# microsoft/tutel

Measured on AMD Instinct MI355X. Metric: MoE-layer fwd tokens/sec, 4096 tok x H=2048 x E=64 top-2, higher is better.
Workload: dtype bf16

## Files before the change

### include/tutel_amd.h

```cpp
#ifndef TUTEL_AMD_H
#define TUTEL_AMD_H

#include <stddef.h>
#include <stdint.h>

#ifdef __cplusplus
extern "C" {
#endif

#define TUTEL_AMD_ABI_VERSION 1

typedef void *tutel_stream_t;

enum { TUTEL_F32 = 0, TUTEL_F16 = 1, TUTEL_BF16 = 2, TUTEL_F64 = 3 };
enum { TUTEL_ACT_NONE = 0, TUTEL_ACT_RELU = 1, TUTEL_ACT_GELU = 2, TUTEL_ACT_SILU = 3 };

int tutel_amd_abi_version(void);
const char *tutel_amd_target_arch(void);
const char *tutel_amd_last_error(void);

size_t tutel_amd_routing_workspace_bytes(int T, int E, int k);

int tutel_amd_gate_topk(const void *in, int dtype, int apply_softmax, int T, int E, int k,
                        int normalize_gate, void *scores_out, int32_t *idx, void *gates, void *ws,
                        size_t ws_bytes, int32_t *clear_map, int clear_n, tutel_stream_t stream);

int tutel_amd_gate_proj_splits(int T, int M, int E, int dtype);
int tutel_amd_gate_proj(const void *x, const void *wg, int dtype, int T, int M, int E, float *partials,
                        size_t partial_bytes, tutel_stream_t stream);
int tutel_amd_gate_topk_partials(const float *partials, int splits, int dtype, int T, int E, int k,
                                 int normalize_gate, void *logits_out, void *scores_out, int32_t *idx, void *gates,
                                 void *ws, size_t ws_bytes, int32_t *clear_map, int clear_n, tutel_stream_t stream);

int tutel_amd_cache_warm(const void *p, size_t chunk_bytes, int n_chunks, size_t stride_bytes, int blocks, void *sink4,
                         tutel_stream_t stream);

int tutel_amd_compute_location(const int32_t *idx, int T, int E, int k, int hist_ready, void *ws,
                               size_t ws_bytes, int32_t *loc, int32_t *dispatch_count,
                               int32_t *stats, void *l_aux, int l_aux_dtype, int capacity,
                               int32_t *slot_map, int slot_map_cleared, tutel_stream_t stream);

int tutel_amd_slot_map(const int32_t *idx, const int32_t *loc, int T, int E, int k, int capacity,
                       int32_t *slot_map, tutel_stream_t stream);

int tutel_amd_cumsum_sub_one(const int32_t *mask, int32_t *out, int T, int E,
                             tutel_stream_t stream);

int tutel_amd_fast_encode(const void *x, int dtype, const int32_t *slot_map, const void *gates,
                          int gate_dtype, int T, int M, int n_slots, int capacity, int num_experts,
                          int chunk_rows, int expert_slice, int ep_world, void *out,
                          tutel_stream_t stream);

int tutel_amd_fast_decode(const void *buf, int dtype, const int32_t *idx, const int32_t *loc,
                          const void *gates, int gate_dtype, int T, int M, int k, int capacity,
                          int num_experts, int chunk_rows, int expert_slice, int ep_world, void *out,
                          tutel_stream_t stream);

int tutel_amd_gate_grad(const void *x, const void *buf, int dtype, const int32_t *idx,
                        const int32_t *loc, int T, int M, int k, int capacity, float *ggate,
                        tutel_stream_t stream);

int tutel_amd_expert_gemm(const void *A, int64_t a_stride_e, int64_t a_stride_w, int a_rows_per_w,
                          int lda, const void *W, int w_kmajor, int64_t w_stride_e, int ldw,
                          const void *bias, int64_t bias_stride_e, void *D, int64_t d_stride_e,
                          int64_t d_stride_w, int d_rows_per_w, int ldd, int E_loc, int R, int N,
                          int K, int dtype, int act, const int32_t *row_counts, int row_align,
                          tutel_stream_t stream);

int tutel_amd_expert_gemm_gather(const void *X, int ldx, const int32_t *slot_map, int T,
                                 const void *zero_row, const void *W, int w_kmajor,
                                 int64_t w_stride_e, int ldw, const void *bias,
                                 int64_t bias_stride_e, void *D, int64_t d_stride_e, int ldd,
                                 int E_loc, int R, int N, int K, int dtype, int act,
                                 const int32_t *row_counts, int row_align, tutel_stream_t stream);

int tutel_amd_expert_ffn(const void *A, int64_t x_stride_e, int ldx, const int32_t *slot_map, int T, const void *zero_row,
                         const void *W1, int64_t w1_stride_e, int ldw1, const void *b1, int64_t b1_stride_e, void *hid,
                         int64_t hid_stride_e, int ldh, const void *W2, int64_t w2_stride_e, int ldw2, const void *b2,
                         int64_t b2_stride_e, void *D, int64_t d_stride_e, int ldd, int E_loc, int R, int M, int H, int M_out,
                         int dtype, int act, tutel_stream_t stream);

int tutel_amd_expert_gemm_glu(const void *A, int64_t a_stride_e, int64_t a_stride_w,
                              int a_rows_per_w, int lda, const void *W, int w_kmajor,
                              int64_t w_stride_e, int ldw, const void *bias, int64_t bias_stride_e,
                              const void *G, void *D, int64_t d_stride_e, int64_t d_stride_w,
                              int d_rows_per_w, int ldd, int E_loc, int R, int N, int K, int dtype,
                              int act, const int32_t *row_counts, int row_align,
                              tutel_stream_t stream);

int tutel_amd_expert_gemm_gate_up(const void *A, int64_t a_stride_e, int64_t a_stride_w, int a_rows_per_w, int lda,
                                  const void *W_gate, const void *W_up, int64_t w_stride_e, int ldw, void *D, int64_t d_stride_e,
                                  int64_t d_stride_w, int d_rows_per_w, int ldd, int E_loc, int R, int N, int K, int dtype, int act,
                                  const int32_t *row_counts, int row_align, tutel_stream_t stream);

typedef struct tutel_amd_ep_comm tutel_amd_ep_comm_t;
#define TUTEL_AMD_EP_ID_BYTES 128

int tutel_amd_ep_load_rccl(const char *path_hint );
int tutel_amd_ep_unique_id(void *out, size_t bytes );
int tutel_amd_ep_comm_create(const void *id, size_t bytes, int world, int rank, tutel_amd_ep_comm_t **out);
int tutel_amd_ep_comm_destroy(tutel_amd_ep_comm_t *comm);
typedef int (*tutel_amd_exchange_fn)(void *user, const void *send, void *recv, size_t bytes_per_peer, int world);
int tutel_amd_ep_comm_create_hosted(int world, int rank, tutel_amd_exchange_fn fn, void *user, tutel_amd_ep_comm_t **out);
int tutel_amd_ep_comm_info(const tutel_amd_ep_comm_t *comm, int *world, int *rank);

typedef struct tutel_amd_ep_segment tutel_amd_ep_segment_t;
#define TUTEL_AMD_IPC_HANDLE_BYTES 64
int tutel_amd_ep_segment_alloc(size_t bytes, int flag_memory, tutel_amd_ep_segment_t **out, void *handle_out, size_t handle_bytes);
int tutel_amd_ep_segment_open(tutel_amd_ep_segment_t *seg, int world, int rank, const void *handles, size_t handle_bytes);
void *tutel_amd_ep_segment_ptr(const tutel_amd_ep_segment_t *seg, int peer);
int tutel_amd_ep_segment_read(const tutel_amd_ep_segment_t *seg, size_t off, void *dst, size_t bytes, tutel_stream_t stream);
int tutel_amd_ep_segment_free(tutel_amd_ep_segment_t *seg);
size_t tutel_amd_ep_flag_bytes(void);
int tutel_amd_ep_comm_create_ipc(int world, int rank, tutel_amd_ep_comm_t **out);
int tutel_amd_ep_comm_attach_ipc(tutel_amd_ep_comm_t *comm, tutel_amd_ep_segment_t *flags, int timeout_ms);
int tutel_amd_ep_comm_has_ipc(const tutel_amd_ep_comm_t *comm);
int tutel_amd_ep_ipc_set_timeout(tutel_amd_ep_comm_t *comm, int timeout_ms);
int tutel_amd_ep_ipc_status(tutel_amd_ep_comm_t *comm);
int tutel_amd_ep_ipc_exchange(tutel_amd_ep_comm_t *comm, tutel_amd_ep_segment_t *seg, const void *send, size_t bytes_per_peer,
                              size_t recv_off, tutel_stream_t stream);
int tutel_amd_ep_ipc_selfcheck(tutel_amd_ep_comm_t *comm, tutel_amd_ep_segment_t *seg, size_t bytes_per_peer, int passes, int flavour,
                               int side_stream, unsigned long long *mismatch, tutel_stream_t stream);

int tutel_amd_ep_all_to_all(tutel_amd_ep_comm_t *comm, const void *send, void *recv, size_t bytes_per_peer,
                            tutel_stream_t stream);

typedef int (*tutel_amd_exchange_v_fn)(void *user, const void *send, void *recv, const uint64_t *send_bytes,
                                       const uint64_t *send_offsets, const uint64_t *recv_bytes, int world);
int tutel_amd_ep_comm_set_hosted_v(tutel_amd_ep_comm_t *comm, tutel_amd_exchange_v_fn fn);
int tutel_amd_ep_all_to_all_v(tutel_amd_ep_comm_t *comm, const void *send, void *recv, const uint64_t *send_bytes,
                              const uint64_t *recv_bytes, tutel_stream_t stream);
int tutel_amd_ep_all_gather_v(tutel_amd_ep_comm_t *comm, const void *send, void *recv, const uint64_t *recv_bytes,
                              tutel_stream_t stream);

typedef struct {
  int sliced;
  int experts_per_stage;
  int chunk;
  int rows;
  int gemm_rows;
} tutel_amd_ep_plan_t;
int tutel_amd_ep_plan(int num_experts, int world, int capacity, int degree, int allow_sliced, tutel_amd_ep_plan_t *out);

typedef struct {
  int T, M, H, M_out;
  int num_experts, world, k;
  int capacity;
  int degree;
  int allow_sliced;
  int dtype, gate_dtype, act;
  int is_postscore;
  int w2_kmajor;
  int fuse_encode;
  const void *x;
  const int32_t *slot_map;
  const int32_t *idx, *loc;
  const void *gates;
  const void *w1, *b1, *w2, *b2;
  void *enc, *recv, *hid, *send, *back;
  const void *zero_row;
  const int32_t *row_counts;
  int row_align;
  void *y;
  const struct tutel_amd_ep_segment *peer_seg;
} tutel_amd_ep_args_t;
int tutel_amd_ep_forward(tutel_amd_ep_comm_t *comm, const tutel_amd_ep_args_t *args, tutel_stream_t stream);

typedef struct {
  tutel_amd_ep_args_t ep;
  const void *logits;
  int logits_dtype;
  int normalize_gate;
  void *ws;
  size_t ws_bytes;
  int32_t *dispatch_count;
  int32_t *stats;
  void *l_aux;
  int capacity_limit, alignment, max_capacity;
  int *capacity_out;
  const void *gate_w;
  float *gate_partials;
  size_t gate_partial_bytes;
  void *logits_out;
  void *fl_ws;
  size_t fl_ws_bytes;
} tutel_amd_moe_args_t;
#define TUTEL_AMD_EAGAIN 1000
#define TUTEL_AMD_ENOTSUP 1001
int tutel_amd_moe_forward(tutel_amd_ep_comm_t *comm, const tutel_amd_moe_args_t *args, tutel_stream_t stream);

typedef struct {
  void *ws;
  size_t ws_bytes;
  int32_t *offsets;
  int32_t *capacity;
} tutel_amd_packed_args_t;
typedef struct {
  int rows_bound;
  int tiles_bound;
  int tile_rows;
  int row_limit;
  size_t ws_bytes;
} tutel_amd_packed_plan_t;
int tutel_amd_packed_plan(int T, int E, int k, int M, int H, int M_out, int dtype, int capacity_limit, int alignment,
                          tutel_amd_packed_plan_t *out);
size_t tutel_amd_moe_packed_workspace_bytes(int T, int E, int k, int M, int H, int M_out, int dtype, int capacity_limit,
                                            int alignment);
int tutel_amd_moe_forward_packed(tutel_amd_ep_comm_t *comm, const tutel_amd_moe_args_t *args,
                                 const tutel_amd_packed_args_t *packed, tutel_stream_t stream);
int tutel_amd_moe_forward_packed_glu(tutel_amd_ep_comm_t *comm, const tutel_amd_moe_args_t *args,
                                     const tutel_amd_packed_args_t *packed, const void *w_up, tutel_stream_t stream);

int tutel_amd_packed_layout(const int32_t *dispatch_count, const int32_t *idx, const int32_t *loc, int T, int E, int k,
                            int capacity_limit, int alignment, int rows_bound, int tiles_bound, int32_t *offsets, int32_t *tiles,
                            int32_t *ntiles, int32_t *capacity, int32_t *slot_map, tutel_stream_t stream);
int tutel_amd_expert_gemm_packed(const void *A, int lda, const int32_t *a_rows, int T, const void *zero_row, const void *W,
                                 int w_kmajor, int64_t w_stride_e, int ldw, const void *bias, int64_t bias_stride_e, const void *mul,
                                 void *D, int ldd, int E, int rows_bound, int N, int K, int dtype, int act, const int32_t *offsets,
                                 const int32_t *tiles, const int32_t *ntiles, const int32_t *capacity, int tiles_bound,
                                 tutel_stream_t stream);
int tutel_amd_expert_wgrad_packed(const void *A, int lda, const void *B, int ldb, const int32_t *rows_map, int gather, int T,
                                  const void *zero_row, void *D, int E, int rows_bound, int Na, int Nb, int dtype,
                                  const int32_t *offsets, tutel_stream_t stream);
int tutel_amd_expert_bgrad_packed(const void *B, int ldb, void *D, int E, int N, int dtype, const int32_t *offsets,
                                  tutel_stream_t stream);
int tutel_amd_gate_grad_packed(const void *x, const void *buf, int dtype, const int32_t *idx, const int32_t *loc, int T, int M,
                               int k, int row_limit, const int32_t *offsets, float *ggate, tutel_stream_t stream);
int tutel_amd_fast_decode_packed(const void *buf, int dtype, const int32_t *idx, const int32_t *loc, const void *gates, int gate_dtype,
                                 int T, int M, int k, int row_limit, const int32_t *offsets, void *out, tutel_stream_t stream);

int tutel_amd_range_push(const char *name);
int tutel_amd_range_pop(void);

enum {
  TUTEL_STAGE_GATE_TOPK = 0, TUTEL_STAGE_LOCATION = 1, TUTEL_STAGE_ENCODE = 2, TUTEL_STAGE_FC1 = 3, TUTEL_STAGE_FC2 = 4,
  TUTEL_STAGE_DECODE = 5, TUTEL_STAGE_A2A_DISPATCH = 6, TUTEL_STAGE_A2A_COMBINE = 7, TUTEL_STAGE_OTHER = 8, TUTEL_STAGE_GATE_PROJ = 9,
  TUTEL_STAGE_COUNT = 10
};
int tutel_amd_stage_timing(int enable);
int tutel_amd_stage_report(double *total_us, int *counts, int n_stages );
int tutel_amd_mark(tutel_stream_t stream);
int tutel_amd_marks_reserve(int n);
int tutel_amd_marks_report(double *delta_us, int n);

#define TUTEL_OPT_GEMM_IMPL 0
#define TUTEL_OPT_GEMM_TILE 1
#define TUTEL_OPT_DECODE 2
#define TUTEL_OPT_EP_STAGE_GRID 3
#define TUTEL_OPT_GEMM_PERSIST 4
#define TUTEL_OPT_EP_STREAMS 5
#define TUTEL_OPT_EP_CANARY 6
#define TUTEL_OPT_GEMM_SPLITK 7
#define TUTEL_OPT_GEMM_GATHER 8
#define TUTEL_OPT_FUSED_LOCATION 9
#define TUTEL_OPT_GEMM_STORE 10
#define TUTEL_OPT_TIE_RULE 11
#define TUTEL_OPT_FFN_FUSED 12
#define TUTEL_OPT_COUNT 13
int tutel_amd_set_option(int key, int value);

int tutel_amd_probe_tr16(uint16_t *out, tutel_stream_t stream);

#ifdef __cplusplus
}
#endif
#endif
```

### tutel_amd/_lib.py

```python
import ctypes
import os
import subprocess

_HERE = os.path.dirname(os.path.abspath(__file__))
LIB_PATH = os.path.join(_HERE, "lib", "libtutel_amd.so")
CSRC_DIR = os.path.join(_HERE, "csrc")

F32, F16, BF16, F64 = 0, 1, 2, 3
ACT_NONE, ACT_RELU, ACT_GELU, ACT_SILU = 0, 1, 2, 3
OPT_GEMM_IMPL, OPT_GEMM_TILE, OPT_DECODE, OPT_EP_STAGE_GRID, OPT_GEMM_PERSIST, OPT_EP_STREAMS, OPT_EP_CANARY, OPT_GEMM_SPLITK, OPT_GEMM_GATHER, OPT_FUSED_LOCATION, OPT_GEMM_STORE, OPT_TIE_RULE, OPT_FFN_FUSED = 0, 1, 2, 3, 4, 5, 6, 7, 8, 9, 10, 11, 12

_vp, _i, _i64, _sz = ctypes.c_void_p, ctypes.c_int, ctypes.c_int64, ctypes.c_size_t

SIGNATURES = {
    "tutel_amd_abi_version": (_i, []),
    "tutel_amd_target_arch": (ctypes.c_char_p, []),
    "tutel_amd_last_error": (ctypes.c_char_p, []),
    "tutel_amd_routing_workspace_bytes": (_sz, [_i, _i, _i]),
    "tutel_amd_gate_topk": (_i, [_vp, _i, _i, _i, _i, _i, _i, _vp, _vp, _vp, _vp, _sz, _vp, _i, _vp]),
    "tutel_amd_gate_proj_splits": (_i, [_i, _i, _i, _i]),
    "tutel_amd_gate_proj": (_i, [_vp, _vp, _i, _i, _i, _i, _vp, _sz, _vp]),
    "tutel_amd_gate_topk_partials": (_i, [_vp, _i, _i, _i, _i, _i, _i, _vp, _vp, _vp, _vp, _vp, _sz, _vp, _i, _vp]),
    "tutel_amd_cache_warm": (_i, [_vp, _sz, _i, _sz, _i, _vp, _vp]),
    "tutel_amd_compute_location": (_i, [_vp, _i, _i, _i, _i, _vp, _sz, _vp, _vp, _vp, _vp, _i, _i, _vp, _i, _vp]),
    "tutel_amd_slot_map": (_i, [_vp, _vp, _i, _i, _i, _i, _vp, _vp]),
    "tutel_amd_cumsum_sub_one": (_i, [_vp, _vp, _i, _i, _vp]),
    "tutel_amd_fast_encode": (_i, [_vp, _i, _vp, _vp, _i, _i, _i, _i, _i, _i, _i, _i, _i, _vp, _vp]),
    "tutel_amd_fast_decode": (_i, [_vp, _i, _vp, _vp, _vp, _i, _i, _i, _i, _i, _i, _i, _i, _i, _vp, _vp]),
    "tutel_amd_gate_grad": (_i, [_vp, _vp, _i, _vp, _vp, _i, _i, _i, _i, _vp, _vp]),
    "tutel_amd_expert_gemm": (_i, [_vp, _i64, _i64, _i, _i, _vp, _i, _i64, _i, _vp, _i64, _vp, _i64,
                                   _i64, _i, _i, _i, _i, _i, _i, _i, _i, _vp, _i, _vp]),
    "tutel_amd_expert_gemm_gather": (_i, [_vp, _i, _vp, _i, _vp, _vp, _i, _i64, _i, _vp, _i64, _vp, _i64, _i,
                                          _i, _i, _i, _i, _i, _i, _vp, _i, _vp]),
    "tutel_amd_expert_ffn": (_i, [_vp, _i64, _i, _vp, _i, _vp, _vp, _i64, _i, _vp, _i64, _vp, _i64, _i, _vp, _i64, _i, _vp, _i64, _vp, _i64, _i,
                                  _i, _i, _i, _i, _i, _i, _i, _vp]),
    "tutel_amd_expert_gemm_glu": (_i, [_vp, _i64, _i64, _i, _i, _vp, _i, _i64, _i, _vp, _i64, _vp, _vp, _i64,
                                       _i64, _i, _i, _i, _i, _i, _i, _i, _i, _vp, _i, _vp]),
    "tutel_amd_expert_gemm_gate_up": (_i, [_vp, _i64, _i64, _i, _i, _vp, _vp, _i64, _i, _vp, _i64, _i64, _i, _i,
                                           _i, _i, _i, _i, _i, _i, _vp, _i, _vp]),
    "tutel_amd_set_option": (_i, [_i, _i]),
    "tutel_amd_probe_tr16": (_i, [_vp, _vp]),
}



class EpPlan(ctypes.Structure):
    _fields_ = [(n, _i) for n in ("sliced", "experts_per_stage", "chunk", "rows", "gemm_rows")]


class EpArgs(ctypes.Structure):
    _fields_ = ([(n, _i) for n in ("T", "M", "H", "M_out", "num_experts", "world", "k", "capacity", "degree", "allow_sliced",
                                   "dtype", "gate_dtype", "act", "is_postscore", "w2_kmajor", "fuse_encode")] +
                [(n, _vp) for n in ("x", "slot_map", "idx", "loc", "gates", "w1", "b1", "w2", "b2",
                                    "enc", "recv", "hid", "send", "back", "zero_row", "row_counts")] +
                [("row_align", _i), ("y", _vp), ("peer_seg", _vp)])


class MoeArgs(ctypes.Structure):
    _fields_ = [("ep", EpArgs), ("logits", _vp), ("logits_dtype", _i), ("normalize_gate", _i), ("ws", _vp), ("ws_bytes", _sz),
                ("dispatch_count", _vp), ("stats", _vp), ("l_aux", _vp),
                ("capacity_limit", _i), ("alignment", _i), ("max_capacity", _i), ("capacity_out", ctypes.POINTER(_i)),
                ("gate_w", _vp), ("gate_partials", _vp), ("gate_partial_bytes", _sz), ("logits_out", _vp),
                ("fl_ws", _vp), ("fl_ws_bytes", _sz)]


class PackedArgs(ctypes.Structure):
    _fields_ = [("ws", _vp), ("ws_bytes", _sz), ("offsets", _vp), ("capacity", _vp)]


class PackedPlan(ctypes.Structure):
    _fields_ = [("rows_bound", _i), ("tiles_bound", _i), ("tile_rows", _i), ("row_limit", _i), ("ws_bytes", _sz)]


SIGNATURES.update({
    "tutel_amd_moe_forward": (_i, [_vp, ctypes.POINTER(MoeArgs), _vp]),
    "tutel_amd_packed_plan": (_i, [_i] * 9 + [ctypes.POINTER(PackedPlan)]),
    "tutel_amd_moe_packed_workspace_bytes": (_sz, [_i] * 9),
    "tutel_amd_moe_forward_packed": (_i, [_vp, ctypes.POINTER(MoeArgs), ctypes.POINTER(PackedArgs), _vp]),
    "tutel_amd_moe_forward_packed_glu": (_i, [_vp, ctypes.POINTER(MoeArgs), ctypes.POINTER(PackedArgs), _vp, _vp]),
    "tutel_amd_packed_layout": (_i, [_vp, _vp, _vp] + [_i] * 7 + [_vp] * 6),
    "tutel_amd_expert_gemm_packed": (_i, [_vp, _i, _vp, _i, _vp, _vp, _i, _i64, _i, _vp, _i64, _vp, _vp] + [_i] * 7 + [_vp] * 4 + [_i, _vp]),
    "tutel_amd_expert_wgrad_packed": (_i, [_vp, _i, _vp, _i, _vp, _i, _i, _vp, _vp] + [_i] * 5 + [_vp, _vp]),
    "tutel_amd_expert_bgrad_packed": (_i, [_vp, _i, _vp, _i, _i, _i, _vp, _vp]),
    "tutel_amd_gate_grad_packed": (_i, [_vp, _vp, _i, _vp, _vp] + [_i] * 4 + [_vp, _vp, _vp]),
    "tutel_amd_fast_decode_packed": (_i, [_vp, _i, _vp, _vp, _vp] + [_i] * 5 + [_vp, _vp, _vp]),
    "tutel_amd_ep_load_rccl": (_i, [ctypes.c_char_p]),
    "tutel_amd_ep_unique_id": (_i, [_vp, _sz]),
    "tutel_amd_ep_comm_create": (_i, [_vp, _sz, _i, _i, ctypes.POINTER(_vp)]),
    "tutel_amd_ep_comm_destroy": (_i, [_vp]),
    "tutel_amd_ep_comm_create_hosted": (_i, [_i, _i, _vp, _vp, ctypes.POINTER(_vp)]),
    "tutel_amd_ep_comm_info": (_i, [_vp, ctypes.POINTER(_i), ctypes.POINTER(_i)]),
    "tutel_amd_ep_all_to_all": (_i, [_vp, _vp, _vp, _sz, _vp]),
    "tutel_amd_ep_comm_set_hosted_v": (_i, [_vp, _vp]),
    "tutel_amd_ep_all_to_all_v": (_i, [_vp, _vp, _vp, ctypes.POINTER(ctypes.c_uint64), ctypes.POINTER(ctypes.c_uint64), _vp]),
    "tutel_amd_ep_all_gather_v": (_i, [_vp, _vp, _vp, ctypes.POINTER(ctypes.c_uint64), _vp]),
    "tutel_amd_ep_plan": (_i, [_i, _i, _i, _i, _i, ctypes.POINTER(EpPlan)]),
    "tutel_amd_ep_forward": (_i, [_vp, ctypes.POINTER(EpArgs), _vp]),
    "tutel_amd_ep_segment_alloc": (_i, [_sz, _i, ctypes.POINTER(_vp), _vp, _sz]),
    "tutel_amd_ep_segment_open": (_i, [_vp, _i, _i, _vp, _sz]),
    "tutel_amd_ep_segment_ptr": (_vp, [_vp, _i]),
    "tutel_amd_ep_segment_read": (_i, [_vp, _sz, _vp, _sz, _vp]),
    "tutel_amd_ep_segment_free": (_i, [_vp]),
    "tutel_amd_ep_flag_bytes": (_sz, []),
    "tutel_amd_ep_comm_create_ipc": (_i, [_i, _i, ctypes.POINTER(_vp)]),
    "tutel_amd_ep_comm_attach_ipc": (_i, [_vp, _vp, _i]),
    "tutel_amd_ep_comm_has_ipc": (_i, [_vp]),
    "tutel_amd_ep_ipc_set_timeout": (_i, [_vp, _i]),
    "tutel_amd_ep_ipc_status": (_i, [_vp]),
    "tutel_amd_ep_ipc_exchange": (_i, [_vp, _vp, _vp, _sz, _sz, _vp]),
    "tutel_amd_ep_ipc_selfcheck": (_i, [_vp, _vp, _sz, _i, _i, _i, _vp, _vp]),
    "tutel_amd_mark": (_i, [_vp]),
    "tutel_amd_marks_reserve": (_i, [_i]),
    "tutel_amd_marks_report": (_i, [ctypes.POINTER(ctypes.c_double), _i]),
    "tutel_amd_stage_timing": (_i, [_i]),
    "tutel_amd_stage_report": (_i, [ctypes.POINTER(ctypes.c_double), ctypes.POINTER(_i), _i]),
    "tutel_amd_range_push": (_i, [ctypes.c_char_p]),
    "tutel_amd_range_pop": (_i, []),
})
EXCHANGE_FN = ctypes.CFUNCTYPE(_i, _vp, _vp, _vp, _sz, _i)
_u64p = ctypes.POINTER(ctypes.c_uint64)
EXCHANGE_V_FN = ctypes.CFUNCTYPE(_i, _vp, _vp, _vp, _u64p, _u64p, _u64p, _i)
EP_ID_BYTES = 128
IPC_HANDLE_BYTES = 64
EAGAIN, ENOTSUP = 1000, 1001
STAGES = ("gate_topk", "location", "fast_encode", "expert_fc1", "expert_fc2", "fast_decode", "all_to_all_dispatch", "all_to_all_combine", "other",
          "gate_projection")

_lib = None


class TutelAmdError(RuntimeError):
    pass


def build(force=False):
    if force or not os.path.exists(LIB_PATH):
        subprocess.check_call(["make", "-C", CSRC_DIR, "-j8"] + (["-B"] if force else []))
    return LIB_PATH


def lib():
    global _lib
    if _lib is None:
        import torch
        if not os.path.exists(LIB_PATH):
            raise TutelAmdError(
                f"tutel_amd: HIP library {LIB_PATH} is missing. Build it with "
                f"`python -c 'import __graft_entry__ as g; g.build()'` or `make -C tutel_amd/csrc` "
                f"(hipcc --offload-arch=gfx950). There is no CPU fallback for the MoE hot path.")
        try:
            handle = ctypes.CDLL(LIB_PATH)
        except OSError as ex:
            raise TutelAmdError(f"tutel_amd: cannot load {LIB_PATH}: {ex}") from ex
        for name, (res, args) in SIGNATURES.items():
            try:
                fn = getattr(handle, name)
            except AttributeError as ex:
                raise TutelAmdError(f"tutel_amd: {LIB_PATH} does not export `{name}` (stale build?)") from ex
            fn.restype, fn.argtypes = res, args
        if handle.tutel_amd_abi_version() != 1:
            raise TutelAmdError("tutel_amd: ABI version mismatch between python and libtutel_amd.so")
        _lib = handle
    return _lib


def check(status, what):
    if status != 0:
        msg = lib().tutel_amd_last_error().decode("utf-8", "replace")
        raise TutelAmdError(f"{what} failed (status {status}): {msg}")
```

### tutel_amd/csrc/api.hip

```cpp
#include <stdarg.h>
#include <stdlib.h>

#include "common.h"

static thread_local char g_err[512] = "";

void tutel_set_error(const char *fmt, ...) {
  va_list ap;
  va_start(ap, fmt);
  vsnprintf(g_err, sizeof(g_err), fmt, ap);
  va_end(ap);
}

extern "C" int tutel_amd_abi_version(void) { return TUTEL_AMD_ABI_VERSION; }
extern "C" const char *tutel_amd_target_arch(void) { return "gfx950"; }
extern "C" const char *tutel_amd_last_error(void) { return g_err; }

static int g_opt[TUTEL_OPT_COUNT] = {-2, -2, -2, -2, -2, -2, -2, -2, -2, -2, -2, -2, -2};
static const char *const g_opt_env[TUTEL_OPT_COUNT] = {"TUTEL_AMD_GEMM_IMPL", "TUTEL_AMD_GEMM_BIG", "TUTEL_AMD_DECODE", "TUTEL_AMD_EP_STAGE_GRID",
                                                       "TUTEL_AMD_GEMM_PERSIST", "TUTEL_AMD_EP_STREAMS", "TUTEL_AMD_EP_CANARY", "TUTEL_AMD_GEMM_SPLITK",
                                                       "TUTEL_AMD_GEMM_GATHER", "TUTEL_AMD_FUSED_LOCATION", "TUTEL_AMD_GEMM_STORE", "TUTEL_AMD_TIE_RULE", "TUTEL_AMD_FFN_FUSED"};

int tutel_get_option(int key) {
  if (key < 0 || key >= TUTEL_OPT_COUNT) return -1;
  if (g_opt[key] == -2) {
    const char *s = getenv(g_opt_env[key]);
    g_opt[key] = s ? atoi(s) : -1;
  }
  return g_opt[key];
}

extern "C" int tutel_amd_set_option(int key, int value) {
  TUTEL_REQUIRE(key >= 0 && key < TUTEL_OPT_COUNT, "tutel_amd_set_option: unknown key %d", key);
  TUTEL_REQUIRE(value >= -1 && value <= 7, "tutel_amd_set_option: value %d out of range", value);
  g_opt[key] = value;
  return 0;
}

#include <dlfcn.h>
static thread_local int g_stage_hint = -1;
static int (*g_roctx_push)(const char *) = nullptr;
static int (*g_roctx_pop)() = nullptr;
static void roctx_init() {
  static bool done = false;
  if (done) return;
  done = true;
  void *h = dlopen("libroctx64.so", RTLD_NOW | RTLD_NOLOAD);
  if (h == nullptr) h = dlopen("libroctx64.so.4", RTLD_NOW | RTLD_NOLOAD);
  if (h == nullptr && getenv("TUTEL_AMD_ROCTX") != nullptr) h = dlopen("libroctx64.so", RTLD_NOW | RTLD_GLOBAL);
  if (h == nullptr) return;
  g_roctx_push = (int (*)(const char *))dlsym(h, "roctxRangePushA");
  g_roctx_pop = (int (*)())dlsym(h, "roctxRangePop");
  if (g_roctx_push == nullptr || g_roctx_pop == nullptr) g_roctx_push = nullptr;
}
extern "C" int tutel_amd_range_push(const char *name) {
  roctx_init();
  return g_roctx_push ? g_roctx_push(name) : 0;
}
extern "C" int tutel_amd_range_pop(void) { return g_roctx_push ? g_roctx_pop() : 0; }
static const char *const g_stage_names[TUTEL_STAGE_COUNT] = {
    "tutel_amd.gate_topk", "tutel_amd.compute_location", "tutel_amd.fast_encode", "tutel_amd.expert_fc1", "tutel_amd.expert_fc2",
    "tutel_amd.fast_decode", "tutel_amd.all_to_all_dispatch", "tutel_amd.all_to_all_combine", "tutel_amd.other", "tutel_amd.gate_projection"};
void tutel_stage_range_push(int stage) {
  roctx_init();
  if (g_stage_hint >= 0) stage = g_stage_hint;
  if (g_roctx_push) g_roctx_push(g_stage_names[stage >= 0 && stage < TUTEL_STAGE_COUNT ? stage : TUTEL_STAGE_OTHER]);
}
void tutel_stage_range_pop() {
  if (g_roctx_push) g_roctx_pop();
}

#include <mutex>
#include <vector>
static std::mutex g_meas_mu;
struct StageRec { hipEvent_t a, b; int stage; };
static std::vector<StageRec> g_recs;
static std::vector<std::pair<hipEvent_t, hipEvent_t>> g_free;
static int g_timing = 0;

void tutel_stage_hint(int stage) { g_stage_hint = stage; }
static thread_local int g_gemm_corun = 0;
void tutel_gemm_corun_hint(int on) { g_gemm_corun = on; }
int tutel_gemm_corun() { return g_gemm_corun; }

int tutel_stage_begin(int stage, hipStream_t st) {
  if (!g_timing) return -1;
  if (g_stage_hint >= 0) stage = g_stage_hint;
  if (g_timing == 2 && stage != TUTEL_STAGE_FC1 && stage != TUTEL_STAGE_FC2) return -1;
  hipStreamCaptureStatus cs = hipStreamCaptureStatusNone;
  if (hipStreamIsCapturing(st, &cs) != hipSuccess || cs != hipStreamCaptureStatusNone) return -1;
  std::lock_guard<std::mutex> lock(g_meas_mu);
  StageRec r;
  r.stage = stage;
  if (!g_free.empty()) {
    r.a = g_free.back().first;
    r.b = g_free.back().second;
    g_free.pop_back();
  } else if (hipEventCreateWithFlags(&r.a, hipEventReleaseToDevice) != hipSuccess ||
             hipEventCreateWithFlags(&r.b, hipEventReleaseToDevice) != hipSuccess) {
    return -1;
  }
  (void)hipEventRecord(r.a, st);
  g_recs.push_back(r);
  return (int)g_recs.size() - 1;
}
void tutel_stage_end(int token, hipStream_t st) {
  if (token < 0) return;
  std::lock_guard<std::mutex> lock(g_meas_mu);
  if (token < (int)g_recs.size()) (void)hipEventRecord(g_recs[token].b, st);
}

static std::vector<hipEvent_t> g_marks;
static std::vector<hipEvent_t> g_marks_free;
extern "C" int tutel_amd_mark(tutel_stream_t stream) {
  std::lock_guard<std::mutex> lock(g_meas_mu);
  hipEvent_t ev;
  if (!g_marks_free.empty()) {
    ev = g_marks_free.back();
    g_marks_free.pop_back();
  } else {
    TUTEL_REQUIRE(hipEventCreateWithFlags(&ev, hipEventReleaseToDevice) == hipSuccess, "tutel_amd_mark: cannot create an event");
  }
  TUTEL_REQUIRE(hipEventRecord(ev, (hipStream_t)stream) == hipSuccess, "tutel_amd_mark: hipEventRecord failed");
  g_marks.push_back(ev);
  return 0;
}
extern "C" int tutel_amd_marks_reserve(int n) {
  std::lock_guard<std::mutex> lock(g_meas_mu);
  while ((int)g_marks_free.size() < n) {
    hipEvent_t ev;
    TUTEL_REQUIRE(hipEventCreateWithFlags(&ev, hipEventReleaseToDevice) == hipSuccess, "tutel_amd_marks_reserve: cannot create an event");
    g_marks_free.push_back(ev);
  }
  return 0;
}
extern "C" int tutel_amd_marks_report(double *delta_us, int n) {
  std::lock_guard<std::mutex> lock(g_meas_mu);
  const int have = (int)g_marks.size();
  int m = 0;
  for (int i = 0; i + 1 < have; ++i) {
    float ms = 0.f;
    if (hipEventSynchronize(g_marks[i + 1]) == hipSuccess && hipEventElapsedTime(&ms, g_marks[i], g_marks[i + 1]) == hipSuccess && m < n && delta_us)
      delta_us[m++] = 1e3 * ms;
  }
  for (auto ev : g_marks) g_marks_free.push_back(ev);
  g_marks.clear();
  return m;
}

extern "C" int tutel_amd_stage_timing(int enable) {
  g_timing = enable < 0 ? 0 : enable > 2 ? 1 : enable;
  return 0;
}

extern "C" int tutel_amd_stage_report(double *total_us, int *counts, int n_stages) {
  TUTEL_REQUIRE(total_us != nullptr && counts != nullptr && n_stages >= TUTEL_STAGE_COUNT, "tutel_amd_stage_report: need arrays of %d entries", TUTEL_STAGE_COUNT);
  for (int i = 0; i < n_stages; ++i) { total_us[i] = 0.0; counts[i] = 0; }
  std::lock_guard<std::mutex> lock(g_meas_mu);
  for (auto &r : g_recs) {
    float ms = 0.f;
    if (hipEventSynchronize(r.b) == hipSuccess && hipEventElapsedTime(&ms, r.a, r.b) == hipSuccess && r.stage >= 0 && r.stage < n_stages) {
      total_us[r.stage] += 1e3 * ms;
      counts[r.stage] += 1;
    }
    g_free.push_back({r.a, r.b});
  }
  g_recs.clear();
  return 0;
}
```

### tutel_amd/csrc/common.h

```cpp
#pragma once
#include <hip/hip_runtime.h>
#include <stdint.h>
#include <stdio.h>
#include <string.h>

#include "../../include/tutel_amd.h"

#define WAVE 64

void tutel_set_error(const char *fmt, ...);
int tutel_get_option(int key);

int tutel_stage_begin(int stage, hipStream_t st);
void tutel_stage_end(int token, hipStream_t st);
void tutel_stage_hint(int stage);
void tutel_gemm_corun_hint(int on);
int tutel_gemm_corun();
void tutel_stage_range_push(int stage);
void tutel_stage_range_pop();
struct StageScope {
  int token;
  hipStream_t st;
  StageScope(int stage, hipStream_t s) : token(tutel_stage_begin(stage, s)), st(s) { tutel_stage_range_push(stage); }
  ~StageScope() {
    tutel_stage_end(token, st);
    tutel_stage_range_pop();
  }
};

#define EP_NCAN 16
struct PeerCanary {
  const uint32_t *epoch;
  long long off;
  int world;
  int stale;
};
struct EncodePeer {
  const uint64_t *tab;
  long long off;
  int rank, rows;
  int slot0;
  PeerCanary can;
};
int tutel_encode_launch(const void *x, int dtype, const int32_t *slot_map, const void *gates, int gate_dtype, int T, int M,
                        int n_slots, int capacity, int num_experts, int chunk_rows, int expert_slice, int ep_world, void *out,
                        const EncodePeer &peer, hipStream_t st);
int tutel_expert_gemm_peer(const void *A, int64_t a_stride_e, int64_t a_stride_w, int a_rows_per_w, int lda, const void *W,
                           int w_kmajor, int64_t w_stride_e, int ldw, const void *bias, int64_t bias_stride_e,
                           const uint64_t *d_peer, int64_t d_peer_off, int64_t d_stride_e, int d_rows_per_w, int ldd, int E_loc,
                           int R, int N, int K, int dtype, int act, const PeerCanary &can, hipStream_t st);

int tutel_expert_gemm_gather_fl(const void *X, int ldx, int32_t *slot_map, int T, const void *zero_row, const void *W, int64_t w_stride_e,
                                int ldw, const void *bias, int64_t bias_stride_e, void *D, int64_t d_stride_e, int ldd, int E_loc, int R,
                                int N, int K, int dtype, int act, const uint8_t *idx8, int n, int32_t *loc, hipStream_t st);
int tutel_expert_ffn(const void *X, int64_t x_stride_e, int ldx, const int32_t *slot_map, int T, const void *zero_row, const void *W1,
                     int64_t w1_stride_e, int ldw1, const void *b1, int64_t b1_stride_e, void *hid, int64_t hid_stride_e, int ldh,
                     const void *W2, int64_t w2_stride_e, int ldw2, const void *b2, int64_t b2_stride_e, void *D, int64_t d_stride_e, int ldd,
                     int E_loc, int R, int M, int H, int M_out, int dtype, int act, const uint8_t *idx8, int n, int32_t *loc, int query,
                     hipStream_t st);
struct RouteFinish;
void tutel_route_finish_args(int T, int E, int k, void *ws, RouteFinish *out);
int tutel_decode_finish_launch(const void *buf, int dtype, const int32_t *idx, const int32_t *loc, const void *gates, int gate_dtype, int T, int M,
                               int k, int capacity, int num_experts, void *out, const RouteFinish &fin, hipStream_t st);
#define PK_TILE_ROWS 256
int tutel_expert_gemm_packed(const void *A, int lda, const int32_t *a_rows, int T, const void *zero_row, const void *W, int64_t w_stride_e,
                             int ldw, const void *bias, int64_t bias_stride_e, void *D, int ldd, int E, int rows_bound, int N, int K, int dtype,
                             int act, const int32_t *off, const int32_t *tiles, const int32_t *ntiles, const int32_t *cap, int tiles_bound,
                             hipStream_t st);
int tutel_expert_gemm_packed_ex(const void *A, int lda, const int32_t *a_rows, int T, const void *zero_row, const void *W, int w_kmajor,
                                int64_t w_stride_e, int ldw, const void *bias, int64_t bias_stride_e, const void *mul, void *D, int ldd, int E,
                                int rows_bound, int N, int K, int dtype, int act, const int32_t *off, const int32_t *tiles, const int32_t *ntiles,
                                const int32_t *cap, int tiles_bound, hipStream_t st);
int tutel_expert_gemm_gate_up_packed(const void *A, int lda, const int32_t *a_rows, int T, const void *zero_row, const void *W_gate,
                                     const void *W_up, int64_t w_stride_e, int ldw, void *D, int ldd, int E, int rows_bound, int N, int K,
                                     int dtype, int act, const int32_t *off, const int32_t *tiles, const int32_t *ntiles, const int32_t *cap,
                                     int tiles_bound, hipStream_t st);
int tutel_decode_packed_launch(const void *buf, int dtype, const int32_t *idx, const int32_t *loc, const void *gates, int gate_dtype, int T,
                               int M, int k, int row_limit, const int32_t *off, void *out, hipStream_t st);
int tutel_gate_topk_launch(const void *in, const float *partials, int splits, int dtype, int T, int E, int k, int normalize_gate,
                           void *logits_out, int32_t *idx, void *gates, void *ws, int32_t *clear_map, int clear_n, uint8_t *idx8,
                           hipStream_t st);

#define TUTEL_REQUIRE(cond, ...)           \
  do {                                     \
    if (!(cond)) {                         \
      tutel_set_error(__VA_ARGS__);        \
      return -1;                           \
    }                                      \
  } while (0)

#define TUTEL_CHECK_LAUNCH(what)                                                    \
  do {                                                                              \
    hipError_t _e = hipGetLastError();                                              \
    if (_e != hipSuccess) {                                                         \
      tutel_set_error("%s: launch failed: %s", what, hipGetErrorString(_e));        \
      return (int)_e;                                                               \
    }                                                                               \
  } while (0)

struct bf16_t { uint16_t v; };
struct f16_t { _Float16 v; };

__device__ __forceinline__ uint16_t f32_to_bf16_bits(float f) {
  uint32_t u = __float_as_uint(f);
  if ((u & 0x7fffffffu) > 0x7f800000u) return 0x7fc0;
  u += 0x7fffu + ((u >> 16) & 1u);
  return (uint16_t)(u >> 16);
}
__device__ __forceinline__ float bf16_bits_to_f32(uint16_t b) {
  return __uint_as_float(((uint32_t)b) << 16);
}

template <typename T> struct Elem;
template <> struct Elem<double> {
  using ct = double;
  static constexpr int dtype = 3;
  __device__ static __forceinline__ double to_f32(double x) { return x; }
  __device__ static __forceinline__ double from_f32(double x) { return x; }
  __device__ static __forceinline__ double eps() { return 2.220446049250313e-16; }
};
template <> struct Elem<float> {
  using ct = float;
  static constexpr int dtype = TUTEL_F32;
  __device__ static __forceinline__ float to_f32(float x) { return x; }
  __device__ static __forceinline__ float from_f32(float x) { return x; }
  __device__ static __forceinline__ float eps() { return 1.1920928955078125e-07f; }
};
template <> struct Elem<bf16_t> {
  using ct = float;
  static constexpr int dtype = TUTEL_BF16;
  __device__ static __forceinline__ float to_f32(bf16_t x) { return bf16_bits_to_f32(x.v); }
  __device__ static __forceinline__ bf16_t from_f32(float x) { return bf16_t{f32_to_bf16_bits(x)}; }
  __device__ static __forceinline__ float eps() { return 0.0078125f; }
};
template <> struct Elem<f16_t> {
  using ct = float;
  static constexpr int dtype = TUTEL_F16;
  __device__ static __forceinline__ float to_f32(f16_t x) { return (float)x.v; }
  __device__ static __forceinline__ f16_t from_f32(float x) { return f16_t{(_Float16)x}; }
  __device__ static __forceinline__ float eps() { return 0.0009765625f; }
};

template <typename T> __device__ __forceinline__ typename Elem<T>::ct round_to(typename Elem<T>::ct x) {
  return Elem<T>::to_f32(Elem<T>::from_f32(x));
}
__device__ __forceinline__ float ct_exp(float x) { return expf(x); }
__device__ __forceinline__ double ct_exp(double x) { return exp(x); }
__device__ __forceinline__ float ct_max(float a, float b) { return fmaxf(a, b); }
__device__ __forceinline__ double ct_max(double a, double b) { return fmax(a, b); }

static inline int dtype_size(int dtype) { return dtype == TUTEL_F32 ? 4 : 2; }
static inline bool dtype_ok(int dtype) {
  return dtype == TUTEL_F32 || dtype == TUTEL_F16 || dtype == TUTEL_BF16;
}

struct __attribute__((aligned(16))) vec16 { uint32_t w[4]; };

template <typename T> struct Vec;
template <> struct Vec<float> {
  static constexpr int N = 4;
  __device__ static __forceinline__ void unpack(const vec16 &v, float *f) {
#pragma unroll
    for (int i = 0; i < 4; ++i) f[i] = __uint_as_float(v.w[i]);
  }
  __device__ static __forceinline__ void pack(const float *f, vec16 &v) {
#pragma unroll
    for (int i = 0; i < 4; ++i) v.w[i] = __float_as_uint(f[i]);
  }
};
template <> struct Vec<bf16_t> {
  static constexpr int N = 8;
  __device__ static __forceinline__ void unpack(const vec16 &v, float *f) {
#pragma unroll
    for (int i = 0; i < 4; ++i) {
      f[2 * i] = __uint_as_float(v.w[i] << 16);
      f[2 * i + 1] = __uint_as_float(v.w[i] & 0xffff0000u);
    }
  }
  __device__ static __forceinline__ void pack(const float *f, vec16 &v) {
#pragma unroll
    for (int i = 0; i < 4; ++i)
      v.w[i] = (uint32_t)f32_to_bf16_bits(f[2 * i]) | ((uint32_t)f32_to_bf16_bits(f[2 * i + 1]) << 16);
  }
};
template <> struct Vec<f16_t> {
  static constexpr int N = 8;
  __device__ static __forceinline__ void unpack(const vec16 &v, float *f) {
#pragma unroll
    for (int i = 0; i < 4; ++i) {
      union { uint32_t u; _Float16 h[2]; } c;
      c.u = v.w[i];
      f[2 * i] = (float)c.h[0];
      f[2 * i + 1] = (float)c.h[1];
    }
  }
  __device__ static __forceinline__ void pack(const float *f, vec16 &v) {
#pragma unroll
    for (int i = 0; i < 4; ++i) {
      union { uint32_t u; _Float16 h[2]; } c;
      c.h[0] = (_Float16)f[2 * i];
      c.h[1] = (_Float16)f[2 * i + 1];
      v.w[i] = c.u;
    }
  }
};

__device__ __forceinline__ float mul_rn(float a, float b) { return __fmul_rn(a, b); }
__device__ __forceinline__ float add_rn(float a, float b) { return __fadd_rn(a, b); }

__device__ __forceinline__ int lane_id() { return (int)(threadIdx.x & 63); }
__device__ __forceinline__ float wave_max(float v) {
#pragma unroll
  for (int o = 32; o > 0; o >>= 1) v = fmaxf(v, __shfl_xor(v, o, 64));
  return v;
}
__device__ __forceinline__ float wave_sum(float v) {
#pragma unroll
  for (int o = 32; o > 0; o >>= 1) v += __shfl_xor(v, o, 64);
  return v;
}

__device__ __forceinline__ void peer_canary_store(const uint64_t *tab, const PeerCanary &c) {
  if (c.epoch == nullptr) return;
  const int nb = (int)gridDim.x, nlast = nb < EP_NCAN ? nb : EP_NCAN, back = nb - 1 - (int)blockIdx.x;
  if (back >= nlast) return;
  __syncthreads();
  const int t = (int)threadIdx.x;
  if (t >= c.world * EP_NCAN) return;
  const int w = t / EP_NCAN, j = t % EP_NCAN;
  if (j % nlast != back) return;
  const uint32_t e = *c.epoch + (c.stale ? 0u : 1u);
  reinterpret_cast<uint32_t *>(tab[w] + c.off)[j] = e;
}
```

### tutel_amd/csrc/ep.hip

```cpp
#include <dlfcn.h>
#include <stdlib.h>

#include <vector>

#include <rccl/rccl.h>

#include "common.h"
#include "routing_dev.h"

struct RcclApi {
  void *handle;
  ncclResult_t (*GetUniqueId)(ncclUniqueId *);
  ncclResult_t (*CommInitRank)(ncclComm_t *, int, ncclUniqueId, int);
  ncclResult_t (*CommDestroy)(ncclComm_t);
  ncclResult_t (*AllToAll)(const void *, void *, size_t, ncclDataType_t, ncclComm_t, hipStream_t);
  const char *(*GetErrorString)(ncclResult_t);
  ncclResult_t (*GroupStart)();
  ncclResult_t (*GroupEnd)();
  ncclResult_t (*Send)(const void *, size_t, ncclDataType_t, int, ncclComm_t, hipStream_t);
  ncclResult_t (*Recv)(void *, size_t, ncclDataType_t, int, ncclComm_t, hipStream_t);
};
static RcclApi g_rccl = {};

extern "C" int tutel_amd_ep_load_rccl(const char *path) {
// ... 623 lines not shown
      case 1: hipLaunchKernelGGL(ep_check_write_kernel<1>, dim3(grid), dim3(256), 0, st, seg->tab_dev, 0LL, vpp, c->world, c->rank, tag, can); break;
      case 2: hipLaunchKernelGGL(ep_check_write_kernel<2>, dim3(grid), dim3(256), 0, st, seg->tab_dev, 0LL, vpp, c->world, c->rank, tag, can); break;
      case 3: hipLaunchKernelGGL(ep_check_write_kernel<3>, dim3(grid), dim3(256), 0, st, seg->tab_dev, 0LL, vpp, c->world, c->rank, tag, can); break;
      default: hipLaunchKernelGGL(ep_check_write_kernel<0>, dim3(grid), dim3(256), 0, st, seg->tab_dev, 0LL, vpp, c->world, c->rank, tag, can);
    }
    TUTEL_CHECK_LAUNCH("tutel_amd_ep_ipc_selfcheck (write)");
    if ((rc = ipc_signal(c, 0, slot, 1, st)) != 0) break;
    if (rd != st) {
      HIP_CHECK(hipEventRecord(c->recv_ev[0], st), "hipEventRecord");
      HIP_CHECK(hipStreamWaitEvent(rd, c->recv_ev[0], 0), "hipStreamWaitEvent");
    }
    if ((rc = ipc_wait(c, 0, slot, 1, rd, seg)) != 0) break;
    hipLaunchKernelGGL(ep_check_read_kernel, dim3(grid), dim3(256), 0, rd, (const uint4 *)seg->local, vpp, c->world, c->rank, tag, mismatch);
    TUTEL_CHECK_LAUNCH("tutel_amd_ep_ipc_selfcheck (read)");
    if ((rc = ipc_signal(c, 1, slot, 1, rd)) != 0) break;
    if (rd != st) {
      HIP_CHECK(hipEventRecord(c->done_ev[0], rd), "hipEventRecord");
      HIP_CHECK(hipStreamWaitEvent(st, c->done_ev[0], 0), "hipStreamWaitEvent");
    }
  }
  if (rc == 0) rc = ipc_wait(c, 1, slot, 1, st);
  return rc;
}

extern "C" int tutel_amd_ep_plan(int E, int W, int capacity, int degree, int allow_sliced, tutel_amd_ep_plan_t *out) {
  TUTEL_REQUIRE(out != nullptr && E >= 1 && W >= 1 && E % W == 0 && degree >= 1 && degree <= EP_MAX_SPLIT && capacity >= 0,
                "tutel_amd_ep_plan: bad sizes E=%d W=%d C=%d degree=%d", E, W, capacity, degree);
  const int E_loc = E / W;
  out->sliced = (allow_sliced && E_loc >= degree && E_loc % degree == 0) ? 1 : 0;
  if (out->sliced) {
    out->experts_per_stage = E_loc / degree;
    out->chunk = capacity;
  } else {
    TUTEL_REQUIRE(capacity % degree == 0, "tutel_amd_ep_plan: capacity %d is not a multiple of a2a_ffn_overlap_degree %d", capacity, degree);
    out->experts_per_stage = E_loc;
    out->chunk = capacity / degree;
  }
  out->rows = out->experts_per_stage * out->chunk;
  out->gemm_rows = W * out->chunk;
  return 0;
}

extern "C" int tutel_amd_ep_forward(tutel_amd_ep_comm_t *c, const tutel_amd_ep_args_t *a, tutel_stream_t stream) {
  TUTEL_REQUIRE(a != nullptr, "tutel_amd_ep_forward: null arguments");
  const int W = a->world, E = a->num_experts, C = a->capacity, T = a->T, M = a->M, H = a->H, Mo = a->M_out, k = a->k;
  TUTEL_REQUIRE(W >= 1 && E >= 1 && E % W == 0 && T >= 0 && M >= 1 && H >= 1 && Mo >= 1 && k >= 1 && C >= 0,
                "tutel_amd_ep_forward: bad sizes");
  TUTEL_REQUIRE(c == nullptr ? W == 1 : c->world == W, "tutel_amd_ep_forward: communicator world size does not match (%d)", W);
  TUTEL_REQUIRE(a->dtype == TUTEL_BF16 || a->dtype == TUTEL_F16, "tutel_amd_ep_forward: bf16 / fp16 experts only (got dtype %d)", a->dtype);
  TUTEL_REQUIRE((T == 0 || (a->x && a->idx && a->loc && a->y)) && (a->slot_map || C == 0) && a->w1 && a->w2, "tutel_amd_ep_forward: null pointer");
  if (T == 0 && c == nullptr) return 0;
  const int E_loc = E / W, es = 2;
  hipStream_t cur = (hipStream_t)stream;
  const void *enc_gates = a->is_postscore ? nullptr : a->gates;
  const void *dec_gates = a->is_postscore ? a->gates : nullptr;
  TUTEL_REQUIRE(a->gates != nullptr || T == 0, "tutel_amd_ep_forward: null gates");
  TUTEL_REQUIRE(a->row_counts == nullptr || (W == 1 && c == nullptr && a->degree <= 1), "tutel_amd_ep_forward: row counts (megablocks) need a single rank");
  const int32_t *rcnt = a->row_counts;
  const int ralign = a->row_counts != nullptr && a->row_align >= 1 ? a->row_align : 1;

  if (C == 0) {
    if (T > 0) HIP_CHECK(hipMemsetAsync(a->y, 0, (size_t)T * Mo * es, cur), "hipMemsetAsync");
    return 0;
  }

  if (c == nullptr && a->degree <= 1 && a->is_postscore && a->fuse_encode) {
    TUTEL_REQUIRE(a->hid && a->send && a->zero_row, "tutel_amd_ep_forward: null workspace");
    int rc = TUTEL_AMD_ENOTSUP;
    if (rcnt == nullptr && a->w2_kmajor) {
      Range r("tutel_amd.expert_ffn");
      rc = tutel_expert_ffn(a->x, 0, M, a->slot_map, T, a->zero_row, a->w1, (int64_t)H * M, M, a->b1, H, a->hid, (int64_t)C * H, H, a->w2,
                            (int64_t)H * Mo, H, a->b2, Mo, a->send, (int64_t)C * Mo, Mo, E_loc, C, M, H, Mo, a->dtype, a->act, nullptr, 0, nullptr, 0, cur);
      if (rc != 0 && rc != TUTEL_AMD_ENOTSUP) return rc;
    }
    if (rc == TUTEL_AMD_ENOTSUP) {
      Range r("tutel_amd.expert_fc1");
      rc = tutel_amd_expert_gemm_gather(a->x, M, a->slot_map, T, a->zero_row, a->w1, 1, (int64_t)H * M, M, a->b1, H, a->hid,
                                        (int64_t)C * H, H, E_loc, C, H, M, a->dtype, a->act, rcnt, ralign, cur);
      if (rc) return rc;
      Range r2("tutel_amd.expert_fc2");
      rc = tutel_amd_expert_gemm(a->hid, (int64_t)C * H, 0, C, H, a->w2, a->w2_kmajor, (int64_t)H * Mo, a->w2_kmajor ? H : Mo, a->b2,
                                 Mo, a->send, (int64_t)C * Mo, 0, C, Mo, E_loc, C, Mo, H, a->dtype, TUTEL_ACT_NONE, rcnt, ralign, cur);
      if (rc) return rc;
    }
    Range r("tutel_amd.fast_decode");
    return tutel_amd_fast_decode(a->send, a->dtype, a->idx, a->loc, dec_gates, a->gate_dtype, T, Mo, k, C, E, 0, 0, 1, a->y, cur);
  }

  const bool ipc = a->peer_seg != nullptr;
  TUTEL_REQUIRE(a->recv && a->hid && a->back && (ipc || (a->enc && a->send)), "tutel_amd_ep_forward: null workspace");
  TUTEL_REQUIRE(rcnt == nullptr, "tutel_amd_ep_forward: row counts need the fused-encode single-rank route (is_postscore, fuse_encode)");
  const int degree = a->degree < 1 ? 1 : a->degree;
  tutel_amd_ep_plan_t pl;
  if (tutel_amd_ep_plan(E, W, C, degree, a->allow_sliced, &pl) != 0) return -1;
  const int s = pl.experts_per_stage, cc = pl.chunk, rows = pl.rows, R = pl.gemm_rows;
  const int chunk_rows = pl.sliced ? 0 : cc, expert_slice = pl.sliced ? s : 0;
  int rc;

  const size_t msg_in = (size_t)W * rows * M * es, msg_out = (size_t)W * rows * Mo * es;
  const size_t hid_stage = (size_t)s * R * H * es;
  const tutel_amd_ep_segment *seg = a->peer_seg;
  long long recv_off = 0, back_off = 0;
  if (ipc) {
    if (ipc_check(c, "tutel_amd_ep_forward") != 0) return -1;
    TUTEL_REQUIRE(seg->tab_dev != nullptr && seg->world == W && seg->rank == c->rank, "tutel_amd_ep_forward: the peer segment is not open for this communicator");
    recv_off = (const char *)a->recv - (const char *)seg->local;
    back_off = (const char *)a->back - (const char *)seg->local;
    TUTEL_REQUIRE(recv_off >= 0 && back_off >= 0 && (size_t)recv_off + degree * msg_in <= seg->bytes && (size_t)back_off + degree * msg_out <= seg->bytes &&
                      recv_off % 16 == 0 && back_off % 16 == 0,
                  "tutel_amd_ep_forward: recv / back must lie inside the peer segment");
  }
  auto stage_gemms = [&](int i, hipStream_t st) -> int {
    const char *recv_i = (const char *)a->recv + (size_t)i * msg_in;
    char *hid_i = (char *)a->hid + (size_t)i * hid_stage;
    const int e0 = pl.sliced ? i * s : 0;
    const char *w1 = (const char *)a->w1 + (size_t)e0 * H * M * es, *w2 = (const char *)a->w2 + (size_t)e0 * H * Mo * es;
    const char *b1 = a->b1 ? (const char *)a->b1 + (size_t)e0 * H * es : nullptr, *b2 = a->b2 ? (const char *)a->b2 + (size_t)e0 * Mo * es : nullptr;
    int r1;
    {
      Range r("tutel_amd.expert_fc1");
      tutel_stage_hint(TUTEL_STAGE_FC1);
      r1 = tutel_amd_expert_gemm(recv_i, (int64_t)cc * M, (int64_t)rows * M, cc, M, w1, 1, (int64_t)H * M, M, b1, H, hid_i,
                                 (int64_t)R * H, 0, R, H, s, R, H, M, a->dtype, a->act, nullptr, 1, st);
      tutel_stage_hint(-1);
      if (r1) return r1;
    }
    Range r("tutel_amd.expert_fc2");
    if (ipc)
      return tutel_expert_gemm_peer(hid_i, (int64_t)R * H, 0, R, H, w2, a->w2_kmajor, (int64_t)H * Mo, a->w2_kmajor ? H : Mo, b2, Mo, seg->tab_dev,
                                    back_off + (long long)(((size_t)i * W + c->rank) * rows * Mo * es), (int64_t)cc * Mo, cc, Mo, s, R, Mo, H, a->dtype,
                                    TUTEL_ACT_NONE, producer_canary(c, seg, 1, i), st);
    char *send_i = (char *)a->send + (size_t)i * msg_out;
    return tutel_amd_expert_gemm(hid_i, (int64_t)R * H, 0, R, H, w2, a->w2_kmajor, (int64_t)H * Mo, a->w2_kmajor ? H : Mo, b2, Mo, send_i,
                                 (int64_t)cc * Mo, (int64_t)rows * Mo, cc, Mo, s, R, Mo, H, a->dtype, TUTEL_ACT_NONE, nullptr, 1, st);
  };
  auto encode_stage = [&](int i, int nst) -> int {
    Range r("tutel_amd.fast_encode");
    EncodePeer pe = {ipc ? seg->tab_dev : nullptr, recv_off, ipc ? c->rank : 0, rows, i * W * rows, producer_canary(ipc ? c : nullptr, seg, 0, i)};
    return tutel_encode_launch(a->x, a->dtype, a->slot_map, enc_gates, a->gate_dtype, T, M, (i + nst) * W * rows, C, E, chunk_rows, expert_slice, W,
                               ipc ? nullptr : a->enc, pe, cur);
  };

  struct ForkGuard {
    hipStream_t cur;
    hipStream_t forked[2] = {nullptr, nullptr};
    hipEvent_t ev[2] = {nullptr, nullptr};
    void fork(int slot, hipStream_t ks, hipEvent_t join_ev) { forked[slot] = ks; ev[slot] = join_ev; }
    void joined(int slot) { forked[slot] = nullptr; }
    ~ForkGuard() {
      for (int j = 0; j < 2; ++j)
        if (forked[j] != nullptr && hipEventRecord(ev[j], forked[j]) == hipSuccess) (void)hipStreamWaitEvent(cur, ev[j], 0);
      tutel_gemm_corun_hint(0);
    }
  } guard{cur};

  if (ipc) {
    hipStream_t kss[2] = {cur, cur};
    if (degree > 1) side_streams_for(c, cur, kss);
    if (degree == 1) {
      rc = encode_stage(0, 1);
      if (rc) return rc;
      {
        StageScope sc(TUTEL_STAGE_A2A_DISPATCH, cur);
        if ((rc = ipc_signal(c, 0, 0, 1, cur)) != 0 || (rc = ipc_wait(c, 0, 0, 1, cur, seg)) != 0) return rc;
      }
      rc = stage_gemms(0, cur);
      if (rc) return rc;
      StageScope sc(TUTEL_STAGE_A2A_COMBINE, cur);
      if ((rc = ipc_signal(c, 1, 0, 1, cur)) != 0) return rc;
    } else {
      for (int i = 0; i < degree; ++i) {
        rc = encode_stage(i, 1);
        if (rc) return rc;
        {
          StageScope sc(TUTEL_STAGE_A2A_DISPATCH, cur);
          if ((rc = ipc_signal(c, 0, i, 1, cur)) != 0) return rc;
        }
        HIP_CHECK(hipEventRecord(c->recv_ev[i], cur), "hipEventRecord");
      }
      for (int i = 0; i < degree; ++i) {
        hipStream_t ks = kss[i & 1];
        HIP_CHECK(hipStreamWaitEvent(ks, c->recv_ev[i], 0), "hipStreamWaitEvent");
        guard.fork(i & 1, ks, c->done_ev[i]);
        {
          StageScope sc(TUTEL_STAGE_A2A_DISPATCH, ks);
          if ((rc = ipc_wait(c, 0, i, 1, ks, seg)) != 0) return rc;
        }
        tutel_gemm_corun_hint(kss[0] != kss[1] && tutel_get_option(TUTEL_OPT_EP_STAGE_GRID) != 0);
        rc = stage_gemms(i, ks);
        tutel_gemm_corun_hint(0);
        if (rc) return rc;
        StageScope sc(TUTEL_STAGE_A2A_COMBINE, ks);
        if ((rc = ipc_signal(c, 1, i, 1, ks)) != 0) return rc;
      }
      for (int j = 0; j < 2; ++j)
        if (guard.forked[j] != nullptr) {
          HIP_CHECK(hipEventRecord(guard.ev[j], guard.forked[j]), "hipEventRecord");
          HIP_CHECK(hipStreamWaitEvent(cur, guard.ev[j], 0), "hipStreamWaitEvent");
          guard.joined(j);
        }
    }
    {
      StageScope sc(TUTEL_STAGE_A2A_COMBINE, cur);
      if ((rc = ipc_wait(c, 1, 0, degree, cur, seg)) != 0) return rc;
    }
    Range r("tutel_amd.fast_decode");
    rc = tutel_amd_fast_decode(a->back, a->dtype, a->idx, a->loc, dec_gates, a->gate_dtype, T, Mo, k, C, E, chunk_rows, expert_slice, W, a->y, cur);
    if (rc != 0 || T == 0) return rc;
    StageScope sc(TUTEL_STAGE_DECODE, cur);
    hipLaunchKernelGGL(ep_poison_kernel, dim3(1), dim3(1024), 0, cur, (const uint32_t *)c->epochs, (uint32_t *)a->y, (size_t)T * Mo * es / 4);
    TUTEL_CHECK_LAUNCH("tutel_amd_ep_forward (poison)");
    return 0;
  }

  rc = encode_stage(0, degree);
  if (rc) return rc;
  if (degree == 1 || c == nullptr) {
    for (int i = 0; i < degree; ++i) {
      {
        Range r("tutel_amd.all_to_all");
        rc = exchange(c, (const char *)a->enc + (size_t)i * msg_in, (char *)a->recv + (size_t)i * msg_in, (size_t)rows * M * es, W, cur, TUTEL_STAGE_A2A_DISPATCH);
        if (rc) return rc;
      }
      rc = stage_gemms(i, cur);
      if (rc) return rc;
      Range r("tutel_amd.all_to_all");
      rc = exchange(c, (const char *)a->send + (size_t)i * msg_out, (char *)a->back + (size_t)i * msg_out, (size_t)rows * Mo * es, W, cur, TUTEL_STAGE_A2A_COMBINE);
      if (rc) return rc;
    }
  } else {
    hipStream_t kss[2];
    side_streams_for(c, cur, kss);
    {
      Range r("tutel_amd.all_to_all(dispatch)");
      for (int i = 0; i < degree; ++i) {
        rc = exchange(c, (const char *)a->enc + (size_t)i * msg_in, (char *)a->recv + (size_t)i * msg_in, (size_t)rows * M * es, W, cur, TUTEL_STAGE_A2A_DISPATCH);
        if (rc) return rc;
        HIP_CHECK(hipEventRecord(c->recv_ev[i], cur), "hipEventRecord");
      }
    }
    for (int i = 0; i < degree; ++i) {
      hipStream_t ks = kss[i & 1];
      HIP_CHECK(hipStreamWaitEvent(ks, c->recv_ev[i], 0), "hipStreamWaitEvent");
      guard.fork(0, ks, c->done_ev[i]);
      tutel_gemm_corun_hint(c->comm != nullptr && tutel_get_option(TUTEL_OPT_EP_STAGE_GRID) != 0);
      rc = stage_gemms(i, ks);
      tutel_gemm_corun_hint(0);
      if (rc) return rc;
      HIP_CHECK(hipEventRecord(c->done_ev[i], ks), "hipEventRecord");
      HIP_CHECK(hipStreamWaitEvent(cur, c->done_ev[i], 0), "hipStreamWaitEvent");
      guard.joined(0);
      Range r("tutel_amd.all_to_all(combine)");
      rc = exchange(c, (const char *)a->send + (size_t)i * msg_out, (char *)a->back + (size_t)i * msg_out, (size_t)rows * Mo * es, W, cur, TUTEL_STAGE_A2A_COMBINE);
      if (rc) return rc;
    }
  }

  Range r("tutel_amd.fast_decode");
  return tutel_amd_fast_decode(a->back, a->dtype, a->idx, a->loc, dec_gates, a->gate_dtype, T, Mo, k, C, E, chunk_rows, expert_slice, W, a->y, cur);
}

extern "C" int tutel_amd_moe_forward(tutel_amd_ep_comm_t *c, const tutel_amd_moe_args_t *m, tutel_stream_t stream) {
  TUTEL_REQUIRE(m != nullptr, "tutel_amd_moe_forward: null arguments");
  const tutel_amd_ep_args_t &a = m->ep;
  const int T = a.T, E = a.num_experts, k = a.k;
  const bool project = m->logits == nullptr && m->gate_w != nullptr;
  TUTEL_REQUIRE((m->logits != nullptr || project || T == 0) && m->ws != nullptr && m->dispatch_count != nullptr, "tutel_amd_moe_forward: null pointer");
  int splits = 0;
  if (project && T > 0) {
    TUTEL_REQUIRE(a.dtype == m->logits_dtype, "tutel_amd_moe_forward: the in-call gate projection needs the gate in the token dtype (%d vs %d)", m->logits_dtype, a.dtype);
    splits = tutel_amd_gate_proj_splits(T, a.M, E, a.dtype);
    TUTEL_REQUIRE(splits > 0, "tutel_amd_moe_forward: the in-call gate projection does not cover T=%d, M=%d, E=%d, dtype=%d (pass logits)", T, a.M, E, a.dtype);
    TUTEL_REQUIRE(a.x != nullptr && m->gate_partials != nullptr && m->gate_partial_bytes >= (size_t)splits * T * E * sizeof(float),
                  "tutel_amd_moe_forward: gate_partials must hold %d x %d x %d floats", splits, T, E);
  }
  TUTEL_REQUIRE(a.slot_map && (T == 0 || (a.idx && a.loc && a.gates)), "tutel_amd_moe_forward: null routing buffers");
  if (T == 0 && c == nullptr) return 0;
  const bool dropless = a.capacity <= 0;
  TUTEL_REQUIRE(!dropless || (c == nullptr && a.world == 1 && m->stats != nullptr && m->capacity_out != nullptr && m->max_capacity >= 1),
                "tutel_amd_moe_forward: dropless routing needs a single rank, stats, capacity_out and max_capacity");
  int32_t *smap = const_cast<int32_t *>(a.slot_map);
  int rc;
  const int Ho = a.H, Mo = a.M_out;
  bool fl = !dropless && c == nullptr && a.world == 1 && a.degree <= 1 && a.is_postscore && a.fuse_encode && T > 0 && k <= 8 && E <= 128 &&
            (long long)k * T <= 15360 && m->fl_ws != nullptr && m->fl_ws_bytes >= (((size_t)k * T + 15) & ~(size_t)15) &&
            (a.dtype == TUTEL_BF16 || a.dtype == TUTEL_F16) && a.row_counts == nullptr && a.hid && a.send && a.zero_row && a.loc && a.w1 &&
            ((uintptr_t)m->fl_ws & 15) == 0;
  if (fl) {
    TUTEL_REQUIRE(k >= 1 && k <= E, "tutel_amd_moe_forward: need 1 <= k <= E (got k=%d, E=%d)", k, E);
    TUTEL_REQUIRE(m->ws_bytes >= tutel_amd_routing_workspace_bytes(T, E, k), "tutel_amd_moe_forward: routing workspace too small (%zu bytes, need %zu)",
                  m->ws_bytes, tutel_amd_routing_workspace_bytes(T, E, k));
  }
  if (fl) {
    char keep[512];
    strncpy(keep, tutel_amd_last_error(), sizeof(keep) - 1);
    keep[sizeof(keep) - 1] = 0;
    fl = tutel_expert_gemm_gather_fl(a.x, a.M, smap, T, a.zero_row, a.w1, (int64_t)Ho * a.M, a.M, a.b1, Ho, a.hid, (int64_t)a.capacity * Ho, Ho, E,
                                     a.capacity, Ho, a.M, a.dtype, a.act, (const uint8_t *)m->fl_ws, k * T, nullptr, (hipStream_t)stream) == 0;
    if (!fl) tutel_set_error("%s", keep);
  }
  if (fl) {
    hipStream_t st = (hipStream_t)stream;
    uint8_t *idx8 = (uint8_t *)m->fl_ws;
    if (project) {
      rc = tutel_amd_gate_proj(a.x, m->gate_w, a.dtype, T, a.M, E, m->gate_partials, m->gate_partial_bytes, stream);
      if (rc) return rc;
    }
    rc = tutel_gate_topk_launch(project ? nullptr : m->logits, project ? m->gate_partials : nullptr, splits, m->logits_dtype, T, E, k,
                                m->normalize_gate, project ? m->logits_out : nullptr, const_cast<int32_t *>(a.idx), const_cast<void *>(a.gates),
                                m->ws, nullptr, 0, idx8, st);
    if (rc) return rc;
    if (m->capacity_out != nullptr) *m->capacity_out = a.capacity;
    rc = TUTEL_AMD_ENOTSUP;
    if (a.w2_kmajor) {
      Range r("tutel_amd.expert_ffn");
      rc = tutel_expert_ffn(a.x, 0, a.M, smap, T, a.zero_row, a.w1, (int64_t)Ho * a.M, a.M, a.b1, Ho, a.hid, (int64_t)a.capacity * Ho, Ho, a.w2,
                            (int64_t)Ho * Mo, Ho, a.b2, Mo, a.send, (int64_t)a.capacity * Mo, Mo, E, a.capacity, a.M, Ho, Mo, a.dtype, a.act, idx8, k * T,
                            const_cast<int32_t *>(a.loc), 0, st);
      if (rc != 0 && rc != TUTEL_AMD_ENOTSUP) return rc;
    }
    if (rc == TUTEL_AMD_ENOTSUP) {
      Range r("tutel_amd.expert_fc1");
      rc = tutel_expert_gemm_gather_fl(a.x, a.M, smap, T, a.zero_row, a.w1, (int64_t)Ho * a.M, a.M, a.b1, Ho, a.hid, (int64_t)a.capacity * Ho, Ho,
                                       E, a.capacity, Ho, a.M, a.dtype, a.act, idx8, k * T, const_cast<int32_t *>(a.loc), st);
      if (rc) return rc;
      Range r2("tutel_amd.expert_fc2");
      rc = tutel_amd_expert_gemm(a.hid, (int64_t)a.capacity * Ho, 0, a.capacity, Ho, a.w2, a.w2_kmajor, (int64_t)Ho * Mo, a.w2_kmajor ? Ho : Mo,
                                 a.b2, Mo, a.send, (int64_t)a.capacity * Mo, 0, a.capacity, Mo, E, a.capacity, Mo, Ho, a.dtype, TUTEL_ACT_NONE,
                                 nullptr, 1, stream);
      if (rc) return rc;
    }
    Range r("tutel_amd.fast_decode");
    RouteFinish fin;
    tutel_route_finish_args(T, E, k, m->ws, &fin);
    fin.on = 1;
    fin.dispatch_count = m->dispatch_count;
    fin.stats = m->stats;
    fin.l_aux = m->l_aux;
    fin.l_aux_dtype = m->logits_dtype;
    return tutel_decode_finish_launch(a.send, a.dtype, a.idx, a.loc, a.gates, m->logits_dtype, T, Mo, k, a.capacity, E, a.y, fin, st);
  }
  if (project && T > 0) {
    rc = tutel_amd_gate_proj(a.x, m->gate_w, a.dtype, T, a.M, E, m->gate_partials, m->gate_partial_bytes, stream);
    if (rc) return rc;
    rc = tutel_amd_gate_topk_partials(m->gate_partials, splits, a.dtype, T, E, k, m->normalize_gate, m->logits_out, nullptr,
                                      const_cast<int32_t *>(a.idx), const_cast<void *>(a.gates), m->ws, m->ws_bytes,
                                      dropless ? nullptr : smap, dropless ? 0 : E * a.capacity, stream);
  } else {
    rc = tutel_amd_gate_topk(m->logits, m->logits_dtype, 1, T, E, k, m->normalize_gate, nullptr, const_cast<int32_t *>(a.idx),
                             const_cast<void *>(a.gates), m->ws, m->ws_bytes, dropless ? nullptr : smap, dropless ? 0 : E * a.capacity, stream);
  }
  if (rc) return rc;
  rc = tutel_amd_compute_location(a.idx, T, E, k, 1, m->ws, m->ws_bytes, const_cast<int32_t *>(a.loc), m->dispatch_count, m->stats,
                                  m->l_aux, m->logits_dtype, dropless ? 0 : a.capacity, dropless ? nullptr : smap, dropless ? 0 : 1, stream);
  if (rc) return rc;
  tutel_amd_ep_args_t e = a;
  e.gate_dtype = m->logits_dtype;
  if (dropless) {
    hipStream_t st = (hipStream_t)stream;
    HIP_CHECK(hipMemcpyAsync(m->capacity_out, m->stats, sizeof(int), hipMemcpyDeviceToHost, st), "hipMemcpyAsync");
    HIP_CHECK(hipStreamSynchronize(st), "hipStreamSynchronize");
    int cap = *m->capacity_out;
    if (m->capacity_limit > 0 && cap > m->capacity_limit) cap = m->capacity_limit;
    const int al = m->alignment >= 1 ? m->alignment : 1;
    cap = (cap + al - 1) / al * al;
    *m->capacity_out = cap;
    if (cap > m->max_capacity) return TUTEL_AMD_EAGAIN;
    if (cap == 0) return hipMemsetAsync(a.y, 0, (size_t)T * a.M_out * 2, st) == hipSuccess ? 0 : -1;
    rc = tutel_amd_slot_map(a.idx, a.loc, T, E, k, cap, smap, stream);
    if (rc) return rc;
    e.capacity = cap;
  } else if (m->capacity_out != nullptr) {
    *m->capacity_out = a.capacity;
  }
  return tutel_amd_ep_forward(c, &e, stream);
}
```

### tutel_amd/csrc/gate_proj.hip

```cpp
#include "common.h"

typedef __attribute__((ext_vector_type(16))) float gp_f32x16;
typedef __attribute__((ext_vector_type(8))) __bf16 gp_bf16x8;
typedef __attribute__((ext_vector_type(8))) _Float16 gp_f16x8;
typedef __attribute__((ext_vector_type(4))) uint32_t gp_u32x4;
typedef __attribute__((ext_vector_type(4))) float gp_f32x4;

template <typename T> struct GpMma;
template <> struct GpMma<bf16_t> {
  __device__ static __forceinline__ gp_f32x16 run(gp_u32x4 a, gp_u32x4 b, gp_f32x16 c) {
    return __builtin_amdgcn_mfma_f32_32x32x16_bf16(__builtin_bit_cast(gp_bf16x8, a), __builtin_bit_cast(gp_bf16x8, b), c, 0, 0, 0);
  }
};
template <> struct GpMma<f16_t> {
  __device__ static __forceinline__ gp_f32x16 run(gp_u32x4 a, gp_u32x4 b, gp_f32x16 c) {
    return __builtin_amdgcn_mfma_f32_32x32x16_f16(__builtin_bit_cast(gp_f16x8, a), __builtin_bit_cast(gp_f16x8, b), c, 0, 0, 0);
  }
};

#define GP_TM 64
#define GP_THREADS 256
#define GP_PANEL 4096

__device__ __forceinline__ void gp_dma16(const uint16_t *g, uint16_t *l) {
  __builtin_amdgcn_global_load_lds((const __attribute__((address_space(1))) void *)g, (__attribute__((address_space(3))) void *)l, 16, 0, 0);
}

template <typename T, int ER, int NP>
__global__ __launch_bounds__(GP_THREADS) void gate_proj_kernel(const uint16_t *__restrict__ x, const uint16_t *__restrict__ wg,
                                                              int Tn, int M, int E, int S, float *__restrict__ part) {
  extern __shared__ __attribute__((aligned(16))) unsigned char smem[];
  uint16_t *sX = reinterpret_cast<uint16_t *>(smem);
  uint16_t *sW = sX + NP * GP_PANEL;
  constexpr int WPW = ER / 32;
  constexpr int NPW = ER / 64;

  const int tid = threadIdx.x, lane = tid & 63;
  const int wid = __builtin_amdgcn_readfirstlane(tid >> 6);
  const int b = blockIdx.x, s = b % S, tile = b / S;
  const int t0 = tile * GP_TM;
  const int kp0 = s * NP;
  const int npan = min(NP, M / 64 - kp0);

  const int rl = lane >> 3;
  {
    const uint16_t *xs[2], *ws[WPW];
#pragma unroll
    for (int i = 0; i < 2; ++i) {
      const int r = 8 * (wid * 2 + i) + rl;
      const int c = (lane & 7) ^ ((r >> 1) & 7);
      xs[i] = x + (size_t)min(t0 + r, Tn - 1) * M + (size_t)kp0 * 64 + c * 8;
    }
#pragma unroll
    for (int i = 0; i < WPW; ++i) {
      const int r = 8 * (wid * WPW + i) + rl;
      const int c = (lane & 7) ^ ((r >> 1) & 7);
      ws[i] = wg + (size_t)min(r, E - 1) * M + (size_t)kp0 * 64 + c * 8;
    }
#pragma unroll
    for (int p = 0; p < NP; ++p) {
      if (p < npan) {
#pragma unroll
        for (int i = 0; i < 2; ++i) gp_dma16(xs[i] + p * 64, sX + p * GP_PANEL + (wid * 2 + i) * 512);
#pragma unroll
        for (int i = 0; i < WPW; ++i) gp_dma16(ws[i] + p * 64, sW + p * (ER * 64) + (wid * WPW + i) * 512);
      }
    }
  }

  const int tt = wid & 1, eg = wid >> 1;
  const int l31 = lane & 31, kg = lane >> 5;
  const int sw = (l31 >> 1) & 7;
  int frag_k[4];
#pragma unroll
  for (int kk = 0; kk < 4; ++kk) frag_k[kk] = (((kk * 2 + kg) ^ sw) << 3);
  const int x_row = (tt * 32 + l31) * 64;
  const int w_row = (eg * NPW * 32 + l31) * 64;

  gp_f32x16 acc[NPW];
#pragma unroll
  for (int i = 0; i < NPW; ++i)
#pragma unroll
    for (int r = 0; r < 16; ++r) acc[i][r] = 0.f;

  constexpr int OPS = 2 + WPW;
#define GP_FRAGS(P, FA, FW)                                                                          \
  do {                                                                                               \
    const uint16_t *cx_ = sX + (P) * GP_PANEL + x_row, *cw_ = sW + (P) * (ER * 64) + w_row;          \
    _Pragma("unroll") for (int kk = 0; kk < 4; ++kk) {                                               \
      FA[kk] = *reinterpret_cast<const gp_u32x4 *>(cx_ + frag_k[kk]);                                \
      _Pragma("unroll") for (int i = 0; i < NPW; ++i)                                                \
        FW[kk][i] = *reinterpret_cast<const gp_u32x4 *>(cw_ + i * 32 * 64 + frag_k[kk]);             \
    }                                                                                                \
  } while (0)
#define GP_MMA(FA, FW)                                                                               \
  do {                                                                                               \
    _Pragma("unroll") for (int kk = 0; kk < 4; ++kk)                                                 \
      _Pragma("unroll") for (int i = 0; i < NPW; ++i) acc[i] = GpMma<T>::run(FW[kk][i], FA[kk], acc[i]); \
  } while (0)
  if (npan == NP) {
#pragma unroll
    for (int p = 0; p < NP; ++p) {
      asm volatile("s_waitcnt vmcnt(%0)" ::"n"((NP - 1 - p) * OPS) : "memory");
      __builtin_amdgcn_s_barrier();
      gp_u32x4 fa[4], fw[4][NPW];
      GP_FRAGS(p, fa, fw);
      __builtin_amdgcn_sched_barrier(0);
      GP_MMA(fa, fw);
      __builtin_amdgcn_sched_barrier(0);
    }
  } else {
    __syncthreads();
    for (int p = 0; p < npan; ++p) {
      gp_u32x4 fa[4], fw[4][NPW];
      GP_FRAGS(p, fa, fw);
      __builtin_amdgcn_sched_barrier(0);
      GP_MMA(fa, fw);
      __builtin_amdgcn_sched_barrier(0);
    }
  }
#undef GP_FRAGS
#undef GP_MMA

  const int t = t0 + tt * 32 + l31;
  if (t < Tn) {
    float *row = part + ((size_t)s * Tn + t) * E;
#pragma unroll
    for (int i = 0; i < NPW; ++i)
#pragma unroll
      for (int rg = 0; rg < 4; ++rg) {
        const int n = (eg * NPW + i) * 32 + rg * 8 + kg * 4;
        if (n < E) {
          gp_f32x4 v = {acc[i][rg * 4 + 0], acc[i][rg * 4 + 1], acc[i][rg * 4 + 2], acc[i][rg * 4 + 3]};
          *reinterpret_cast<gp_f32x4 *>(row + n) = v;
        }
      }
  }
}

struct GpPlan {
  int er, np, splits;
};
static bool gp_plan(int T, int M, int E, int dtype, GpPlan *out) {
  if (!(dtype == TUTEL_BF16 || dtype == TUTEL_F16) || T < 1 || E < 1 || E > 128 || (E & 3) || M < 64 || (M & 63)) return false;
  const int P = M / 64, ntt = (T + GP_TM - 1) / GP_TM;
  const int er = E <= 64 ? 64 : 128;
  int np = er == 64 ? 8 : 4;
  while (np > 2 && (long long)ntt * ((P + np - 1) / np) < 256) np >>= 1;
  const int S = (P + np - 1) / np;
  if (S > 64) return false;
  out->er = er;
  out->np = np;
  out->splits = S;
  return true;
}

extern "C" int tutel_amd_gate_proj_splits(int T, int M, int E, int dtype) {
  GpPlan pl;
  return gp_plan(T, M, E, dtype, &pl) ? pl.splits : 0;
}

template <typename T, int ER, int NP>
static int gp_launch(const void *x, const void *wg, int Tn, int M, int E, int S, float *part, hipStream_t st) {
  const size_t lds = (size_t)NP * (GP_PANEL + ER * 64) * 2;
  if (lds > 65536) (void)hipFuncSetAttribute((const void *)gate_proj_kernel<T, ER, NP>, hipFuncAttributeMaxDynamicSharedMemorySize, (int)lds);
  const int ntt = (Tn + GP_TM - 1) / GP_TM;
  hipLaunchKernelGGL((gate_proj_kernel<T, ER, NP>), dim3(ntt * S), dim3(GP_THREADS), lds, st, (const uint16_t *)x, (const uint16_t *)wg, Tn, M,
                     E, S, part);
  TUTEL_CHECK_LAUNCH("tutel_amd_gate_proj");
  return 0;
}

template <typename T>
static int gp_dispatch(const GpPlan &pl, const void *x, const void *wg, int Tn, int M, int E, float *part, hipStream_t st) {
  if (pl.er == 64) {
    if (pl.np == 8) return gp_launch<T, 64, 8>(x, wg, Tn, M, E, pl.splits, part, st);
    if (pl.np == 4) return gp_launch<T, 64, 4>(x, wg, Tn, M, E, pl.splits, part, st);
    return gp_launch<T, 64, 2>(x, wg, Tn, M, E, pl.splits, part, st);
  }
  if (pl.np == 4) return gp_launch<T, 128, 4>(x, wg, Tn, M, E, pl.splits, part, st);
  return gp_launch<T, 128, 2>(x, wg, Tn, M, E, pl.splits, part, st);
}

extern "C" int tutel_amd_gate_proj(const void *x, const void *wg, int dtype, int T, int M, int E, float *partials,
                                   size_t partial_bytes, tutel_stream_t stream) {
  GpPlan pl;
  if (T == 0) return 0;
  if (!gp_plan(T, M, E, dtype, &pl)) {
    tutel_set_error("tutel_amd_gate_proj: shape not covered (T=%d, M=%d, E=%d, dtype=%d): needs a 16-bit dtype, E <= 128, E %% 4 == 0, "
                    "M %% 64 == 0 -- use a library GEMM + tutel_amd_gate_topk", T, M, E, dtype);
    return TUTEL_AMD_ENOTSUP;
  }
  TUTEL_REQUIRE(x && wg && partials, "tutel_amd_gate_proj: null pointer");
  TUTEL_REQUIRE(((uintptr_t)x & 15) == 0 && ((uintptr_t)wg & 15) == 0 && ((uintptr_t)partials & 15) == 0,
                "tutel_amd_gate_proj: x, wg and partials must be 16-byte aligned");
  TUTEL_REQUIRE(partial_bytes >= (size_t)pl.splits * T * E * sizeof(float), "tutel_amd_gate_proj: partials buffer too small (%zu < %zu)",
                partial_bytes, (size_t)pl.splits * T * E * sizeof(float));
  hipStream_t st = (hipStream_t)stream;
  StageScope stage(TUTEL_STAGE_GATE_PROJ, st);
  if (dtype == TUTEL_BF16) return gp_dispatch<bf16_t>(pl, x, wg, T, M, E, partials, st);
  return gp_dispatch<f16_t>(pl, x, wg, T, M, E, partials, st);
}

#define CW_THREADS 512
#define CW_UNR 8
__global__ __launch_bounds__(CW_THREADS) void cache_warm_kernel(const unsigned char *__restrict__ base, size_t chunk_vec, int n_chunks,
                                                                size_t stride_bytes, uint32_t *__restrict__ sink) {
  const int c = blockIdx.x % n_chunks, bi = blockIdx.x / n_chunks, nbi = (gridDim.x - c + n_chunks - 1) / n_chunks;
  const gp_u32x4 *p = reinterpret_cast<const gp_u32x4 *>(base + (size_t)c * stride_bytes);
  const size_t stride = (size_t)nbi * CW_THREADS;
  size_t i = (size_t)bi * CW_THREADS + threadIdx.x;
  uint32_t acc = 0;
  for (; i + (CW_UNR - 1) * stride < chunk_vec; i += CW_UNR * stride) {
    gp_u32x4 v[CW_UNR];
#pragma unroll
    for (int u = 0; u < CW_UNR; ++u) v[u] = p[i + u * stride];
#pragma unroll
    for (int u = 0; u < CW_UNR; ++u) acc ^= v[u][u & 3];
  }
  for (; i < chunk_vec; i += stride) acc ^= p[i][0];
  if (acc == 0x9e3779b9u && sink != nullptr) *sink = acc;
}

extern "C" int tutel_amd_cache_warm(const void *p, size_t chunk_bytes, int n_chunks, size_t stride_bytes, int blocks, void *sink4,
                                    tutel_stream_t stream) {
  if (chunk_bytes < 16 || n_chunks < 1) return 0;
  TUTEL_REQUIRE(p != nullptr && ((uintptr_t)p & 15) == 0 && (stride_bytes & 15) == 0, "tutel_amd_cache_warm: pointer and stride must be 16-byte aligned");
  if (blocks < n_chunks) blocks = n_chunks > 256 ? n_chunks : 256;
  hipLaunchKernelGGL(cache_warm_kernel, dim3(blocks), dim3(CW_THREADS), 0, (hipStream_t)stream, (const unsigned char *)p, chunk_bytes / 16, n_chunks,
                     stride_bytes, (uint32_t *)sink4);
  TUTEL_CHECK_LAUNCH("tutel_amd_cache_warm");
  return 0;
}
```

### tutel_amd/csrc/routing.hip

```cpp
#include "common.h"
#include "routing_dev.h"
#include "topk_ties.h"

#define GT_THREADS 1024
#define GT_WAVES 16
#define RT_MAX_TILES 128
#define RT_MAX_K 16
#define RT_MAX_E 4096
#define GT_COL_SLAB 1024

static inline int rt_tile(int T) {
  int per = (T + 64 * RT_MAX_TILES - 1) / (64 * RT_MAX_TILES);
  if (per < 1) per = 1;
  return 64 * per;
}
static inline int rt_ntiles(int T) { return (T + rt_tile(T) - 1) / rt_tile(T); }

extern "C" size_t tutel_amd_routing_workspace_bytes(int T, int E, int k) {
  if (T <= 0 || E <= 0 || k <= 0) return 0;
  size_t nt = (size_t)rt_ntiles(T);
  return nt * ((size_t)k * E * sizeof(int32_t) + (size_t)E * sizeof(float));
}

template <typename T, int EPL, int GT_BATCH>
__global__ __launch_bounds__(GT_THREADS) void gate_topk_kernel(
    const T *__restrict__ in, int apply_softmax, int Tn, int E, int k, int normalize, int tile,
    T *__restrict__ scores_out, int32_t *__restrict__ idx, T *__restrict__ gates,
    int32_t *__restrict__ ws_hist, float *__restrict__ ws_colsum, int32_t *__restrict__ clear_map,
    int clear_n, int tie_mode) {
  using CT = typename Elem<T>::ct;
  extern __shared__ __attribute__((aligned(16))) unsigned char smem[];
  int32_t *s_hist = reinterpret_cast<int32_t *>(smem);
  float *s_col = reinterpret_cast<float *>(smem) + (size_t)k * E;
  const int tie_slots = tie_mode > 0 ? tie_mode : GT_WAVES, tie_slot = (int)(threadIdx.x >> 6) % tie_slots;
  CT *s_tv = reinterpret_cast<CT *>(smem + (((size_t)k * E * 4 + 7) & ~(size_t)7)) + (size_t)tie_slot * E;
  uint16_t *s_tp = reinterpret_cast<uint16_t *>(reinterpret_cast<CT *>(smem + (((size_t)k * E * 4 + 7) & ~(size_t)7)) + (size_t)tie_slots * E) +
                   (size_t)tie_slot * E;
  __shared__ int s_lock[GT_WAVES];

  const int tid = threadIdx.x, lane = tid & 63, wid = tid >> 6;
  const int b = blockIdx.x;
  const int t0 = b * tile, t1 = min(Tn, t0 + tile);

  if (clear_map != nullptr) {
    const int per = (clear_n + (int)gridDim.x - 1) / (int)gridDim.x;
    const int c0 = b * per, c1 = min(clear_n, c0 + per);
    for (int i = c0 + tid; i < c1; i += GT_THREADS) clear_map[i] = -1;
  }

  for (int i = tid; i < k * E; i += GT_THREADS) s_hist[i] = 0;
  if (tid < GT_WAVES) s_lock[tid] = 0;
  __syncthreads();

  float colacc[EPL];
#pragma unroll
  for (int j = 0; j < EPL; ++j) colacc[j] = 0.f;

  for (int tb = t0 + wid; tb < t1; tb += GT_WAVES * GT_BATCH) {
    CT v[GT_BATCH][EPL];
    bool live[GT_BATCH];
    int tt[GT_BATCH];
#pragma unroll
    for (int u = 0; u < GT_BATCH; ++u) {
      tt[u] = tb + u * GT_WAVES;
      live[u] = tt[u] < t1;
      const T *row = in + (size_t)min(tt[u], Tn - 1) * E;
#pragma unroll
      for (int j = 0; j < EPL; ++j) {
        int e = lane + 64 * j;
        v[u][j] = (e < E) ? Elem<T>::to_f32(row[e]) : -INFINITY;
      }
    }
    if (apply_softmax) {
      CT m[GT_BATCH], s[GT_BATCH];
#pragma unroll
      for (int u = 0; u < GT_BATCH; ++u) {
        m[u] = -INFINITY;
#pragma unroll
        for (int j = 0; j < EPL; ++j) m[u] = ct_max(m[u], v[u][j]);
      }
#pragma unroll
      for (int o = 32; o > 0; o >>= 1)
#pragma unroll
        for (int u = 0; u < GT_BATCH; ++u) m[u] = ct_max(m[u], __shfl_xor(m[u], o, 64));
#pragma unroll
      for (int u = 0; u < GT_BATCH; ++u) {
        s[u] = 0.f;
#pragma unroll
        for (int j = 0; j < EPL; ++j) {
          int e = lane + 64 * j;
          v[u][j] = (e < E) ? ct_exp(v[u][j] - m[u]) : 0.f;
          s[u] += v[u][j];
        }
      }
#pragma unroll
      for (int o = 32; o > 0; o >>= 1)
#pragma unroll
        for (int u = 0; u < GT_BATCH; ++u) s[u] += __shfl_xor(s[u], o, 64);
#pragma unroll
      for (int u = 0; u < GT_BATCH; ++u)
#pragma unroll
        for (int j = 0; j < EPL; ++j) {
          int e = lane + 64 * j;
          if (e < E) {
            T r = Elem<T>::from_f32(v[u][j] / s[u]);
            v[u][j] = Elem<T>::to_f32(r);
            if (scores_out && live[u]) scores_out[(size_t)tt[u] * E + e] = r;
          } else {
            v[u][j] = -INFINITY;
          }
        }
    }
    unsigned long long nanm[GT_BATCH];
#pragma unroll
    for (int u = 0; u < GT_BATCH; ++u) {
      nanm[u] = 0;
#pragma unroll
      for (int j = 0; j < EPL; ++j) {
        int e = lane + 64 * j;
        if (e < E && live[u]) colacc[j] += (float)v[u][j];
        if (v[u][j] != v[u][j]) { v[u][j] = -INFINITY; nanm[u] |= 1ull << j; }
      }
    }

    unsigned long long taken[GT_BATCH];
    CT myg[GT_BATCH], prev[GT_BATCH];
    int myidx[GT_BATCH];
    bool tied[GT_BATCH];
#pragma unroll
    for (int u = 0; u < GT_BATCH; ++u) { taken[u] = 0; myg[u] = 0; myidx[u] = -1; prev[u] = 0; tied[u] = false; }
    const int rounds = tie_mode ? k + 1 : k;
    for (int c = 0; c < rounds; ++c) {
      CT bv[GT_BATCH];
      int be[GT_BATCH];
#pragma unroll
      for (int u = 0; u < GT_BATCH; ++u) {
        bv[u] = -INFINITY;
        be[u] = 0x7fffffff;
#pragma unroll
        for (int j = 0; j < EPL; ++j) {
          int e = lane + 64 * j;
          bool ok = (e < E) && !((taken[u] >> j) & 1ull);
          if (ok && (v[u][j] > bv[u] || (v[u][j] == bv[u] && e < be[u]))) { bv[u] = v[u][j]; be[u] = e; }
        }
      }
#pragma unroll
      for (int o = 32; o > 0; o >>= 1)
#pragma unroll
        for (int u = 0; u < GT_BATCH; ++u) {
          CT ov = __shfl_xor(bv[u], o, 64);
          int oe = __shfl_xor(be[u], o, 64);
          if (ov > bv[u] || (ov == bv[u] && oe < be[u])) { bv[u] = ov; be[u] = oe; }
        }
#pragma unroll
      for (int u = 0; u < GT_BATCH; ++u) {
        if (c > 0 && bv[u] == prev[u] && be[u] != 0x7fffffff) tied[u] = true;
        prev[u] = bv[u];
        if (c < k) {
          if ((be[u] & 63) == lane) taken[u] |= 1ull << (be[u] >> 6);
          if (lane == c) { myg[u] = bv[u]; myidx[u] = be[u]; }
        }
      }
    }
    if (tie_mode) {
#pragma unroll
      for (int u = 0; u < GT_BATCH; ++u) {
        if (__ballot(nanm[u] != 0ull) != 0ull) tied[u] = true;
        if (tied[u] && live[u]) {
          const bool shared_slot = tie_slots < GT_WAVES;
          if (shared_slot) {
            if (lane == 0)
              while (atomicCAS(&s_lock[tie_slot], 0, 1) != 0) __builtin_amdgcn_s_sleep(2);
            __builtin_amdgcn_fence(__ATOMIC_ACQUIRE, "workgroup");
            __builtin_amdgcn_wave_barrier();
          }
#pragma unroll
          for (int j = 0; j < EPL; ++j) {
            int e = lane + 64 * j;
            if (e < E) {
              s_tv[e] = ((nanm[u] >> j) & 1ull) ? (CT)NAN : v[u][j];
              s_tp[e] = (uint16_t)e;
            }
          }
          __builtin_amdgcn_fence(__ATOMIC_RELEASE, "wavefront");
          __builtin_amdgcn_wave_barrier();
          if constexpr (EPL <= 4) {
            using Rep = typename TkRepOf<T>::type;
            WaveQueue<EPL, Rep> wq;
            wq.sel = reinterpret_cast<uint8_t *>(s_tp);
            wq.seln = E;
#pragma unroll
            for (int j = 0; j < EPL; ++j) wq.r[j] = Rep::make(((nanm[u] >> j) & 1ull) ? (CT)NAN : v[u][j], lane + 64 * j);
            AtenTopk<WaveQueue<EPL, Rep>> tsw(wq);
            tsw.run(E, k);
            if (lane < k) {
              myidx[u] = Rep::id_of(wq.r[0].unpack());
              myg[u] = s_tv[myidx[u]];
            }
          } else {
            if (lane == 0) {
              LdsQueue<CT, uint16_t> lq{s_tv, s_tp};
              AtenTopk<LdsQueue<CT, uint16_t>> ts(lq);
              ts.run(E, k);
            }
            __builtin_amdgcn_fence(__ATOMIC_ACQ_REL, "wavefront");
            __builtin_amdgcn_wave_barrier();
            if (lane < k) {
              myidx[u] = s_tp[lane];
              myg[u] = s_tv[myidx[u]];
            }
          }
          __builtin_amdgcn_fence(__ATOMIC_ACQ_REL, "wavefront");
          __builtin_amdgcn_wave_barrier();
          if (shared_slot) {
            __builtin_amdgcn_fence(__ATOMIC_RELEASE, "workgroup");
            __builtin_amdgcn_wave_barrier();
            if (lane == 0) __hip_atomic_store(&s_lock[tie_slot], 0, __ATOMIC_RELEASE, __HIP_MEMORY_SCOPE_WORKGROUP);
          }
        }
      }
    }
#pragma unroll
    for (int u = 0; u < GT_BATCH; ++u) {
      CT denom = __shfl(myg[u], 0, 64);
      for (int c = 1; c < k; ++c) denom = round_to<T>(denom + __shfl(myg[u], c, 64));
      if (lane < k && live[u]) {
        CT g = myg[u];
        if (normalize && k > 1) {
          CT d = ct_max(denom, (CT)Elem<T>::eps());
          if (denom != denom) d = denom;
          g = g / d;
        }
        gates[(size_t)lane * Tn + tt[u]] = Elem<T>::from_f32(g);
        idx[(size_t)lane * Tn + tt[u]] = myidx[u];
        atomicAdd(&s_hist[lane * E + myidx[u]], 1);
      }
    }
  }

  __syncthreads();
  for (int i = tid; i < k * E; i += GT_THREADS) ws_hist[(size_t)b * k * E + i] = s_hist[i];
  const int slab = E < GT_COL_SLAB ? E : GT_COL_SLAB;
  for (int e0 = 0; e0 < E; e0 += slab) {
#pragma unroll
    for (int j = 0; j < EPL; ++j) {
      int e = lane + 64 * j;
      if (e >= e0 && e < e0 + slab && e < E) s_col[wid * slab + (e - e0)] = colacc[j];
    }
    __syncthreads();
    for (int e = e0 + tid; e < e0 + slab && e < E; e += GT_THREADS) {
      float s = 0.f;
#pragma unroll
      for (int w = 0; w < GT_WAVES; ++w) s += s_col[w * slab + (e - e0)];
      ws_colsum[(size_t)b * E + e] = s;
    }
    __syncthreads();
  }
}

__global__ __launch_bounds__(RT_THREADS) void tile_hist_kernel(const int32_t *__restrict__ idx,
                                                              int Tn, int E, int k, int tile,
                                                              int32_t *__restrict__ ws_hist) {
  extern __shared__ __attribute__((aligned(16))) unsigned char smem[];
  int32_t *s_hist = reinterpret_cast<int32_t *>(smem);
  const int tid = threadIdx.x, b = blockIdx.x;
  const int t0 = b * tile, t1 = min(Tn, t0 + tile);
  for (int i = tid; i < k * E; i += RT_THREADS) s_hist[i] = 0;
  __syncthreads();
  for (int j = 0; j < k; ++j)
    for (int t = t0 + tid; t < t1; t += RT_THREADS) {
      int e = idx[(size_t)j * Tn + t];
      if (e >= 0 && e < E) atomicAdd(&s_hist[j * E + e], 1);
    }
  __syncthreads();
  for (int i = tid; i < k * E; i += RT_THREADS) ws_hist[(size_t)b * k * E + i] = s_hist[i];
}

template <int NW, bool COH = false>
__device__ __forceinline__ void loc_rank(int tid, int t0, int t1, int Tn, int E, int k, const int32_t *__restrict__ idx,
                                         const int32_t *lidx, int lidx_stride, int e_first, bool have_first, int32_t *s_cur,
                                         int32_t *__restrict__ loc, int capacity, int32_t *__restrict__ slot_map) {
  const int lane = tid & 63, wid = tid >> 6;
  int ebits = 0;
  while ((1 << ebits) < E) ++ebits;
  for (int j = wid; j < k; j += NW) {
    int32_t *cur = s_cur + j * E;
    for (int c0 = t0; c0 < t1; c0 += 64) {
      int t = c0 + lane;
      int e;
      if (have_first && j == wid && c0 == t0) e = e_first;
      else if (t >= t1) e = -1;
      else e = lidx != nullptr ? lidx[j * lidx_stride + (t - t0)] : idx[(size_t)j * Tn + t];
      bool valid = (e >= 0) && (e < E);
      unsigned long long same = __ballot(valid);
      for (int bit = 0; bit < ebits; ++bit) {
        const unsigned long long bb = __ballot(valid && ((e >> bit) & 1));
        same &= ((e >> bit) & 1) ? bb : ~bb;
      }
      const int rank = __popcll(same & ((1ull << lane) - 1ull));
      const int cnt = __popcll(same);
      const bool leader = valid && (__ffsll((long long)same) - 1 == lane);
      int base = valid ? cur[e] : 0;
      int l = base + rank;
      if (leader) cur[e] = base + cnt;
      if (t < t1) {
        loc[(size_t)j * Tn + t] = valid ? l : 0;
        if (slot_map != nullptr && valid && l < capacity) st_i32<COH>(slot_map + (size_t)e * capacity + l, j * Tn + t);
      }
    }
  }
}

__global__ __launch_bounds__(RT_THREADS) void location_kernel(
    const int32_t *__restrict__ idx, int Tn, int E, int k, int tile, int ntiles,
    const int32_t *__restrict__ ws_hist, const float *__restrict__ ws_colsum,
    int32_t *__restrict__ loc, int32_t *__restrict__ dispatch_count, int32_t *__restrict__ stats,
    void *__restrict__ l_aux, int l_aux_dtype, int capacity, int32_t *__restrict__ slot_map) {
  extern __shared__ __attribute__((aligned(16))) unsigned char smem[];
  int32_t *s_cur = reinterpret_cast<int32_t *>(smem);
  int32_t *s_tot = s_cur + (size_t)k * E;
  float *s_parts = reinterpret_cast<float *>(smem) + (size_t)2 * k * E;
  __shared__ float s_red[RT_WAVES];
  __shared__ int s_redi[RT_WAVES];

  const int tid = threadIdx.x, lane = tid & 63, wid = tid >> 6;
  const int b = blockIdx.x;
  const int t0 = b * tile, t1 = min(Tn, t0 + tile);

  int e_first = -1;
  if (wid < k && t0 + lane < t1) e_first = idx[(size_t)wid * Tn + t0 + lane];
  const int cs_parts = (E >= RT_THREADS) ? 1 : (RT_THREADS / E);
  const int cs_per = (ntiles + cs_parts - 1) / cs_parts;
  const bool cs_early = b == 0 && l_aux != nullptr && cs_parts * E <= RT_THREADS;
  float cs_first[16];
  if (cs_early && tid < cs_parts * E) {
    const int e = tid % E, a = (tid / E) * cs_per, z = min(ntiles, a + cs_per);
#pragma unroll
    for (int u = 0; u < 16; ++u) cs_first[u] = (a + u < z) ? ws_colsum[(size_t)(a + u) * E + e] : 0.f;
  }
  loc_prefix<RT_WAVES>(tid, b, E, k, ntiles, ws_hist, s_cur, s_tot, dispatch_count);
  loc_rank<RT_WAVES>(tid, t0, t1, Tn, E, k, idx, nullptr, 0, e_first, true, s_cur, loc, capacity, slot_map);
  if (b == 0) loc_finish<RT_WAVES>(tid, Tn, E, k, ntiles, ws_colsum, s_tot, s_parts, s_red, s_redi, cs_first, cs_early, stats, l_aux, l_aux_dtype);
}

#define GQ_LPT 16
#define GQ_THREADS 1024

template <typename V, int N> struct alignas((sizeof(V) * N) > 16 ? 16 : (sizeof(V) * N)) GqPack { V v[N]; };
template <typename V, int N> __device__ __forceinline__ void gq_load(const V *p, V (&o)[N]) {
  const GqPack<V, N> pk = *reinterpret_cast<const GqPack<V, N> *>(p);
#pragma unroll
  for (int i = 0; i < N; ++i) o[i] = pk.v[i];
}

template <typename T, int EPQ>
__global__ __launch_bounds__(GQ_THREADS) void gate_topk_quad_kernel(
    const T *__restrict__ in, int apply_softmax, int Tn, int E, int k, int normalize, int tile,
    T *__restrict__ scores_out, int32_t *__restrict__ idx, T *__restrict__ gates,
    int32_t *__restrict__ ws_hist, float *__restrict__ ws_colsum, int32_t *__restrict__ clear_map,
    int clear_n, const float *__restrict__ part, int nsplit, T *__restrict__ logits_out, uint8_t *__restrict__ idx8, int tie_mode) {
  using CT = typename Elem<T>::ct;
  extern __shared__ __attribute__((aligned(16))) unsigned char smem[];
  const int ES = GQ_LPT * EPQ + 1;
  int32_t *s_hist = reinterpret_cast<int32_t *>(smem);
  float *s_sc = reinterpret_cast<float *>(smem) + (size_t)k * E;
  CT *s_tv = reinterpret_cast<CT *>(smem + ((((size_t)k * E + (size_t)64 * ES) * 4 + 7) & ~(size_t)7));
  uint8_t *s_sel = reinterpret_cast<uint8_t *>(s_tv + (size_t)64 * E) + (size_t)(threadIdx.x >> 6) * 256;
  __shared__ int s_nlist[2];
  __shared__ int s_list[64];

  const int tid = threadIdx.x, q = tid & (GQ_LPT - 1), tl = tid / GQ_LPT;
  const int b = blockIdx.x;
  const int t0 = b * tile, t1 = min(Tn, t0 + tile);

  if (clear_map != nullptr) {
    const int per = (clear_n + (int)gridDim.x - 1) / (int)gridDim.x;
    const int c0 = b * per, c1 = min(clear_n, c0 + per);
    for (int i = c0 + tid; i < c1; i += GQ_THREADS) clear_map[i] = -1;
  }
  for (int i = tid; i < k * E; i += GQ_THREADS) s_hist[i] = 0;
  if (tid < 2) s_nlist[tid] = 0;
  float colsum = 0.f;
  __syncthreads();

  int pass = -1;
  for (int ts = t0; ts < t1; ts += 64) {
    ++pass;
    const int t = ts + tl;
    const bool live = t < t1;
    CT v[EPQ];
    if (part != nullptr) {
      const float *row = part + (size_t)min(t, Tn - 1) * E + q * EPQ;
      const size_t sstride = (size_t)Tn * E;
      const bool exact = E == GQ_LPT * EPQ;
      int ej[EPQ];
#pragma unroll
      for (int j = 0; j < EPQ; ++j) ej[j] = min(q * EPQ + j, E - 1) - q * EPQ;
      float a[EPQ];
#pragma unroll
      for (int j = 0; j < EPQ; ++j) a[j] = 0.f;
#define GQ_PART_SUM(LOAD)                                                                          \
      for (int s0 = 0; s0 < nsplit; s0 += 4) {                                                     \
        float b[4][EPQ];                                                                           \
        _Pragma("unroll") for (int i = 0; i < 4; ++i) {                                            \
          const float *rs = row + (size_t)min(s0 + i, nsplit - 1) * sstride;                       \
          LOAD;                                                                                    \
        }                                                                                          \
        _Pragma("unroll") for (int i = 0; i < 4; ++i)                                              \
          if (s0 + i < nsplit) {                                                                   \
            _Pragma("unroll") for (int j = 0; j < EPQ; ++j) a[j] = (s0 + i == 0) ? b[i][j] : a[j] + b[i][j]; \
          }                                                                                        \
      }
      if (exact) {
        GQ_PART_SUM((gq_load<float, EPQ>(rs, b[i])));
      } else {
        GQ_PART_SUM(_Pragma("unroll") for (int j = 0; j < EPQ; ++j) b[i][j] = rs[ej[j]]);
      }
#undef GQ_PART_SUM
#pragma unroll
      for (int j = 0; j < EPQ; ++j) {
        int e = q * EPQ + j;
        const T r = Elem<T>::from_f32((CT)a[j]);
        if (logits_out && live && e < E) logits_out[(size_t)t * E + e] = r;
        v[j] = (e < E) ? Elem<T>::to_f32(r) : -INFINITY;
      }
    } else {
      const T *row = in + (size_t)min(t, Tn - 1) * E + q * EPQ;
      T raw[EPQ];
      if (E == GQ_LPT * EPQ && (reinterpret_cast<uintptr_t>(in) & 15) == 0) {
        gq_load<T, EPQ>(row, raw);
      } else {
#pragma unroll
        for (int j = 0; j < EPQ; ++j) raw[j] = row[min(q * EPQ + j, E - 1) - q * EPQ];
      }
#pragma unroll
      for (int j = 0; j < EPQ; ++j) {
        int e = q * EPQ + j;
        v[j] = (e < E) ? Elem<T>::to_f32(raw[j]) : -INFINITY;
      }
    }
    if (apply_softmax) {
      CT m = -INFINITY;
#pragma unroll
      for (int j = 0; j < EPQ; ++j) m = ct_max(m, v[j]);
#pragma unroll
      for (int o = 1; o < GQ_LPT; o <<= 1) m = ct_max(m, __shfl_xor(m, o, 64));
      CT s = 0;
#pragma unroll
      for (int j = 0; j < EPQ; ++j) {
        int e = q * EPQ + j;
        v[j] = (e < E) ? ct_exp(v[j] - m) : CT(0);
        s += v[j];
      }
#pragma unroll
      for (int o = 1; o < GQ_LPT; o <<= 1) s += __shfl_xor(s, o, 64);
#pragma unroll
      for (int j = 0; j < EPQ; ++j) {
        int e = q * EPQ + j;
        if (e < E) {
          T r = Elem<T>::from_f32(v[j] / s);
          v[j] = Elem<T>::to_f32(r);
          if (scores_out && live) scores_out[(size_t)t * E + e] = r;
        } else {
          v[j] = -INFINITY;
        }
      }
    }
    uint32_t nanm = 0;
#pragma unroll
    for (int j = 0; j < EPQ; ++j) {
      int e = q * EPQ + j;
      if (e < E) s_sc[tl * ES + e] = live ? (float)v[j] : 0.f;
      if (v[j] != v[j]) { v[j] = -INFINITY; nanm |= 1u << j; }
    }

    uint32_t taken = 0;
    CT myg = 0, prev = 0;
    int myidx = 0;
    bool tied = false;
    const int rounds = tie_mode ? k + 1 : k;
    for (int c = 0; c < rounds; ++c) {
      CT bv = -INFINITY;
      int be = 0x7fffffff;
#pragma unroll
      for (int j = 0; j < EPQ; ++j) {
        int e = q * EPQ + j;
        bool ok = (e < E) && !((taken >> j) & 1u);
        if (ok && (v[j] > bv || (v[j] == bv && e < be))) { bv = v[j]; be = e; }
      }
#pragma unroll
      for (int o = 1; o < GQ_LPT; o <<= 1) {
        CT ov = __shfl_xor(bv, o, 64);
        int oe = __shfl_xor(be, o, 64);
        if (ov > bv || (ov == bv && oe < be)) { bv = ov; be = oe; }
      }
      if (c > 0 && bv == prev && be != 0x7fffffff) tied = true;
      prev = bv;
      if (c < k) {
        if (be / EPQ == q) taken |= 1u << (be - q * EPQ);
        if (c == q) { myg = bv; myidx = be; }
        if (q == 0 && live) {
          idx[(size_t)c * Tn + t] = be;
          if (idx8 != nullptr) idx8[(size_t)c * Tn + t] = (uint8_t)be;
        }
      }
    }
    if (tie_mode) {
      const int rowsh = (int)(threadIdx.x & 48);
      if ((__ballot(nanm != 0) >> rowsh) & 0xffffull) tied = true;
      if (tied && live) {
#pragma unroll
        for (int j = 0; j < EPQ; ++j) {
          int e = q * EPQ + j;
          if (e < E) s_tv[tl * E + e] = ((nanm >> j) & 1u) ? (CT)NAN : v[j];
        }
        if (q == 0) s_list[atomicAdd(&s_nlist[pass & 1], 1)] = tl;
      }
    }
    {
      const int row0 = (int)(threadIdx.x & 48);
      CT denom = __shfl(myg, row0, 64);
      for (int c = 1; c < k; ++c) denom = round_to<T>(denom + __shfl(myg, row0 + c, 64));
      if (q < k && live && !(tie_mode && tied)) {
        CT g = myg;
        if (normalize && k > 1) {
          CT d = ct_max(denom, (CT)Elem<T>::eps());
          if (denom != denom) d = denom;
          g = g / d;
        }
        gates[(size_t)q * Tn + t] = Elem<T>::from_f32(g);
        atomicAdd(&s_hist[q * E + myidx], 1);
      }
    }
    __syncthreads();
    if (tid < E) {
      float s = colsum;
      for (int r = 0; r < 64; ++r) s += s_sc[r * ES + tid];
      colsum = s;
    }
    if (tie_mode) {
      const int wv = (int)(threadIdx.x >> 6), nbusy = (E + 63) >> 6, wl = (int)(threadIdx.x & 63);
      constexpr int SL = (GQ_LPT * EPQ + 63) / 64;
      const int nrep = s_nlist[pass & 1];
      for (int ent = wv - nbusy; ent >= 0 && ent < nrep; ent += GQ_THREADS / 64 - nbusy) {
        const int trow = s_list[ent], tt = ts + trow;
        using Rep = typename TkRepOf<T>::type;
        WaveQueue<SL, Rep> wq;
        wq.sel = s_sel;
        wq.seln = E;
#pragma unroll
        for (int sl = 0; sl < SL; ++sl) {
          const int e = wl + 64 * sl;
          wq.r[sl] = Rep::make(e < E ? s_tv[trow * E + e] : (CT)0, e);
        }
        AtenTopk<WaveQueue<SL, Rep>> tk(wq);
        tk.run(E, k);
        TkElem<CT> res;
        res.id = Rep::id_of(wq.r[0].unpack());
        res.v = s_tv[trow * E + (wl < k ? res.id : 0)];
        CT denom = tk_readlane(res.v, 0);
        for (int c = 1; c < k; ++c) denom = round_to<T>(denom + tk_readlane(res.v, c));
        if (wl < k) {
          CT g = res.v;
          if (normalize && k > 1) {
            CT d = ct_max(denom, (CT)Elem<T>::eps());
            if (denom != denom) d = denom;
            g = g / d;
          }
          gates[(size_t)wl * Tn + tt] = Elem<T>::from_f32(g);
          idx[(size_t)wl * Tn + tt] = res.id;
          if (idx8 != nullptr) idx8[(size_t)wl * Tn + tt] = (uint8_t)res.id;
          atomicAdd(&s_hist[wl * E + res.id], 1);
        }
      }
      if (tid == 0) s_nlist[(pass + 1) & 1] = 0;
    }
    __syncthreads();
  }
  for (int i = tid; i < k * E; i += GQ_THREADS) ws_hist[(size_t)b * k * E + i] = s_hist[i];
  if (tid < E) ws_colsum[(size_t)b * E + tid] = colsum;
}

__global__ __launch_bounds__(256) void slot_map_kernel(const int32_t *__restrict__ idx,
                                                       const int32_t *__restrict__ loc, int n,
                                                       int E, int capacity,
                                                       int32_t *__restrict__ slot_map) {
  int q = blockIdx.x * 256 + threadIdx.x;
  if (q >= n) return;
  int e = idx[q], l = loc[q];
  if (e >= 0 && e < E && l >= 0 && l < capacity) slot_map[(size_t)e * capacity + l] = q;
}

#define CS_WAVES 16
__global__ __launch_bounds__(CS_WAVES * 64) void cumsum_kernel(const int32_t *__restrict__ in,
                                                              int32_t *__restrict__ out, int Tn,
                                                              int E) {
  __shared__ int32_t s_part[CS_WAVES][64];
  const int lane = threadIdx.x & 63, wid = threadIdx.x >> 6;
  const int col = blockIdx.x * 64 + lane;
  const int rows_per = (Tn + CS_WAVES - 1) / CS_WAVES;
  const int r0 = wid * rows_per, r1 = min(Tn, r0 + rows_per);
  int acc = 0;
  if (col < E)
    for (int r = r0; r < r1; ++r) acc += in[(size_t)r * E + col];
  s_part[wid][lane] = acc;
  __syncthreads();
  int run = -1;
  for (int w = 0; w < wid; ++w) run += s_part[w][lane];
  if (col < E)
    for (int r = r0; r < r1; ++r) {
      run += in[(size_t)r * E + col];
      out[(size_t)r * E + col] = run;
    }
}

template <typename T>
static int launch_gate_topk(const void *in, int apply_softmax, int Tn, int E, int k, int normalize,
                            void *scores_out, int32_t *idx, void *gates, void *ws,
                            int32_t *clear_map, int clear_n, hipStream_t st, const float *part = nullptr, int nsplit = 0,
                            void *logits_out = nullptr, uint8_t *idx8 = nullptr) {
  const int tile = rt_tile(Tn), nt = rt_ntiles(Tn);
  int32_t *ws_hist = (int32_t *)ws;
  float *ws_col = (float *)(ws_hist + (size_t)nt * k * E);
  using CTh = typename Elem<T>::ct;
  int tie_mode = tutel_get_option(TUTEL_OPT_TIE_RULE) != 0;
  size_t lds = (size_t)k * E * 4 + 8;
  {
    const size_t col = (size_t)GT_WAVES * (E < GT_COL_SLAB ? E : GT_COL_SLAB) * 4, slot = (size_t)E * (sizeof(CTh) + 2);
    const size_t room = (size_t)160 * 1024 - lds - 256;
    int slots = (int)(room / slot);
    if (slots > GT_WAVES) slots = GT_WAVES;
    if (slots < 1) tie_mode = 0;
    const size_t tie = tie_mode ? (size_t)slots * slot : 0;
    lds += tie > col ? tie : col;
    if (tie_mode && E > 128) tie_mode = slots;
  }
  if (E <= 128) {
    const int epq = (E + GQ_LPT - 1) / GQ_LPT;
    const int epq_t = epq <= 1 ? 1 : (epq <= 2 ? 2 : (epq <= 4 ? 4 : 8));
    const size_t lds_q = ((size_t)k * E + (size_t)64 * (GQ_LPT * epq_t + 1)) * 4 + 8 + (tie_mode ? (size_t)64 * E * sizeof(CTh) + 16 * 256 : 0);
#define GQ_LAUNCH(EPQ)                                                                         \
    do {                                                                                       \
      if (lds_q > 65536) {                                                                     \
        (void)hipFuncSetAttribute((const void *)gate_topk_quad_kernel<T, EPQ>, hipFuncAttributeMaxDynamicSharedMemorySize, (int)lds_q); \
        (void)hipGetLastError();                                                               \
      }                                                                                        \
      hipLaunchKernelGGL((gate_topk_quad_kernel<T, EPQ>), dim3(nt), dim3(GQ_THREADS), lds_q, st,            \
                         (const T *)in, apply_softmax, Tn, E, k, normalize, tile, (T *)scores_out,          \
                         idx, (T *)gates, ws_hist, ws_col, clear_map, clear_n, part, nsplit, (T *)logits_out, idx8, tie_mode); \
    } while (0)
    if (epq_t == 1) GQ_LAUNCH(1);
    else if (epq_t == 2) GQ_LAUNCH(2);
    else if (epq_t == 4) GQ_LAUNCH(4);
    else GQ_LAUNCH(8);
#undef GQ_LAUNCH
    TUTEL_CHECK_LAUNCH("tutel_amd_gate_topk");
    return 0;
  }
  TUTEL_REQUIRE(part == nullptr && idx8 == nullptr, "tutel_amd_gate_topk_partials: E = %d is past the 128 experts the partial-sum form covers", E);
  const int epl = (E + 63) / 64;
#define GT_LAUNCH(EPL)                                                                          \
  do {                                                                                          \
    if (lds > 65536) {                                                                          \
      (void)hipFuncSetAttribute((const void *)gate_topk_kernel<T, EPL, (EPL <= 4 ? 4 : (EPL <= 8 ? 2 : 1))>,                         \
                                hipFuncAttributeMaxDynamicSharedMemorySize, (int)lds);          \
      (void)hipGetLastError();                                                                  \
    }                                                                                           \
    hipLaunchKernelGGL((gate_topk_kernel<T, EPL, (EPL <= 4 ? 4 : (EPL <= 8 ? 2 : 1))>), dim3(nt), dim3(GT_THREADS), lds, st,         \
                       (const T *)in, apply_softmax, Tn, E, k, normalize, tile,                 \
                       (T *)scores_out, idx, (T *)gates, ws_hist, ws_col, clear_map, clear_n, tie_mode);  \
  } while (0)
  if (epl <= 1) GT_LAUNCH(1);
  else if (epl <= 2) GT_LAUNCH(2);
  else if (epl <= 4) GT_LAUNCH(4);
  else if (epl <= 8) GT_LAUNCH(8);
  else if (epl <= 16) GT_LAUNCH(16);
  else if (epl <= 32) GT_LAUNCH(32);
  else GT_LAUNCH(64);
#undef GT_LAUNCH
  TUTEL_CHECK_LAUNCH("tutel_amd_gate_topk");
  return 0;
}

extern "C" int tutel_amd_gate_topk(const void *in, int dtype, int apply_softmax, int T, int E,
                                   int k, int normalize_gate, void *scores_out, int32_t *idx,
                                   void *gates, void *ws, size_t ws_bytes, int32_t *clear_map,
                                   int clear_n, tutel_stream_t stream) {
  TUTEL_REQUIRE(dtype_ok(dtype) || dtype == TUTEL_F64, "tutel_amd_gate_topk: unsupported dtype %d", dtype);
  TUTEL_REQUIRE(T >= 0 && E >= 1 && E <= RT_MAX_E, "tutel_amd_gate_topk: need 1 <= E <= %d (got %d)", RT_MAX_E, E);
  TUTEL_REQUIRE(k >= 1 && k <= RT_MAX_K && k <= E, "tutel_amd_gate_topk: need 1 <= k <= min(E,%d) (got k=%d, E=%d)", RT_MAX_K, k, E);
  TUTEL_REQUIRE((size_t)k * E <= 8192, "tutel_amd_gate_topk: k*E = %d exceeds 8192", k * E);
  if (T == 0) return 0;
  TUTEL_REQUIRE(in && idx && gates && ws, "tutel_amd_gate_topk: null pointer");
  TUTEL_REQUIRE(ws_bytes >= tutel_amd_routing_workspace_bytes(T, E, k), "tutel_amd_gate_topk: workspace too small");
  TUTEL_REQUIRE(clear_n >= 0 && (clear_map != nullptr || clear_n == 0), "tutel_amd_gate_topk: bad clear_map");
  if (clear_n == 0) clear_map = nullptr;
  hipStream_t st = (hipStream_t)stream;
  StageScope stage(TUTEL_STAGE_GATE_TOPK, st);
  if (dtype == TUTEL_F64) return launch_gate_topk<double>(in, apply_softmax, T, E, k, normalize_gate, scores_out, idx, gates, ws, clear_map, clear_n, st);
  if (dtype == TUTEL_F32) return launch_gate_topk<float>(in, apply_softmax, T, E, k, normalize_gate, scores_out, idx, gates, ws, clear_map, clear_n, st);
  if (dtype == TUTEL_BF16) return launch_gate_topk<bf16_t>(in, apply_softmax, T, E, k, normalize_gate, scores_out, idx, gates, ws, clear_map, clear_n, st);
  return launch_gate_topk<f16_t>(in, apply_softmax, T, E, k, normalize_gate, scores_out, idx, gates, ws, clear_map, clear_n, st);
}

void tutel_route_finish_args(int T, int E, int k, void *ws, RouteFinish *out) {
  const int nt = rt_ntiles(T);
  out->Tn = T; out->E = E; out->k = k; out->ntiles = nt;
  out->ws_hist = (const int32_t *)ws;
  out->ws_colsum = (const float *)((const int32_t *)ws + (size_t)nt * k * E);
}

int tutel_gate_topk_launch(const void *in, const float *partials, int splits, int dtype, int T, int E, int k, int normalize_gate,
                           void *logits_out, int32_t *idx, void *gates, void *ws, int32_t *clear_map, int clear_n, uint8_t *idx8,
                           hipStream_t st) {
  TUTEL_REQUIRE(E <= 128 || (partials == nullptr && idx8 == nullptr), "tutel_gate_topk_launch: E = %d is past the 16-lanes-per-token kernel", E);
  if (clear_n == 0) clear_map = nullptr;
  StageScope stage(TUTEL_STAGE_GATE_TOPK, st);
  const int sm = 1;
  if (dtype == TUTEL_F32) return launch_gate_topk<float>(in, sm, T, E, k, normalize_gate, nullptr, idx, gates, ws, clear_map, clear_n, st, partials, splits, logits_out, idx8);
  if (dtype == TUTEL_BF16) return launch_gate_topk<bf16_t>(in, sm, T, E, k, normalize_gate, nullptr, idx, gates, ws, clear_map, clear_n, st, partials, splits, logits_out, idx8);
  return launch_gate_topk<f16_t>(in, sm, T, E, k, normalize_gate, nullptr, idx, gates, ws, clear_map, clear_n, st, partials, splits, logits_out, idx8);
}

extern "C" int tutel_amd_gate_topk_partials(const float *partials, int splits, int dtype, int T, int E, int k,
                                            int normalize_gate, void *logits_out, void *scores_out, int32_t *idx,
                                            void *gates, void *ws, size_t ws_bytes, int32_t *clear_map, int clear_n,
                                            tutel_stream_t stream) {
  TUTEL_REQUIRE(dtype == TUTEL_F16 || dtype == TUTEL_BF16, "tutel_amd_gate_topk_partials: the logits dtype must be fp16 / bf16 (got %d)", dtype);
  TUTEL_REQUIRE(T >= 0 && E >= 1 && E <= 128, "tutel_amd_gate_topk_partials: need 1 <= E <= 128 (got %d)", E);
  TUTEL_REQUIRE(k >= 1 && k <= RT_MAX_K && k <= E, "tutel_amd_gate_topk_partials: need 1 <= k <= min(E,%d) (got k=%d, E=%d)", RT_MAX_K, k, E);
  TUTEL_REQUIRE(splits >= 1 && splits <= 64, "tutel_amd_gate_topk_partials: bad split count %d", splits);
  if (T == 0) return 0;
  TUTEL_REQUIRE(partials && idx && gates && ws, "tutel_amd_gate_topk_partials: null pointer");
  TUTEL_REQUIRE(ws_bytes >= tutel_amd_routing_workspace_bytes(T, E, k), "tutel_amd_gate_topk_partials: workspace too small");
  TUTEL_REQUIRE(clear_n >= 0 && (clear_map != nullptr || clear_n == 0), "tutel_amd_gate_topk_partials: bad clear_map");
  if (clear_n == 0) clear_map = nullptr;
  hipStream_t st = (hipStream_t)stream;
  StageScope stage(TUTEL_STAGE_GATE_TOPK, st);
  if (dtype == TUTEL_BF16)
    return launch_gate_topk<bf16_t>(nullptr, 1, T, E, k, normalize_gate, scores_out, idx, gates, ws, clear_map, clear_n, st, partials, splits, logits_out);
  return launch_gate_topk<f16_t>(nullptr, 1, T, E, k, normalize_gate, scores_out, idx, gates, ws, clear_map, clear_n, st, partials, splits, logits_out);
}

extern "C" int tutel_amd_compute_location(const int32_t *idx, int T, int E, int k, int hist_ready,
                                          void *ws, size_t ws_bytes, int32_t *loc,
                                          int32_t *dispatch_count, int32_t *stats, void *l_aux,
                                          int l_aux_dtype, int capacity, int32_t *slot_map,
                                          int slot_map_cleared, tutel_stream_t stream) {
  TUTEL_REQUIRE(T >= 0 && E >= 1 && E <= RT_MAX_E, "tutel_amd_compute_location: need 1 <= E <= %d (got %d)", RT_MAX_E, E);
  TUTEL_REQUIRE(k >= 1 && k <= RT_MAX_K, "tutel_amd_compute_location: need 1 <= k <= %d (got %d)", RT_MAX_K, k);
  TUTEL_REQUIRE((size_t)k * E <= 8192, "tutel_amd_compute_location: k*E = %d exceeds 8192", k * E);
  TUTEL_REQUIRE(dispatch_count != nullptr, "tutel_amd_compute_location: dispatch_count is null");
  TUTEL_REQUIRE(l_aux == nullptr || dtype_ok(l_aux_dtype), "tutel_amd_compute_location: bad l_aux dtype %d", l_aux_dtype);
  TUTEL_REQUIRE((long long)k * T < 0x7fffffffLL, "tutel_amd_compute_location: k*T overflows int32");
  TUTEL_REQUIRE(hist_ready || l_aux == nullptr, "tutel_amd_compute_location: l_aux needs the column sums written by tutel_amd_gate_topk (hist_ready=1)");
  hipStream_t st = (hipStream_t)stream;
  if (T == 0) {
    (void)hipMemsetAsync(dispatch_count, 0, (size_t)E * 4, st);
    if (stats) (void)hipMemsetAsync(stats, 0, 4, st);
    if (l_aux) (void)hipMemsetAsync(l_aux, 0, dtype_size(l_aux_dtype), st);
    if (slot_map && capacity > 0) (void)hipMemsetAsync(slot_map, 0xFF, (size_t)E * capacity * 4, st);
    return 0;
  }
  TUTEL_REQUIRE(idx && loc && ws, "tutel_amd_compute_location: null pointer");
  TUTEL_REQUIRE(ws_bytes >= tutel_amd_routing_workspace_bytes(T, E, k), "tutel_amd_compute_location: workspace too small");
  const int tile = rt_tile(T), nt = rt_ntiles(T);
  int32_t *ws_hist = (int32_t *)ws;
  float *ws_col = (float *)(ws_hist + (size_t)nt * k * E);
  StageScope stage(TUTEL_STAGE_LOCATION, st);
  if (!hist_ready) {
    hipLaunchKernelGGL(tile_hist_kernel, dim3(nt), dim3(RT_THREADS), (size_t)k * E * 4, st, idx, T, E, k, tile, ws_hist);
    TUTEL_CHECK_LAUNCH("tutel_amd_compute_location(hist)");
  }
  if (slot_map != nullptr && capacity > 0) {
    if (!slot_map_cleared) {
      hipError_t e = hipMemsetAsync(slot_map, 0xFF, (size_t)E * capacity * 4, st);
      TUTEL_REQUIRE(e == hipSuccess, "tutel_amd_compute_location: memset failed: %s", hipGetErrorString(e));
    }
  } else {
    slot_map = nullptr;
    capacity = 0;
  }
  const size_t lds_loc = ((size_t)2 * k * E + (size_t)(E > RT_THREADS ? E : RT_THREADS)) * 4;
  if (lds_loc > 65536) {
    (void)hipFuncSetAttribute((const void *)location_kernel, hipFuncAttributeMaxDynamicSharedMemorySize, (int)lds_loc);
    (void)hipGetLastError();
  }
  hipLaunchKernelGGL(location_kernel, dim3(nt), dim3(RT_THREADS), lds_loc, st, idx, T, E, k,
                     tile, nt, ws_hist, ws_col, loc, dispatch_count, stats, l_aux, l_aux_dtype, capacity, slot_map);
  TUTEL_CHECK_LAUNCH("tutel_amd_compute_location");
  return 0;
}

extern "C" int tutel_amd_slot_map(const int32_t *idx, const int32_t *loc, int T, int E, int k,
                                  int capacity, int32_t *slot_map, tutel_stream_t stream) {
  TUTEL_REQUIRE(E >= 1 && k >= 1 && capacity >= 0 && T >= 0, "tutel_amd_slot_map: bad sizes");
  TUTEL_REQUIRE((long long)k * T < 0x7fffffffLL, "tutel_amd_slot_map: k*T overflows int32");
  hipStream_t st = (hipStream_t)stream;
  if (capacity == 0) return 0;
  TUTEL_REQUIRE(slot_map != nullptr, "tutel_amd_slot_map: null slot_map");
  StageScope stage(TUTEL_STAGE_OTHER, st);
  hipError_t e = hipMemsetAsync(slot_map, 0xFF, (size_t)E * capacity * 4, st);
  TUTEL_REQUIRE(e == hipSuccess, "tutel_amd_slot_map: memset failed: %s", hipGetErrorString(e));
  int n = k * T;
  if (n == 0) return 0;
  TUTEL_REQUIRE(idx && loc, "tutel_amd_slot_map: null pointer");
  hipLaunchKernelGGL(slot_map_kernel, dim3((n + 255) / 256), dim3(256), 0, st, idx, loc, n, E, capacity, slot_map);
  TUTEL_CHECK_LAUNCH("tutel_amd_slot_map");
  return 0;
}

extern "C" int tutel_amd_cumsum_sub_one(const int32_t *mask, int32_t *out, int T, int E,
                                        tutel_stream_t stream) {
  TUTEL_REQUIRE(T >= 0 && E >= 0, "tutel_amd_cumsum_sub_one: bad sizes");
  if (T == 0 || E == 0) return 0;
  TUTEL_REQUIRE(mask && out, "tutel_amd_cumsum_sub_one: null pointer");
  hipLaunchKernelGGL(cumsum_kernel, dim3((E + 63) / 64), dim3(CS_WAVES * 64), 0, (hipStream_t)stream, mask, out, T, E);
  TUTEL_CHECK_LAUNCH("tutel_amd_cumsum_sub_one");
  return 0;
}
```

### tutel_amd/ops.py

```python
import torch

from . import _lib

_DT = {torch.float32: _lib.F32, torch.float16: _lib.F16, torch.bfloat16: _lib.BF16}
ACT_CODES = {"none": _lib.ACT_NONE, "relu": _lib.ACT_RELU, "gelu": _lib.ACT_GELU, "silu": _lib.ACT_SILU}


def _code(t):
    try:
        return _DT[t.dtype]
    except KeyError:
        raise _lib.TutelAmdError(f"tutel_amd: dtype {t.dtype} is not supported by the HIP kernels") from None


def _dev(*tensors):
    for t in tensors:
        if t is not None and not t.is_cuda:
            raise _lib.TutelAmdError(
                "tutel_amd: the MoE hot path runs on the HIP device only (got a CPU tensor); "
                "there is no CPU fallback.")


def _ptr(t):
    return None if t is None else t.data_ptr()


def _a16(t):
    if t is None or t.data_ptr() % 16 == 0:
        return t
    return t.clone(memory_format=torch.contiguous_format)


_raw_stream = getattr(torch._C, "_cuda_getCurrentRawStream", None)


def _stream():
    if _raw_stream is not None:
        return _raw_stream(torch.cuda.current_device())
    return torch.cuda.current_stream().cuda_stream


def supported_dtype(dtype):
    return dtype in _DT


def routing_dtype(dtype):
    return dtype in _DT or dtype == torch.float64


def routing_workspace(T, E, k, device):
    n = _lib.lib().tutel_amd_routing_workspace_bytes(T, E, k)
    return torch.empty([max(int(n), 4)], dtype=torch.uint8, device=device)


def gate_topk(inp, k, apply_softmax=False, normalize_gate=True, want_scores=False, ws=None, clear=None):
    _dev(inp)
    assert inp.dim() == 2
    inp = inp.contiguous()
    T, E = inp.shape
    k = min(int(k), E)
    idx = torch.empty([k, T], dtype=torch.int32, device=inp.device)
    gates = torch.empty([k, T], dtype=inp.dtype, device=inp.device)
    scores = torch.empty_like(inp) if (want_scores and apply_softmax) else None
    if ws is None:
        ws = routing_workspace(T, E, k, inp.device)
    L = _lib.lib()
    code = _lib.F64 if inp.dtype == torch.float64 else _code(inp)
    _lib.check(L.tutel_amd_gate_topk(_ptr(inp), code, int(bool(apply_softmax)), T, E, k,
                                     int(bool(normalize_gate)), _ptr(scores), _ptr(idx), _ptr(gates),
                                     _ptr(ws), ws.numel(), _ptr(clear), clear.numel() if clear is not None else 0,
                                     _stream()), "tutel_amd_gate_topk")
    return idx, gates, ws, (scores if apply_softmax else inp)


def gate_proj_splits(T, M, E, dtype):
    if dtype not in (torch.bfloat16, torch.float16):
        return 0
    return int(_lib.lib().tutel_amd_gate_proj_splits(int(T), int(M), int(E), _lib.BF16 if dtype == torch.bfloat16 else _lib.F16))


def gate_proj(x, wg, partials=None):
    _dev(x)
    assert x.dim() == 2 and wg.dim() == 2 and x.shape[1] == wg.shape[1] and x.dtype == wg.dtype
    T, M = x.shape
    E = wg.shape[0]
    S = gate_proj_splits(T, M, E, x.dtype)
    if S == 0 or T == 0:
        return None
    x, wg = x.contiguous(), wg.contiguous()
    if partials is None:
        partials = torch.empty([S, T, E], dtype=torch.float32, device=x.device)
    assert partials.numel() >= S * T * E and partials.dtype == torch.float32
    _lib.check(_lib.lib().tutel_amd_gate_proj(_ptr(x), _ptr(wg), _code(x), T, M, E, _ptr(partials), partials.numel() * 4, _stream()),
               "tutel_amd_gate_proj")
    return partials


def gate_topk_partials(partials, dtype, k, normalize_gate=True, want_logits=False, want_scores=False, ws=None, clear=None):
    _dev(partials)
    assert partials.dim() == 3 and partials.dtype == torch.float32 and partials.is_contiguous()
    S, T, E = partials.shape
    k = min(int(k), E)
    dev = partials.device
    idx = torch.empty([k, T], dtype=torch.int32, device=dev)
    gates = torch.empty([k, T], dtype=dtype, device=dev)
    logits = torch.empty([T, E], dtype=dtype, device=dev) if want_logits else None
    scores = torch.empty([T, E], dtype=dtype, device=dev) if want_scores else None
    if ws is None:
        ws = routing_workspace(T, E, k, dev)
    code = _lib.BF16 if dtype == torch.bfloat16 else _lib.F16
    _lib.check(_lib.lib().tutel_amd_gate_topk_partials(_ptr(partials), S, code, T, E, k, int(bool(normalize_gate)), _ptr(logits),
                                                       _ptr(scores), _ptr(idx), _ptr(gates), _ptr(ws), ws.numel(), _ptr(clear),
                                                       clear.numel() if clear is not None else 0, _stream()),
               "tutel_amd_gate_topk_partials")
    return idx, gates, ws, logits, scores


def gate_logits(x, wg):
    part = gate_proj(x, wg)
    if part is None:
        return None
    return gate_topk_partials(part, x.dtype, 1, want_logits=True)[3]


def cache_warm(t, chunk_bytes=None, n_chunks=1, stride_bytes=0, blocks=0, offset=0):
    _dev(t)
    total = t.numel() * t.element_size()
    chunk_bytes = total - offset if chunk_bytes is None else int(chunk_bytes)
    assert offset + (n_chunks - 1) * stride_bytes + chunk_bytes <= total
    _lib.check(_lib.lib().tutel_amd_cache_warm(t.data_ptr() + offset, chunk_bytes, int(n_chunks), int(stride_bytes), int(blocks), None, _stream()),
               "tutel_amd_cache_warm")


def compute_location(idx, E, ws=None, capacity=0, want_l_aux=False, l_aux_dtype=torch.float32, cleared_slot_map=None):
    _dev(idx)
    assert idx.dtype == torch.int32 and idx.dim() == 2 and idx.is_contiguous()
    k, T = idx.shape
    dev = idx.device
    hist_ready = ws is not None
    if ws is None:
        ws = routing_workspace(T, E, k, dev)
    loc = torch.empty_like(idx)
    cnt = torch.empty([E], dtype=torch.int32, device=dev)
    stats = torch.empty([1], dtype=torch.int32, device=dev)
    l_aux = torch.empty([1], dtype=l_aux_dtype, device=dev) if (want_l_aux and hist_ready) else None
    smap = None
    if capacity > 0:
        if cleared_slot_map is not None:
            assert cleared_slot_map.numel() == E * capacity and cleared_slot_map.dtype == torch.int32
            smap = cleared_slot_map
        else:
            smap = torch.empty([E * capacity], dtype=torch.int32, device=dev)
    L = _lib.lib()
    _lib.check(L.tutel_amd_compute_location(_ptr(idx), T, E, k, int(hist_ready), _ptr(ws), ws.numel(),
                                            _ptr(loc), _ptr(cnt), _ptr(stats), _ptr(l_aux),
                                            _code(l_aux) if l_aux is not None else 0,
                                            int(capacity), _ptr(smap), int(cleared_slot_map is not None), _stream()),
               "tutel_amd_compute_location")
    return loc, cnt, stats, l_aux, smap


def slot_map(idx, loc, E, capacity):
    _dev(idx, loc)
    assert idx.dtype == torch.int32 and loc.dtype == torch.int32
    assert idx.is_contiguous() and loc.is_contiguous() and idx.shape == loc.shape
    k, T = idx.shape
    smap = torch.empty([E * capacity], dtype=torch.int32, device=idx.device)
    _lib.check(_lib.lib().tutel_amd_slot_map(_ptr(idx), _ptr(loc), T, E, k, int(capacity), _ptr(smap),
                                             _stream()), "tutel_amd_slot_map")
    return smap


def cumsum_sub_one(mask):
    _dev(mask)
    m = mask.to(torch.int32).contiguous()
    out = torch.empty_like(m)
    _lib.check(_lib.lib().tutel_amd_cumsum_sub_one(_ptr(m), _ptr(out), m.shape[0], m.shape[1], _stream()),
               "tutel_amd_cumsum_sub_one")
    return out


def fast_encode(x, smap, gates, n_slots, capacity=0, num_experts=0, chunk_rows=0, expert_slice=0, ep_world=1):
    _dev(x, smap, gates)
    assert x.dim() == 2 and x.is_contiguous() and smap.dtype == torch.int32 and smap.numel() == n_slots
    x = _a16(x)
    T, M = x.shape
    out = torch.empty([n_slots, M], dtype=x.dtype, device=x.device)
    if gates is not None:
        assert gates.is_contiguous()
    _lib.check(_lib.lib().tutel_amd_fast_encode(_ptr(x), _code(x), _ptr(smap), _ptr(gates),
                                                _code(gates) if gates is not None else 0, T, M,
                                                int(n_slots), int(capacity), int(num_experts), int(chunk_rows),
                                                int(expert_slice), int(ep_world), _ptr(out), _stream()),
               "tutel_amd_fast_encode")
    return out


def fast_decode(buf, idx, loc, gates, capacity, num_experts=0, chunk_rows=0, expert_slice=0, ep_world=1):
    _dev(buf, idx, loc, gates)
    assert buf.dim() == 2 and buf.is_contiguous()
    buf = _a16(buf)
    assert idx.dtype == torch.int32 and loc.dtype == torch.int32 and idx.is_contiguous() and loc.is_contiguous()
    k, T = idx.shape
    M = buf.shape[1]
    out = torch.empty([T, M], dtype=buf.dtype, device=buf.device)
    if gates is not None:
        assert gates.is_contiguous() and gates.shape == idx.shape
    _lib.check(_lib.lib().tutel_amd_fast_decode(_ptr(buf), _code(buf), _ptr(idx), _ptr(loc), _ptr(gates),
                                                _code(gates) if gates is not None else 0, T, M, k,
                                                int(capacity), int(num_experts), int(chunk_rows), int(expert_slice), int(ep_world),
                                                _ptr(out), _stream()),
               "tutel_amd_fast_decode")
    return out


def gate_grad(x, buf, idx, loc, capacity):
    _dev(x, buf, idx, loc)
    assert x.is_contiguous() and buf.is_contiguous() and x.dtype == buf.dtype
    x, buf = _a16(x), _a16(buf)
    k, T = idx.shape
    M = x.shape[1]
    out = torch.empty([k, T], dtype=torch.float32, device=x.device)
    _lib.check(_lib.lib().tutel_amd_gate_grad(_ptr(x), _ptr(buf), _code(x), _ptr(idx), _ptr(loc), T, M, k,
                                              int(capacity), _ptr(out), _stream()), "tutel_amd_gate_grad")
    return out


def gemm_supported(dtype, N, K):
    return dtype in (torch.bfloat16, torch.float16) and K % 64 == 0 and N % 8 == 0


def expert_gemm(a, w, bias, w_kmajor, act="none", E_loc=None, R=None, a_layout=None, out=None,
                d_layout=None, row_counts=None, row_align=1, mul=None):
    _dev(a, w, bias, out, row_counts, mul)
    assert w.dim() == 3 and w.is_contiguous()
    if w_kmajor:
        El, N, K = w.shape
    else:
        El, K, N = w.shape
    E_loc = El if E_loc is None else E_loc
    if a_layout is None:
        assert a.dim() == 3 and a.is_contiguous() and a.shape[0] == E_loc and a.shape[2] == K
        a = _a16(a)
        R = a.shape[1]
        a_layout = (R * K, 0, R, K)
    assert R is not None
    if out is None:
        out = torch.empty([E_loc, R, N], dtype=a.dtype, device=a.device)
        d_layout = (R * N, 0, R, N)
    assert d_layout is not None
    if bias is not None:
        assert bias.is_contiguous() and bias.shape[-1] == N and bias.dtype == a.dtype
    assert w.dtype == a.dtype
    if mul is not None:
        assert mul.dtype == a.dtype and mul.is_contiguous()
        _lib.check(_lib.lib().tutel_amd_expert_gemm_glu(
            _ptr(a), a_layout[0], a_layout[1], a_layout[2], a_layout[3],
            _ptr(w), int(bool(w_kmajor)), w.stride(0), w.stride(1),
            _ptr(bias), (bias.stride(0) if bias is not None else 0), _ptr(mul),
            _ptr(out), d_layout[0], d_layout[1], d_layout[2], d_layout[3],
            E_loc, R, N, K, _code(a), ACT_CODES[act],
            _ptr(row_counts), int(row_align), _stream()), "tutel_amd_expert_gemm_glu")
        return out
    _lib.check(_lib.lib().tutel_amd_expert_gemm(
        _ptr(a), a_layout[0], a_layout[1], a_layout[2], a_layout[3],
        _ptr(w), int(bool(w_kmajor)), w.stride(0), w.stride(1),
        _ptr(bias), (bias.stride(0) if bias is not None else 0),
        _ptr(out), d_layout[0], d_layout[1], d_layout[2], d_layout[3],
        E_loc, R, N, K, _code(a), ACT_CODES[act],
        _ptr(row_counts), int(row_align), _stream()), "tutel_amd_expert_gemm")
    return out


def expert_gemm_gate_up(a, w_gate, w_up, act="silu", row_counts=None, row_align=1):
    _dev(a, w_gate, w_up, row_counts)
    assert a.dim() == 3 and a.is_contiguous() and w_gate.dim() == 3 and w_gate.is_contiguous()
    assert w_up.shape == w_gate.shape and w_up.is_contiguous() and w_gate.dtype == a.dtype and w_up.dtype == a.dtype
    E, N, K = w_gate.shape
    assert a.shape[0] == E and a.shape[2] == K
    a = _a16(a)
    R = a.shape[1]
    out = torch.empty([E, R, N], dtype=a.dtype, device=a.device)
    _lib.check(_lib.lib().tutel_amd_expert_gemm_gate_up(
        _ptr(a), R * K, 0, R, K, _ptr(w_gate), _ptr(w_up), w_gate.stride(0), w_gate.stride(1),
        _ptr(out), R * N, 0, R, N, E, R, N, K, _code(a), ACT_CODES[act],
        _ptr(row_counts), int(row_align), _stream()), "tutel_amd_expert_gemm_gate_up")
    return out


_zero_rows = {}


def expert_gemm_gather(x, smap, w, bias, w_kmajor, act, R, row_counts=None, row_align=1):
    _dev(x, smap, w, bias, row_counts)
    assert x.dim() == 2 and x.is_contiguous() and w.dim() == 3 and w.is_contiguous() and w.dtype == x.dtype
    E_loc, N, K = (w.shape if w_kmajor else (w.shape[0], w.shape[2], w.shape[1]))
    assert x.shape[1] == K and smap.dtype == torch.int32 and smap.numel() == E_loc * R
    x = _a16(x)
    key = (x.device, x.dtype)
    z = _zero_rows.get(key)
    if z is None or z.numel() < K:
        z = _zero_rows[key] = torch.zeros([max(K, 8192)], dtype=x.dtype, device=x.device)
    out = torch.empty([E_loc, R, N], dtype=x.dtype, device=x.device)
    _lib.check(_lib.lib().tutel_amd_expert_gemm_gather(
        _ptr(x), x.stride(0), _ptr(smap), x.shape[0], _ptr(z), _ptr(w), int(bool(w_kmajor)), w.stride(0), w.stride(1),
        _ptr(bias), (bias.stride(0) if bias is not None else 0), _ptr(out), R * N, N, E_loc, R, N, K, _code(x),
        ACT_CODES[act], _ptr(row_counts), int(row_align), _stream()), "tutel_amd_expert_gemm_gather")
    return out


def expert_ffn(x, w1, b1, w2_kmajor, b2, act, R=None, smap=None, hid=None):
    _dev(x, w1, b1, w2_kmajor, b2, smap)
    assert w1.dim() == 3 and w2_kmajor.dim() == 3 and w1.is_contiguous() and w2_kmajor.is_contiguous() and w1.dtype == x.dtype == w2_kmajor.dtype
    E_loc, H, M = w1.shape
    M_out = w2_kmajor.shape[1]
    assert w2_kmajor.shape == (E_loc, M_out, H) and x.is_contiguous()
    x = _a16(x)
    if smap is None:
        assert x.dim() == 3 and x.shape[0] == E_loc and x.shape[2] == M
        R = x.shape[1]
        xs, ldx, T, z = R * M, M, 0, None
    else:
        assert x.dim() == 2 and x.shape[1] == M and smap.dtype == torch.int32 and smap.numel() == E_loc * R
        key = (x.device, x.dtype)
        z = _zero_rows.get(key)
        if z is None or z.numel() < M:
            z = _zero_rows[key] = torch.zeros([max(M, 8192)], dtype=x.dtype, device=x.device)
        xs, ldx, T = 0, x.stride(0), x.shape[0]
    if hid is None:
        hid = torch.empty([E_loc, R, H], dtype=x.dtype, device=x.device)
    out = torch.empty([E_loc, R, M_out], dtype=x.dtype, device=x.device)
    rc = _lib.lib().tutel_amd_expert_ffn(_ptr(x), xs, ldx, _ptr(smap), T, _ptr(z), _ptr(w1), w1.stride(0), w1.stride(1), _ptr(b1),
                                         (b1.stride(0) if b1 is not None else 0), _ptr(hid), R * H, H, _ptr(w2_kmajor), w2_kmajor.stride(0),
                                         w2_kmajor.stride(1), _ptr(b2), (b2.stride(0) if b2 is not None else 0), _ptr(out), R * M_out, M_out,
                                         E_loc, R, M, H, M_out, _code(x), ACT_CODES[act], _stream())
    if rc == _lib.ENOTSUP:
        return None
    _lib.check(rc, "tutel_amd_expert_ffn")
    return out


_OPT_ENV = {_lib.OPT_GEMM_IMPL: "TUTEL_AMD_GEMM_IMPL", _lib.OPT_GEMM_TILE: "TUTEL_AMD_GEMM_BIG", _lib.OPT_DECODE: "TUTEL_AMD_DECODE",
            _lib.OPT_EP_STAGE_GRID: "TUTEL_AMD_EP_STAGE_GRID", _lib.OPT_GEMM_PERSIST: "TUTEL_AMD_GEMM_PERSIST", _lib.OPT_EP_STREAMS: "TUTEL_AMD_EP_STREAMS",
            _lib.OPT_EP_CANARY: "TUTEL_AMD_EP_CANARY", _lib.OPT_GEMM_SPLITK: "TUTEL_AMD_GEMM_SPLITK", _lib.OPT_GEMM_STORE: "TUTEL_AMD_GEMM_STORE",
            _lib.OPT_GEMM_GATHER: "TUTEL_AMD_GEMM_GATHER", _lib.OPT_FUSED_LOCATION: "TUTEL_AMD_FUSED_LOCATION", _lib.OPT_TIE_RULE: "TUTEL_AMD_TIE_RULE", _lib.OPT_FFN_FUSED: "TUTEL_AMD_FFN_FUSED"}
_opts = {}


class PackedLayout:

    def __init__(self, E, rows_bound, tiles_bound, row_limit, device):
        self.E, self.rows_bound, self.tiles_bound, self.row_limit = int(E), int(rows_bound), int(tiles_bound), int(row_limit)
        self.offsets = torch.empty([E + 1], dtype=torch.int32, device=device)
        self.tiles = torch.empty([2 * max(tiles_bound, 1)], dtype=torch.int32, device=device)
        self.ntiles = torch.empty([1], dtype=torch.int32, device=device)
        self.capacity = torch.empty([1], dtype=torch.int32, device=device)
        self.slot_map = torch.empty([max(rows_bound, 1)], dtype=torch.int32, device=device)

    @property
    def decode_limit(self):
        return self.row_limit if self.row_limit > 0 else 0x7fffffff


def packed_layout(dispatch_count, idx, loc, capacity_limit, alignment, rows_bound, tiles_bound, row_limit, out=None):
    _dev(dispatch_count, idx, loc)
    k, T = idx.shape
    E = dispatch_count.numel()
    lay = out if out is not None else PackedLayout(E, rows_bound, tiles_bound, row_limit, idx.device)
    _lib.check(_lib.lib().tutel_amd_packed_layout(_ptr(dispatch_count), _ptr(idx), _ptr(loc), T, E, k, int(capacity_limit), int(alignment),
                                                  lay.rows_bound, lay.tiles_bound, _ptr(lay.offsets), _ptr(lay.tiles), _ptr(lay.ntiles),
                                                  _ptr(lay.capacity), _ptr(lay.slot_map), _stream()), "tutel_amd_packed_layout")
    return lay


def expert_gemm_packed(a, w, bias, w_kmajor, layout, act="none", gather=None, zero_row=None, mul=None, out=None):
    _dev(a, w, bias, mul)
    assert a.dim() == 2 and a.is_contiguous() and w.dim() == 3 and w.is_contiguous() and w.dtype == a.dtype
    E, N, K = (w.shape[0], w.shape[1], w.shape[2]) if w_kmajor else (w.shape[0], w.shape[2], w.shape[1])
    assert a.shape[1] == K and E == layout.E
    if bias is not None:
        assert bias.is_contiguous() and bias.shape[-1] == N and bias.dtype == a.dtype
    if mul is not None:
        assert mul.shape == (layout.rows_bound, N) and mul.is_contiguous() and mul.dtype == a.dtype
    a = _a16(a)
    if out is None:
        out = torch.empty([layout.rows_bound, N], dtype=a.dtype, device=a.device)
    else:
        _dev(out)
        assert out.shape == (layout.rows_bound, N) and out.is_contiguous() and out.dtype == a.dtype
    _lib.check(_lib.lib().tutel_amd_expert_gemm_packed(
        _ptr(a), K, _ptr(layout.slot_map) if gather else None, a.shape[0] if gather else 0, _ptr(zero_row) if gather else None,
        _ptr(w), int(bool(w_kmajor)), w.stride(0), w.stride(1), _ptr(bias), (bias.stride(0) if bias is not None else 0), _ptr(mul),
        _ptr(out), N, E, layout.rows_bound, N, K, _code(a), ACT_CODES[act], _ptr(layout.offsets), _ptr(layout.tiles), _ptr(layout.ntiles),
        _ptr(layout.capacity), layout.tiles_bound, _stream()), "tutel_amd_expert_gemm_packed")
    return out


def expert_wgrad_packed(a, b, layout, gather=None, zero_row=None):
    _dev(a, b)
    assert a.dim() == 2 and b.dim() == 2 and a.is_contiguous() and b.is_contiguous() and a.dtype == b.dtype
    assert gather in (None, "a", "b")
    a, b = _a16(a), _a16(b)
    Na, Nb = a.shape[1], b.shape[1]
    g = {None: 0, "a": 1, "b": 2}[gather]
    T = (a if gather == "a" else b).shape[0] if gather else 0
    out = torch.empty([layout.E, Na, Nb], dtype=a.dtype, device=a.device)
    _lib.check(_lib.lib().tutel_amd_expert_wgrad_packed(
        _ptr(a), Na, _ptr(b), Nb, _ptr(layout.slot_map) if g else None, g, T, _ptr(zero_row) if g else None,
        _ptr(out), layout.E, layout.rows_bound, Na, Nb, _code(a), _ptr(layout.offsets), _stream()), "tutel_amd_expert_wgrad_packed")
    return out


def expert_bgrad_packed(b, layout):
    _dev(b)
    assert b.dim() == 2 and b.is_contiguous()
    out = torch.empty([layout.E, b.shape[1]], dtype=b.dtype, device=b.device)
    _lib.check(_lib.lib().tutel_amd_expert_bgrad_packed(_ptr(b), b.shape[1], _ptr(out), layout.E, b.shape[1], _code(b), _ptr(layout.offsets),
                                                        _stream()), "tutel_amd_expert_bgrad_packed")
# ... 77 lines not shown
```

Baseline: 16.86 million.

## Fuse gate projection and top-k routing into a single kernel

Adds a fused route kernel that computes the gate projection with MFMA and performs softmax/top-k selection in the same launch, replacing the separate gate_proj plus gate_topk_partials kernels when supported. The aim is to cut one kernel launch and the round trip of fp32 partials through global memory. The shared selection logic is factored into a header so both paths reuse it. The fused path falls back to the old two-kernel route on ENOTSUP, and may have lower parallelism for the projection than the split-K version.

```diff
diff --git a/include/tutel_amd.h b/include/tutel_amd.h
--- a/include/tutel_amd.h
+++ b/include/tutel_amd.h
@@ -31,6 +31,12 @@
 int tutel_amd_gate_topk_partials(const float *partials, int splits, int dtype, int T, int E, int k,
                                  int normalize_gate, void *logits_out, void *scores_out, int32_t *idx, void *gates,
                                  void *ws, size_t ws_bytes, int32_t *clear_map, int clear_n, tutel_stream_t stream);
+
+size_t tutel_amd_route_fused_scratch_bytes(int T, int M, int E, int k, int dtype);
+int tutel_amd_route_fused(const void *x, const void *wg, int dtype, int T, int M, int E, int k, int normalize_gate, void *logits_out,
+                          int32_t *idx, uint8_t *idx8, void *gates, void *ws, size_t ws_bytes, int32_t *clear_map, int clear_n,
+                          void *scratch, size_t scratch_bytes, tutel_stream_t stream);
+int tutel_amd_set_route_fused(int value);
 
 int tutel_amd_cache_warm(const void *p, size_t chunk_bytes, int n_chunks, size_t stride_bytes, int blocks, void *sink4,
                          tutel_stream_t stream);
@@ -235,7 +241,7 @@
 enum {
   TUTEL_STAGE_GATE_TOPK = 0, TUTEL_STAGE_LOCATION = 1, TUTEL_STAGE_ENCODE = 2, TUTEL_STAGE_FC1 = 3, TUTEL_STAGE_FC2 = 4,
   TUTEL_STAGE_DECODE = 5, TUTEL_STAGE_A2A_DISPATCH = 6, TUTEL_STAGE_A2A_COMBINE = 7, TUTEL_STAGE_OTHER = 8, TUTEL_STAGE_GATE_PROJ = 9,
-  TUTEL_STAGE_COUNT = 10
+  TUTEL_STAGE_ROUTE_FUSED = 10, TUTEL_STAGE_COUNT = 11
 };
 int tutel_amd_stage_timing(int enable);
 int tutel_amd_stage_report(double *total_us, int *counts, int n_stages );
diff --git a/tutel_amd/_lib.py b/tutel_amd/_lib.py
--- a/tutel_amd/_lib.py
+++ b/tutel_amd/_lib.py
@@ -21,6 +21,9 @@
     "tutel_amd_gate_proj_splits": (_i, [_i, _i, _i, _i]),
     "tutel_amd_gate_proj": (_i, [_vp, _vp, _i, _i, _i, _i, _vp, _sz, _vp]),
     "tutel_amd_gate_topk_partials": (_i, [_vp, _i, _i, _i, _i, _i, _i, _vp, _vp, _vp, _vp, _vp, _sz, _vp, _i, _vp]),
+    "tutel_amd_route_fused_scratch_bytes": (_sz, [_i, _i, _i, _i, _i]),
+    "tutel_amd_route_fused": (_i, [_vp, _vp, _i, _i, _i, _i, _i, _i, _vp, _vp, _vp, _vp, _vp, _sz, _vp, _i, _vp, _sz, _vp]),
+    "tutel_amd_set_route_fused": (_i, [_i]),
     "tutel_amd_cache_warm": (_i, [_vp, _sz, _i, _sz, _i, _vp, _vp]),
     "tutel_amd_compute_location": (_i, [_vp, _i, _i, _i, _i, _vp, _sz, _vp, _vp, _vp, _vp, _i, _i, _vp, _i, _vp]),
     "tutel_amd_slot_map": (_i, [_vp, _vp, _i, _i, _i, _i, _vp, _vp]),
@@ -124,7 +127,7 @@
 IPC_HANDLE_BYTES = 64
 EAGAIN, ENOTSUP = 1000, 1001
 STAGES = ("gate_topk", "location", "fast_encode", "expert_fc1", "expert_fc2", "fast_decode", "all_to_all_dispatch", "all_to_all_combine", "other",
-          "gate_projection")
+          "gate_projection", "route_fused")
 
 _lib = None
 
diff --git a/tutel_amd/csrc/api.hip b/tutel_amd/csrc/api.hip
--- a/tutel_amd/csrc/api.hip
+++ b/tutel_amd/csrc/api.hip
@@ -60,7 +60,8 @@
 extern "C" int tutel_amd_range_pop(void) { return g_roctx_push ? g_roctx_pop() : 0; }
 static const char *const g_stage_names[TUTEL_STAGE_COUNT] = {
     "tutel_amd.gate_topk", "tutel_amd.compute_location", "tutel_amd.fast_encode", "tutel_amd.expert_fc1", "tutel_amd.expert_fc2",
-    "tutel_amd.fast_decode", "tutel_amd.all_to_all_dispatch", "tutel_amd.all_to_all_combine", "tutel_amd.other", "tutel_amd.gate_projection"};
+    "tutel_amd.fast_decode", "tutel_amd.all_to_all_dispatch", "tutel_amd.all_to_all_combine", "tutel_amd.other", "tutel_amd.gate_projection",
+    "tutel_amd.route_fused"};
 void tutel_stage_range_push(int stage) {
   roctx_init();
   if (g_stage_hint >= 0) stage = g_stage_hint;
diff --git a/tutel_amd/csrc/common.h b/tutel_amd/csrc/common.h
--- a/tutel_amd/csrc/common.h
+++ b/tutel_amd/csrc/common.h
@@ -81,6 +81,11 @@
                            void *logits_out, int32_t *idx, void *gates, void *ws, int32_t *clear_map, int clear_n, uint8_t *idx8,
                            hipStream_t st);
 
+int tutel_route_fused_launch(const void *x, const void *wg, int dtype, int T, int M, int E, int k, int normalize_gate, void *logits_out,
+                             int32_t *idx, void *gates, void *ws, int32_t *clear_map, int clear_n, uint8_t *idx8, void *scratch,
+                             size_t scratch_bytes, const char **why, hipStream_t st);
+int tutel_gate_proj_plan(int T, int M, int E, int dtype, int *np);
+
 #define TUTEL_REQUIRE(cond, ...)           \
   do {                                     \
     if (!(cond)) {                         \
diff --git a/tutel_amd/csrc/ep.hip b/tutel_amd/csrc/ep.hip
--- a/tutel_amd/csrc/ep.hip
+++ b/tutel_amd/csrc/ep.hip
@@ -949,13 +949,19 @@
   if (fl) {
     hipStream_t st = (hipStream_t)stream;
     uint8_t *idx8 = (uint8_t *)m->fl_ws;
-    if (project) {
-      rc = tutel_amd_gate_proj(a.x, m->gate_w, a.dtype, T, a.M, E, m->gate_partials, m->gate_partial_bytes, stream);
-      if (rc) return rc;
-    }
-    rc = tutel_gate_topk_launch(project ? nullptr : m->logits, project ? m->gate_partials : nullptr, splits, m->logits_dtype, T, E, k,
-                                m->normalize_gate, project ? m->logits_out : nullptr, const_cast<int32_t *>(a.idx), const_cast<void *>(a.gates),
-                                m->ws, nullptr, 0, idx8, st);
+    rc = TUTEL_AMD_ENOTSUP;
+    if (project)
+      rc = tutel_route_fused_launch(a.x, m->gate_w, a.dtype, T, a.M, E, k, m->normalize_gate, m->logits_out, const_cast<int32_t *>(a.idx),
+                                    const_cast<void *>(a.gates), m->ws, nullptr, 0, idx8, m->gate_partials, m->gate_partial_bytes, nullptr, st);
+    if (rc == TUTEL_AMD_ENOTSUP) {
+      if (project) {
+        rc = tutel_amd_gate_proj(a.x, m->gate_w, a.dtype, T, a.M, E, m->gate_partials, m->gate_partial_bytes, stream);
+        if (rc) return rc;
+      }
+      rc = tutel_gate_topk_launch(project ? nullptr : m->logits, project ? m->gate_partials : nullptr, splits, m->logits_dtype, T, E, k,
+                                  m->normalize_gate, project ? m->logits_out : nullptr, const_cast<int32_t *>(a.idx), const_cast<void *>(a.gates),
+                                  m->ws, nullptr, 0, idx8, st);
+    }
     if (rc) return rc;
     if (m->capacity_out != nullptr) *m->capacity_out = a.capacity;
     rc = TUTEL_AMD_ENOTSUP;
@@ -988,11 +994,18 @@
     return tutel_decode_finish_launch(a.send, a.dtype, a.idx, a.loc, a.gates, m->logits_dtype, T, Mo, k, a.capacity, E, a.y, fin, st);
   }
   if (project && T > 0) {
-    rc = tutel_amd_gate_proj(a.x, m->gate_w, a.dtype, T, a.M, E, m->gate_partials, m->gate_partial_bytes, stream);
-    if (rc) return rc;
-    rc = tutel_amd_gate_topk_partials(m->gate_partials, splits, a.dtype, T, E, k, m->normalize_gate, m->logits_out, nullptr,
-                                      const_cast<int32_t *>(a.idx), const_cast<void *>(a.gates), m->ws, m->ws_bytes,
-                                      dropless ? nullptr : smap, dropless ? 0 : E * a.capacity, stream);
+    rc = TUTEL_AMD_ENOTSUP;
+    if (k >= 1 && k <= E && m->ws_bytes >= tutel_amd_routing_workspace_bytes(T, E, k))
+      rc = tutel_route_fused_launch(a.x, m->gate_w, a.dtype, T, a.M, E, k, m->normalize_gate, m->logits_out, const_cast<int32_t *>(a.idx),
+                                    const_cast<void *>(a.gates), m->ws, dropless ? nullptr : smap, dropless ? 0 : E * a.capacity, nullptr,
+                                    m->gate_partials, m->gate_partial_bytes, nullptr, (hipStream_t)stream);
+    if (rc == TUTEL_AMD_ENOTSUP) {
+      rc = tutel_amd_gate_proj(a.x, m->gate_w, a.dtype, T, a.M, E, m->gate_partials, m->gate_partial_bytes, stream);
+      if (rc) return rc;
+      rc = tutel_amd_gate_topk_partials(m->gate_partials, splits, a.dtype, T, E, k, m->normalize_gate, m->logits_out, nullptr,
+                                        const_cast<int32_t *>(a.idx), const_cast<void *>(a.gates), m->ws, m->ws_bytes,
+                                        dropless ? nullptr : smap, dropless ? 0 : E * a.capacity, stream);
+    }
   } else {
     rc = tutel_amd_gate_topk(m->logits, m->logits_dtype, 1, T, E, k, m->normalize_gate, nullptr, const_cast<int32_t *>(a.idx),
                              const_cast<void *>(a.gates), m->ws, m->ws_bytes, dropless ? nullptr : smap, dropless ? 0 : E * a.capacity, stream);
diff --git a/tutel_amd/csrc/gate_dev.h b/tutel_amd/csrc/gate_dev.h
--- /dev/null
+++ b/tutel_amd/csrc/gate_dev.h
@@ -0,0 +1,172 @@
+#pragma once
+#include "common.h"
+#include "topk_ties.h"
+
+typedef __attribute__((ext_vector_type(16))) float gp_f32x16;
+typedef __attribute__((ext_vector_type(8))) __bf16 gp_bf16x8;
+typedef __attribute__((ext_vector_type(8))) _Float16 gp_f16x8;
+typedef __attribute__((ext_vector_type(4))) uint32_t gp_u32x4;
+typedef __attribute__((ext_vector_type(4))) float gp_f32x4;
+
+template <typename T> struct GpMma;
+template <> struct GpMma<bf16_t> {
+  __device__ static __forceinline__ gp_f32x16 run(gp_u32x4 a, gp_u32x4 b, gp_f32x16 c) {
+    return __builtin_amdgcn_mfma_f32_32x32x16_bf16(__builtin_bit_cast(gp_bf16x8, a), __builtin_bit_cast(gp_bf16x8, b), c, 0, 0, 0);
+  }
+};
+template <> struct GpMma<f16_t> {
+  __device__ static __forceinline__ gp_f32x16 run(gp_u32x4 a, gp_u32x4 b, gp_f32x16 c) {
+    return __builtin_amdgcn_mfma_f32_32x32x16_f16(__builtin_bit_cast(gp_f16x8, a), __builtin_bit_cast(gp_f16x8, b), c, 0, 0, 0);
+  }
+};
+
+__device__ __forceinline__ void gp_dma16(const uint16_t *g, uint16_t *l) {
+  __builtin_amdgcn_global_load_lds((const __attribute__((address_space(1))) void *)g, (__attribute__((address_space(3))) void *)l, 16, 0, 0);
+}
+
+#define GQ_LPT 16
+
+template <typename V, int N> struct alignas((sizeof(V) * N) > 16 ? 16 : (sizeof(V) * N)) GqPack { V v[N]; };
+template <typename V, int N> __device__ __forceinline__ void gq_load(const V *p, V (&o)[N]) {
+  const GqPack<V, N> pk = *reinterpret_cast<const GqPack<V, N> *>(p);
+#pragma unroll
+  for (int i = 0; i < N; ++i) o[i] = pk.v[i];
+}
+
+template <typename T, int EPQ>
+__device__ __forceinline__ void gq_select_row(typename Elem<T>::ct (&v)[EPQ], int apply_softmax, bool live, int t, int tl, int q, int Tn, int E,
+                                              int k, int normalize, int tie_mode, int ES, float *s_sc, typename Elem<T>::ct *s_tv, int *s_list,
+                                              int *s_nlist, T *__restrict__ scores_out, int32_t *__restrict__ idx, uint8_t *__restrict__ idx8,
+                                              T *__restrict__ gates, int32_t *s_hist) {
+  using CT = typename Elem<T>::ct;
+  if (apply_softmax) {
+    CT m = -INFINITY;
+#pragma unroll
+    for (int j = 0; j < EPQ; ++j) m = ct_max(m, v[j]);
+#pragma unroll
+    for (int o = 1; o < GQ_LPT; o <<= 1) m = ct_max(m, __shfl_xor(m, o, 64));
+    CT s = 0;
+#pragma unroll
+    for (int j = 0; j < EPQ; ++j) {
+      int e = q * EPQ + j;
+      v[j] = (e < E) ? ct_exp(v[j] - m) : CT(0);
+      s += v[j];
+    }
+#pragma unroll
+    for (int o = 1; o < GQ_LPT; o <<= 1) s += __shfl_xor(s, o, 64);
+#pragma unroll
+    for (int j = 0; j < EPQ; ++j) {
+      int e = q * EPQ + j;
+      if (e < E) {
+        T r = Elem<T>::from_f32(v[j] / s);
+        v[j] = Elem<T>::to_f32(r);
+        if (scores_out && live) scores_out[(size_t)t * E + e] = r;
+      } else {
+        v[j] = -INFINITY;
+      }
+    }
+  }
+  uint32_t nanm = 0;
+#pragma unroll
+  for (int j = 0; j < EPQ; ++j) {
+    int e = q * EPQ + j;
+    if (e < E) s_sc[tl * ES + e] = live ? (float)v[j] : 0.f;
+    if (v[j] != v[j]) { v[j] = -INFINITY; nanm |= 1u << j; }
+  }
+
+  uint32_t taken = 0;
+  CT myg = 0, prev = 0;
+  int myidx = 0;
+  bool tied = false;
+  const int rounds = tie_mode ? k + 1 : k;
+  for (int c = 0; c < rounds; ++c) {
+    CT bv = -INFINITY;
+    int be = 0x7fffffff;
+#pragma unroll
+    for (int j = 0; j < EPQ; ++j) {
+      int e = q * EPQ + j;
+      bool ok = (e < E) && !((taken >> j) & 1u);
+      if (ok && (v[j] > bv || (v[j] == bv && e < be))) { bv = v[j]; be = e; }
+    }
+#pragma unroll
+    for (int o = 1; o < GQ_LPT; o <<= 1) {
+      CT ov = __shfl_xor(bv, o, 64);
+      int oe = __shfl_xor(be, o, 64);
+      if (ov > bv || (ov == bv && oe < be)) { bv = ov; be = oe; }
+    }
+    if (c > 0 && bv == prev && be != 0x7fffffff) tied = true;
+    prev = bv;
+    if (c < k) {
+      if (be / EPQ == q) taken |= 1u << (be - q * EPQ);
+      if (c == q) { myg = bv; myidx = be; }
+      if (q == 0 && live) {
+        idx[(size_t)c * Tn + t] = be;
+        if (idx8 != nullptr) idx8[(size_t)c * Tn + t] = (uint8_t)be;
+      }
+    }
+  }
+  if (tie_mode) {
+    const int rowsh = (int)(threadIdx.x & 48);
+    if ((__ballot(nanm != 0) >> rowsh) & 0xffffull) tied = true;
+    if (tied && live) {
+#pragma unroll
+      for (int j = 0; j < EPQ; ++j) {
+        int e = q * EPQ + j;
+        if (e < E) s_tv[tl * E + e] = ((nanm >> j) & 1u) ? (CT)NAN : v[j];
+      }
+      if (q == 0) s_list[atomicAdd(s_nlist, 1)] = tl;
+    }
+  }
+  {
+    const int row0 = (int)(threadIdx.x & 48);
+    CT denom = __shfl(myg, row0, 64);
+    for (int c = 1; c < k; ++c) denom = round_to<T>(denom + __shfl(myg, row0 + c, 64));
+    if (q < k && live && !(tie_mode && tied)) {
+      CT g = myg;
+      if (normalize && k > 1) {
+        CT d = ct_max(denom, (CT)Elem<T>::eps());
+        if (denom != denom) d = denom;
+        g = g / d;
+      }
+      gates[(size_t)q * Tn + t] = Elem<T>::from_f32(g);
+      atomicAdd(&s_hist[q * E + myidx], 1);
+    }
+  }
+}
+
+template <typename T, int EPQ>
+__device__ __forceinline__ void gq_replay_row(int trow, int tt, int Tn, int E, int k, int normalize, const typename Elem<T>::ct *s_tv,
+                                              uint8_t *s_sel, int32_t *__restrict__ idx, uint8_t *__restrict__ idx8, T *__restrict__ gates,
+                                              int32_t *s_hist) {
+  using CT = typename Elem<T>::ct;
+  const int wl = (int)(threadIdx.x & 63);
+  constexpr int SL = (GQ_LPT * EPQ + 63) / 64;
+  using Rep = typename TkRepOf<T>::type;
+  WaveQueue<SL, Rep> wq;
+  wq.sel = s_sel;
+  wq.seln = E;
+#pragma unroll
+  for (int sl = 0; sl < SL; ++sl) {
+    const int e = wl + 64 * sl;
+    wq.r[sl] = Rep::make(e < E ? s_tv[trow * E + e] : (CT)0, e);
+  }
+  AtenTopk<WaveQueue<SL, Rep>> tk(wq);
+  tk.run(E, k);
+  TkElem<CT> res;
+  res.id = Rep::id_of(wq.r[0].unpack());
+  res.v = s_tv[trow * E + (wl < k ? res.id : 0)];
+  CT denom = tk_readlane(res.v, 0);
+  for (int c = 1; c < k; ++c) denom = round_to<T>(denom + tk_readlane(res.v, c));
+  if (wl < k) {
+    CT g = res.v;
+    if (normalize && k > 1) {
+      CT d = ct_max(denom, (CT)Elem<T>::eps());
+      if (denom != denom) d = denom;
+      g = g / d;
+    }
+    gates[(size_t)wl * Tn + tt] = Elem<T>::from_f32(g);
+    idx[(size_t)wl * Tn + tt] = res.id;
+    if (idx8 != nullptr) idx8[(size_t)wl * Tn + tt] = (uint8_t)res.id;
+    atomicAdd(&s_hist[wl * E + res.id], 1);
+  }
+}
diff --git a/tutel_amd/csrc/gate_proj.hip b/tutel_amd/csrc/gate_proj.hip
--- a/tutel_amd/csrc/gate_proj.hip
+++ b/tutel_amd/csrc/gate_proj.hip
@@ -1,30 +1,9 @@
 #include "common.h"
-
-typedef __attribute__((ext_vector_type(16))) float gp_f32x16;
-typedef __attribute__((ext_vector_type(8))) __bf16 gp_bf16x8;
-typedef __attribute__((ext_vector_type(8))) _Float16 gp_f16x8;
-typedef __attribute__((ext_vector_type(4))) uint32_t gp_u32x4;
-typedef __attribute__((ext_vector_type(4))) float gp_f32x4;
-
-template <typename T> struct GpMma;
-template <> struct GpMma<bf16_t> {
-  __device__ static __forceinline__ gp_f32x16 run(gp_u32x4 a, gp_u32x4 b, gp_f32x16 c) {
-    return __builtin_amdgcn_mfma_f32_32x32x16_bf16(__builtin_bit_cast(gp_bf16x8, a), __builtin_bit_cast(gp_bf16x8, b), c, 0, 0, 0);
-  }
-};
-template <> struct GpMma<f16_t> {
-  __device__ static __forceinline__ gp_f32x16 run(gp_u32x4 a, gp_u32x4 b, gp_f32x16 c) {
-    return __builtin_amdgcn_mfma_f32_32x32x16_f16(__builtin_bit_cast(gp_f16x8, a), __builtin_bit_cast(gp_f16x8, b), c, 0, 0, 0);
-  }
-};
+#include "gate_dev.h"
 
 #define GP_TM 64
 #define GP_THREADS 256
 #define GP_PANEL 4096
-
-__device__ __forceinline__ void gp_dma16(const uint16_t *g, uint16_t *l) {
-  __builtin_amdgcn_global_load_lds((const __attribute__((address_space(1))) void *)g, (__attribute__((address_space(3))) void *)l, 16, 0, 0);
-}
 
 template <typename T, int ER, int NP>
 __global__ __launch_bounds__(GP_THREADS) void gate_proj_kernel(const uint16_t *__restrict__ x, const uint16_t *__restrict__ wg,
@@ -155,6 +134,13 @@
   return true;
 }
 
+int tutel_gate_proj_plan(int T, int M, int E, int dtype, int *np) {
+  GpPlan pl;
+  if (!gp_plan(T, M, E, dtype, &pl)) return 0;
+  *np = pl.np;
+  return pl.splits;
+}
+
 extern "C" int tutel_amd_gate_proj_splits(int T, int M, int E, int dtype) {
   GpPlan pl;
   return gp_plan(T, M, E, dtype, &pl) ? pl.splits : 0;
diff --git a/tutel_amd/csrc/route_fused.hip b/tutel_amd/csrc/route_fused.hip
--- /dev/null
+++ b/tutel_amd/csrc/route_fused.hip
@@ -0,0 +1,350 @@
+#include <stdlib.h>
+
+#include <mutex>
+
+#include "common.h"
+#include "gate_dev.h"
+
+#define RF_TOK 16
+#define RF_THREADS 256
+#define RF_TILE 64
+#define RF_MAX_TILES 128
+#define RF_LDS_MAX (160 * 1024 - 512)
+
+__host__ __device__ constexpr int rf_vmcnt(int NP, int WOPS, int p) {
+  const int init = 2 * NP + 2 * WOPS;
+  const int need = p < 2 ? (p + 1) * (2 + WOPS) : init + (p - 1) * WOPS;
+  const int total = init + (p < NP - 2 ? p : NP - 2) * WOPS;
+  return total - need;
+}
+
+template <typename T, int EPQ, int NT, int NP>
+__global__ __launch_bounds__(RF_THREADS) void route_fused_kernel(const uint16_t *__restrict__ x, const uint16_t *__restrict__ wg, int Tn, int M,
+                                                                int E, int k, int normalize, int tie_mode, T *__restrict__ logits_out,
+                                                                int32_t *__restrict__ idx, uint8_t *__restrict__ idx8, T *__restrict__ gates,
+                                                                int32_t *__restrict__ ws_hist, float *__restrict__ ws_colsum,
+                                                                int32_t *__restrict__ clear_map, int clear_n, float *sc_g, int32_t *hist_g,
+                                                                uint32_t *ctr) {
+  using CT = typename Elem<T>::ct;
+  extern __shared__ __attribute__((aligned(16))) unsigned char smem[];
+  constexpr int ER = 32 * NT;
+  constexpr int WOPS = ER / 8;
+  constexpr int SLOT = ER * 64;
+  constexpr int RINGB = 2 * SLOT * 2;
+  constexpr int ES = GQ_LPT * EPQ + 1;
+  static_assert(16 * ES * 4 <= SLOT * 2 && 4 * 256 <= SLOT * 2, "the selection scratch must fit a ring slot");
+  __shared__ int s_nlist, s_ticket;
+  __shared__ int s_list[RF_TOK];
+
+  const int tid = threadIdx.x, lane = tid & 63;
+  const int wid = __builtin_amdgcn_readfirstlane(tid >> 6);
+  const int g = blockIdx.x, t0 = g * RF_TOK;
+  uint16_t *ring = reinterpret_cast<uint16_t *>(smem + (size_t)wid * RINGB);
+  uint16_t *sXw = reinterpret_cast<uint16_t *>(smem + (size_t)4 * RINGB) + (size_t)wid * NP * 1024;
+  const int kp0 = wid * NP;
+
+  if (clear_map != nullptr) {
+    const int per = (clear_n + (int)gridDim.x - 1) / (int)gridDim.x;
+    const int c0 = g * per, c1 = min(clear_n, c0 + per);
+    for (int i = c0 + tid; i < c1; i += RF_THREADS) clear_map[i] = -1;
+  }
+
+  const int rl = lane >> 3, cl = lane & 7;
+  const uint16_t *xp[2];
+  int woff[WOPS];
+#pragma unroll
+  for (int i = 0; i < 2; ++i) {
+    const int r = 8 * i + rl;
+    xp[i] = x + (size_t)min(t0 + r, Tn - 1) * M + (size_t)kp0 * 64 + (cl ^ ((r >> 1) & 7)) * 8;
+  }
+#pragma unroll
+  for (int i = 0; i < WOPS; ++i) {
+    const int r = 8 * i + rl;
+    woff[i] = min(r, E - 1) * M + kp0 * 64 + (cl ^ ((r >> 1) & 7)) * 8;
+  }
+#define RF_ISSUE_X(P)                                                                              \
+  do {                                                                                             \
+    _Pragma("unroll") for (int i = 0; i < 2; ++i) gp_dma16(xp[i] + (P) * 64, sXw + (P) * 1024 + i * 512); \
+  } while (0)
+#define RF_ISSUE_W(P)                                                                              \
+  do {                                                                                             \
+    _Pragma("unroll") for (int i = 0; i < WOPS; ++i) gp_dma16(wg + woff[i] + (P) * 64, ring + ((P) & 1) * SLOT + i * 512); \
+  } while (0)
+#pragma unroll
+  for (int p = 0; p < NP; ++p) {
+    RF_ISSUE_X(p);
+    if (p < 2) RF_ISSUE_W(p);
+  }
+
+  const int l31 = lane & 31, kg = lane >> 5;
+  const int sw = (l31 >> 1) & 7;
+  int frag_k[4];
+#pragma unroll
+  for (int kk = 0; kk < 4; ++kk) frag_k[kk] = (((kk * 2 + kg) ^ sw) << 3);
+  const int x_row = (l31 & 15) * 64;
+  const int w_row = l31 * 64;
+
+  gp_f32x16 acc[NT];
+#pragma unroll
+  for (int i = 0; i < NT; ++i)
+#pragma unroll
+    for (int r = 0; r < 16; ++r) acc[i][r] = 0.f;
+
+#pragma unroll
+  for (int p = 0; p < NP; ++p) {
+    asm volatile("s_waitcnt vmcnt(%0)" ::"n"(rf_vmcnt(NP, WOPS, p)) : "memory");
+    gp_u32x4 fa[4], fw[4][NT];
+    const uint16_t *cx = sXw + p * 1024 + x_row, *cw = ring + (p & 1) * SLOT + w_row;
+#pragma unroll
+    for (int kk = 0; kk < 4; ++kk) {
+      fa[kk] = *reinterpret_cast<const gp_u32x4 *>(cx + frag_k[kk]);
+#pragma unroll
+      for (int i = 0; i < NT; ++i) fw[kk][i] = *reinterpret_cast<const gp_u32x4 *>(cw + i * 32 * 64 + frag_k[kk]);
+    }
+    __builtin_amdgcn_sched_barrier(0);
+    if (p + 2 < NP) {
+      asm volatile("s_waitcnt lgkmcnt(0)" ::: "memory");
+      RF_ISSUE_W(p + 2);
+    }
+#pragma unroll
+    for (int kk = 0; kk < 4; ++kk)
+#pragma unroll
+      for (int i = 0; i < NT; ++i) acc[i] = GpMma<T>::run(fw[kk][i], fa[kk], acc[i]);
+    __builtin_amdgcn_sched_barrier(0);
+  }
+#undef RF_ISSUE_X
+#undef RF_ISSUE_W
+
+  if (l31 < RF_TOK) {
+    float *sp = reinterpret_cast<float *>(ring) + l31 * E;
+#pragma unroll
+    for (int i = 0; i < NT; ++i)
+#pragma unroll
+      for (int rg = 0; rg < 4; ++rg) {
+        const int n = i * 32 + rg * 8 + kg * 4;
+        if (n < E) {
+          gp_f32x4 v4 = {acc[i][rg * 4 + 0], acc[i][rg * 4 + 1], acc[i][rg * 4 + 2], acc[i][rg * 4 + 3]};
+          *reinterpret_cast<gp_f32x4 *>(sp + n) = v4;
+        }
+      }
+  }
+  __syncthreads();
+
+  float *s_sc = reinterpret_cast<float *>(smem + 0 * RINGB + SLOT * 2);
+  CT *s_tv = reinterpret_cast<CT *>(smem + 1 * RINGB + SLOT * 2);
+  int32_t *s_hist = reinterpret_cast<int32_t *>(smem + 2 * RINGB + SLOT * 2);
+  uint8_t *s_sel = smem + 3 * RINGB + SLOT * 2 + (size_t)wid * 256;
+  const int q = tid & (GQ_LPT - 1), tl = tid / GQ_LPT;
+  const int t = t0 + tl;
+  const bool live = t < Tn;
+  for (int i = tid; i < k * E; i += RF_THREADS) s_hist[i] = 0;
+  if (tid == 0) s_nlist = 0;
+  CT v[EPQ];
+  {
+    float a[EPQ];
+#pragma unroll
+    for (int s = 0; s < 4; ++s) {
+      const float *ps = reinterpret_cast<const float *>(smem + (size_t)s * RINGB) + tl * E;
+#pragma unroll
+      for (int j = 0; j < EPQ; ++j) {
+        const float bsj = ps[min(q * EPQ + j, E - 1)];
+        a[j] = (s == 0) ? bsj : a[j] + bsj;
+      }
+    }
+#pragma unroll
+    for (int j = 0; j < EPQ; ++j) {
+      const int e = q * EPQ + j;
+      const T r = Elem<T>::from_f32((CT)a[j]);
+      if (logits_out && live && e < E) logits_out[(size_t)t * E + e] = r;
+      v[j] = (e < E) ? Elem<T>::to_f32(r) : -INFINITY;
+    }
+  }
+  __syncthreads();
+  gq_select_row<T, EPQ>(v, 1, live, t, tl, q, Tn, E, k, normalize, tie_mode, ES, s_sc, s_tv, s_list, &s_nlist, nullptr, idx, idx8, gates, s_hist);
+  __syncthreads();
+  float *my_sc = sc_g + (size_t)g * RF_TOK * E;
+  for (int i = tid; i < RF_TOK * E; i += RF_THREADS) my_sc[i] = s_sc[(i / E) * ES + (i % E)];
+  if (tie_mode) {
+    const int nrep = s_nlist;
+    for (int ent = wid; ent < nrep; ent += RF_THREADS / 64) {
+      const int trow = s_list[ent];
+      gq_replay_row<T, EPQ>(trow, t0 + trow, Tn, E, k, normalize, s_tv, s_sel, idx, idx8, gates, s_hist);
+    }
+  }
+  __syncthreads();
+  int32_t *my_hist = hist_g + (size_t)g * k * E;
+  for (int i = tid; i < k * E; i += RF_THREADS) my_hist[i] = s_hist[i];
+
+  const int b = g / (RF_TILE / RF_TOK);
+  const int nsub = min(RF_TILE / RF_TOK, (min(Tn, (b + 1) * RF_TILE) - b * RF_TILE + RF_TOK - 1) / RF_TOK);
+  __builtin_amdgcn_fence(__ATOMIC_RELEASE, "agent");
+  __syncthreads();
+  if (tid == 0) s_ticket = (int)__hip_atomic_fetch_add(ctr + b, 1u, __ATOMIC_RELAXED, __HIP_MEMORY_SCOPE_AGENT);
+  __syncthreads();
+  if (s_ticket != nsub - 1) return;
+  if (tid == 0) __hip_atomic_store(ctr + b, 0u, __ATOMIC_RELAXED, __HIP_MEMORY_SCOPE_AGENT);
+  __builtin_amdgcn_fence(__ATOMIC_ACQUIRE, "agent");
+  const int g0 = b * (RF_TILE / RF_TOK);
+  for (int i = tid; i < k * E; i += RF_THREADS) {
+    int32_t s = 0;
+    for (int u = 0; u < nsub; ++u) s += hist_g[(size_t)(g0 + u) * k * E + i];
+    ws_hist[(size_t)b * k * E + i] = s;
+  }
+  if (tid < E) {
+    const float *col = sc_g + (size_t)g0 * RF_TOK * E + tid;
+    float s = 0.f;
+#pragma unroll 16
+    for (int r = 0; r < RF_TILE; ++r) s += (r / RF_TOK) < nsub ? col[(size_t)r * E] : 0.f;
+    ws_colsum[(size_t)b * E + tid] = s;
+  }
+}
+
+#define RF_SLOTS 256
+#define RF_DEVS 64
+static std::mutex g_rf_mu;
+static uint32_t *g_rf_pool[RF_DEVS];
+static const void *g_rf_key[RF_DEVS][RF_SLOTS];
+static int g_rf_n[RF_DEVS];
+static uint32_t *rf_counters(const void *key, hipStream_t st) {
+  int dev = 0;
+  if (hipGetDevice(&dev) != hipSuccess || dev < 0 || dev >= RF_DEVS) return nullptr;
+  std::lock_guard<std::mutex> lock(g_rf_mu);
+  if (g_rf_pool[dev] == nullptr) {
+    hipStreamCaptureStatus cs = hipStreamCaptureStatusNone;
+    if (hipStreamIsCapturing(st, &cs) != hipSuccess || cs != hipStreamCaptureStatusNone) return nullptr;
+    uint32_t *c = nullptr;
+    const size_t bytes = (size_t)RF_SLOTS * RF_MAX_TILES * sizeof(uint32_t);
+    if (hipMalloc((void **)&c, bytes) != hipSuccess || hipMemset(c, 0, bytes) != hipSuccess || hipDeviceSynchronize() != hipSuccess) {
+      (void)hipGetLastError();
+      if (c) (void)hipFree(c);
+      return nullptr;
+    }
+    g_rf_pool[dev] = c;
+  }
+  int slot = -1;
+  for (int i = 0; i < g_rf_n[dev]; ++i)
+    if (g_rf_key[dev][i] == key) slot = i;
+  if (slot < 0) {
+    if (g_rf_n[dev] >= RF_SLOTS) return nullptr;
+    slot = g_rf_n[dev]++;
+    g_rf_key[dev][slot] = key;
+  }
+  return g_rf_pool[dev] + (size_t)slot * RF_MAX_TILES;
+}
+
+int tutel_gate_proj_plan(int T, int M, int E, int dtype, int *np);
+struct RfPlan {
+  int np, nt, epq;
+  size_t lds;
+};
+static const char *rf_plan(int T, int M, int E, int k, int dtype, RfPlan *out) {
+  if (!(dtype == TUTEL_BF16 || dtype == TUTEL_F16)) return "needs a 16-bit gate";
+  if (T < 1 || T > RF_TILE * RF_MAX_TILES) return "needs 1 <= T <= 8192 (64-token tiles)";
+  if (E < 16 || E > 128 || (E & 15)) return "needs E <= 128, E % 16 == 0";
+  if (k < 1 || k > 16 || k > E) return "needs 1 <= k <= min(E, 16)";
+  if (M < 64 || (M & 63)) return "needs M % 64 == 0";
+  int np = 0;
+  const int S = tutel_gate_proj_plan(T, M, E, dtype, &np);
+  if (S != 4 || M / 64 != 4 * np) return "the gate projection's split count for this shape is not four whole K slices";
+  out->np = np;
+  out->nt = (E + 31) / 32;
+  const int epq = E / 16;
+  out->epq = epq <= 1 ? 1 : (epq <= 2 ? 2 : (epq <= 4 ? 4 : 8));
+  out->lds = (size_t)4 * 2 * (32 * out->nt) * 64 * 2 + (size_t)RF_TOK * M * 2;
+  if (out->lds > RF_LDS_MAX) return "the token slab and the weight rings do not fit in LDS";
+  return nullptr;
+}
+
+static int g_rf_mode = -2;
+static int rf_mode() {
+  if (g_rf_mode == -2) {
+    const char *s = getenv("TUTEL_AMD_ROUTE_FUSED");
+    g_rf_mode = s ? atoi(s) : -1;
+  }
+  return g_rf_mode;
+}
+extern "C" int tutel_amd_set_route_fused(int value) {
+  TUTEL_REQUIRE(value >= -1 && value <= 1, "tutel_amd_set_route_fused: value %d out of range", value);
+  g_rf_mode = value;
+  return 0;
+}
+
+extern "C" size_t tutel_amd_route_fused_scratch_bytes(int T, int M, int E, int k, int dtype) {
+  RfPlan pl;
+  if (rf_plan(T, M, E, k, dtype, &pl) != nullptr) return 0;
+  return (size_t)((T + RF_TOK - 1) / RF_TOK) * ((size_t)RF_TOK * E + (size_t)k * E) * 4;
+}
+
+template <typename T, int EPQ, int NT, int NP>
+static int rf_launch(const RfPlan &pl, const void *x, const void *wg, int Tn, int M, int E, int k, int normalize, void *logits_out, int32_t *idx,
+                     uint8_t *idx8, void *gates, int32_t *ws_hist, float *ws_col, int32_t *clear_map, int clear_n, float *sc_g, int32_t *hist_g,
+                     uint32_t *ctr, hipStream_t st) {
+  if (pl.lds > 65536) {
+    (void)hipFuncSetAttribute((const void *)route_fused_kernel<T, EPQ, NT, NP>, hipFuncAttributeMaxDynamicSharedMemorySize, (int)pl.lds);
+    (void)hipGetLastError();
+  }
+  const int tie_mode = tutel_get_option(TUTEL_OPT_TIE_RULE) != 0;
+  hipLaunchKernelGGL((route_fused_kernel<T, EPQ, NT, NP>), dim3((Tn + RF_TOK - 1) / RF_TOK), dim3(RF_THREADS), pl.lds, st, (const uint16_t *)x,
+                     (const uint16_t *)wg, Tn, M, E, k, normalize, tie_mode, (T *)logits_out, idx, idx8, (T *)gates, ws_hist, ws_col, clear_map,
+                     clear_n, sc_g, hist_g, ctr);
+  TUTEL_CHECK_LAUNCH("tutel_amd_route_fused");
+  return 0;
+}
+
+template <typename T, int EPQ, int NT, typename... A> static int rf_dispatch_np(const RfPlan &pl, A... a) {
+  if (pl.np == 8) return rf_launch<T, EPQ, NT, 8>(pl, a...);
+  if (pl.np == 4) return rf_launch<T, EPQ, NT, 4>(pl, a...);
+  return rf_launch<T, EPQ, NT, 2>(pl, a...);
+}
+template <typename T, typename... A> static int rf_dispatch(const RfPlan &pl, A... a) {
+  if (pl.epq == 1) return rf_dispatch_np<T, 1, 1>(pl, a...);
+  if (pl.epq == 2) return rf_dispatch_np<T, 2, 1>(pl, a...);
+  if (pl.epq == 4) return rf_dispatch_np<T, 4, 2>(pl, a...);
+  if (pl.nt == 3) return rf_dispatch_np<T, 8, 3>(pl, a...);
+  return rf_dispatch_np<T, 8, 4>(pl, a...);
+}
+
+int tutel_route_fused_launch(const void *x, const void *wg, int dtype, int T, int M, int E, int k, int normalize_gate, void *logits_out,
+                             int32_t *idx, void *gates, void *ws, int32_t *clear_map, int clear_n, uint8_t *idx8, void *scratch,
+                             size_t scratch_bytes, const char **why, hipStream_t st) {
+  const char *none = nullptr;
+  if (why == nullptr) why = &none;
+  RfPlan pl;
+  if (rf_mode() != 1) { *why = "not switched on (tutel_amd_set_route_fused(1) / TUTEL_AMD_ROUTE_FUSED=1)"; return TUTEL_AMD_ENOTSUP; }
+  if ((*why = rf_plan(T, M, E, k, dtype, &pl)) != nullptr) return TUTEL_AMD_ENOTSUP;
+  const size_t ngroups = (size_t)(T + RF_TOK - 1) / RF_TOK;
+  if (scratch == nullptr || ((uintptr_t)scratch & 15) != 0 || scratch_bytes < ngroups * ((size_t)RF_TOK * E + (size_t)k * E) * 4) {
+    *why = "scratch too small (tutel_amd_route_fused_scratch_bytes) or not 16-byte aligned";
+    return TUTEL_AMD_ENOTSUP;
+  }
+  if (((uintptr_t)x & 15) != 0 || ((uintptr_t)wg & 15) != 0) { *why = "x and wg must be 16-byte aligned"; return TUTEL_AMD_ENOTSUP; }
+  uint32_t *ctr = rf_counters(ws, st);
+  if (ctr == nullptr) { *why = "no tile counters (first call inside a stream capture, or more than 256 routing workspaces)"; return TUTEL_AMD_ENOTSUP; }
+  if (clear_n == 0) clear_map = nullptr;
+  const int nt = (T + RF_TILE - 1) / RF_TILE;
+  int32_t *ws_hist = (int32_t *)ws;
+  float *ws_col = (float *)(ws_hist + (size_t)nt * k * E);
+  float *sc_g = (float *)scratch;
+  int32_t *hist_g = (int32_t *)(sc_g + ngroups * RF_TOK * E);
+  StageScope stage(TUTEL_STAGE_ROUTE_FUSED, st);
+  if (dtype == TUTEL_BF16)
+    return rf_dispatch<bf16_t>(pl, x, wg, T, M, E, k, normalize_gate, logits_out, idx, idx8, gates, ws_hist, ws_col, clear_map, clear_n, sc_g, hist_g, ctr, st);
+  return rf_dispatch<f16_t>(pl, x, wg, T, M, E, k, normalize_gate, logits_out, idx, idx8, gates, ws_hist, ws_col, clear_map, clear_n, sc_g, hist_g, ctr, st);
+}
+
+extern "C" int tutel_amd_route_fused(const void *x, const void *wg, int dtype, int T, int M, int E, int k, int normalize_gate, void *logits_out,
+                                     int32_t *idx, uint8_t *idx8, void *gates, void *ws, size_t ws_bytes, int32_t *clear_map, int clear_n,
+                                     void *scratch, size_t scratch_bytes, tutel_stream_t stream) {
+  TUTEL_REQUIRE(T >= 0 && E >= 1 && k >= 1 && k <= E, "tutel_amd_route_fused: need T >= 0 and 1 <= k <= E (got T=%d, k=%d, E=%d)", T, k, E);
+  if (T == 0) return 0;
+  TUTEL_REQUIRE(x && wg && idx && gates && ws, "tutel_amd_route_fused: null pointer");
+  TUTEL_REQUIRE(ws_bytes >= tutel_amd_routing_workspace_bytes(T, E, k), "tutel_amd_route_fused: workspace too small");
+  TUTEL_REQUIRE(clear_n >= 0 && (clear_map != nullptr || clear_n == 0), "tutel_amd_route_fused: bad clear_map");
+  const char *why = nullptr;
+  const int rc = tutel_route_fused_launch(x, wg, dtype, T, M, E, k, normalize_gate, logits_out, idx, gates, ws, clear_map, clear_n, idx8, scratch,
+                                          scratch_bytes, &why, (hipStream_t)stream);
+  if (rc == TUTEL_AMD_ENOTSUP)
+    tutel_set_error("tutel_amd_route_fused: not taken (T=%d, M=%d, E=%d, k=%d, dtype=%d): %s -- use tutel_amd_gate_proj + tutel_amd_gate_topk_partials",
+                    T, M, E, k, dtype, why ? why : "?");
+  return rc;
+}
diff --git a/tutel_amd/csrc/routing.hip b/tutel_amd/csrc/routing.hip
--- a/tutel_amd/csrc/routing.hip
+++ b/tutel_amd/csrc/routing.hip
@@ -1,6 +1,7 @@
 #include "common.h"
 #include "routing_dev.h"
 #include "topk_ties.h"
+#include "gate_dev.h"
 
 #define GT_THREADS 1024
 #define GT_WAVES 16
@@ -343,15 +344,7 @@
   if (b == 0) loc_finish<RT_WAVES>(tid, Tn, E, k, ntiles, ws_colsum, s_tot, s_parts, s_red, s_redi, cs_first, cs_early, stats, l_aux, l_aux_dtype);
 }
 
-#define GQ_LPT 16
 #define GQ_THREADS 1024
-
-template <typename V, int N> struct alignas((sizeof(V) * N) > 16 ? 16 : (sizeof(V) * N)) GqPack { V v[N]; };
-template <typename V, int N> __device__ __forceinline__ void gq_load(const V *p, V (&o)[N]) {
-  const GqPack<V, N> pk = *reinterpret_cast<const GqPack<V, N> *>(p);
-#pragma unroll
-  for (int i = 0; i < N; ++i) o[i] = pk.v[i];
-}
 
 template <typename T, int EPQ>
 __global__ __launch_bounds__(GQ_THREADS) void gate_topk_quad_kernel(
@@ -439,99 +432,8 @@
         v[j] = (e < E) ? Elem<T>::to_f32(raw[j]) : -INFINITY;
       }
     }
-    if (apply_softmax) {
-      CT m = -INFINITY;
-#pragma unroll
-      for (int j = 0; j < EPQ; ++j) m = ct_max(m, v[j]);
-#pragma unroll
-      for (int o = 1; o < GQ_LPT; o <<= 1) m = ct_max(m, __shfl_xor(m, o, 64));
-      CT s = 0;
-#pragma unroll
-      for (int j = 0; j < EPQ; ++j) {
-        int e = q * EPQ + j;
-        v[j] = (e < E) ? ct_exp(v[j] - m) : CT(0);
-        s += v[j];
-      }
-#pragma unroll
-      for (int o = 1; o < GQ_LPT; o <<= 1) s += __shfl_xor(s, o, 64);
-#pragma unroll
-      for (int j = 0; j < EPQ; ++j) {
-        int e = q * EPQ + j;
-        if (e < E) {
-          T r = Elem<T>::from_f32(v[j] / s);
-          v[j] = Elem<T>::to_f32(r);
-          if (scores_out && live) scores_out[(size_t)t * E + e] = r;
-        } else {
-          v[j] = -INFINITY;
-        }
-      }
-    }
-    uint32_t nanm = 0;
-#pragma unroll
-    for (int j = 0; j < EPQ; ++j) {
-      int e = q * EPQ + j;
-      if (e < E) s_sc[tl * ES + e] = live ? (float)v[j] : 0.f;
-      if (v[j] != v[j]) { v[j] = -INFINITY; nanm |= 1u << j; }
-    }
-
-    uint32_t taken = 0;
-    CT myg = 0, prev = 0;
-    int myidx = 0;
-    bool tied = false;
-    const int rounds = tie_mode ? k + 1 : k;
-    for (int c = 0; c < rounds; ++c) {
-      CT bv = -INFINITY;
-      int be = 0x7fffffff;
-#pragma unroll
-      for (int j = 0; j < EPQ; ++j) {
-        int e = q * EPQ + j;
-        bool ok = (e < E) && !((taken >> j) & 1u);
-        if (ok && (v[j] > bv || (v[j] == bv && e < be))) { bv = v[j]; be = e; }
-      }
-#pragma unroll
-      for (int o = 1; o < GQ_LPT; o <<= 1) {
-        CT ov = __shfl_xor(bv, o, 64);
-        int oe = __shfl_xor(be, o, 64);
-        if (ov > bv || (ov == bv && oe < be)) { bv = ov; be = oe; }
-      }
-      if (c > 0 && bv == prev && be != 0x7fffffff) tied = true;
-      prev = bv;
-      if (c < k) {
-        if (be / EPQ == q) taken |= 1u << (be - q * EPQ);
-        if (c == q) { myg = bv; myidx = be; }
-        if (q == 0 && live) {
-          idx[(size_t)c * Tn + t] = be;
-          if (idx8 != nullptr) idx8[(size_t)c * Tn + t] = (uint8_t)be;
-        }
-      }
-    }
-    if (tie_mode) {
-      const int rowsh = (int)(threadIdx.x & 48);
-      if ((__ballot(nanm != 0) >> rowsh) & 0xffffull) tied = true;
-      if (tied && live) {
-#pragma unroll
-        for (int j = 0; j < EPQ; ++j) {
-          int e = q * EPQ + j;
-          if (e < E) s_tv[tl * E + e] = ((nanm >> j) & 1u) ? (CT)NAN : v[j];
-        }
-        if (q == 0) s_list[atomicAdd(&s_nlist[pass & 1], 1)] = tl;
-      }
-    }
-    {
-      const int row0 = (int)(threadIdx.x & 48);
-      CT denom = __shfl(myg, row0, 64);
-      for (int c = 1; c < k; ++c) denom = round_to<T>(denom + __shfl(myg, row0 + c, 64));
-      if (q < k && live && !(tie_mode && tied)) {
-        CT g = myg;
-        if (normalize && k > 1) {
-          CT d = ct_max(denom, (CT)Elem<T>::eps());
-          if (denom != denom) d = denom;
-          g = g / d;
-        }
-        gates[(size_t)q * Tn + t] = Elem<T>::from_f32(g);
-        atomicAdd(&s_hist[q * E + myidx], 1);
-      }
-    }
+    gq_select_row<T, EPQ>(v, apply_softmax, live, t, tl, q, Tn, E, k, normalize, tie_mode, ES, s_sc, s_tv, s_list, &s_nlist[pass & 1], scores_out,
+                          idx, idx8, gates, s_hist);
     __syncthreads();
     if (tid < E) {
       float s = colsum;
@@ -539,39 +441,11 @@
       colsum = s;
     }
     if (tie_mode) {
-      const int wv = (int)(threadIdx.x >> 6), nbusy = (E + 63) >> 6, wl = (int)(threadIdx.x & 63);
-      constexpr int SL = (GQ_LPT * EPQ + 63) / 64;
+      const int wv = (int)(threadIdx.x >> 6), nbusy = (E + 63) >> 6;
       const int nrep = s_nlist[pass & 1];
       for (int ent = wv - nbusy; ent >= 0 && ent < nrep; ent += GQ_THREADS / 64 - nbusy) {
-        const int trow = s_list[ent], tt = ts + trow;
-        using Rep = typename TkRepOf<T>::type;
-        WaveQueue<SL, Rep> wq;
-        wq.sel = s_sel;
-        wq.seln = E;
-#pragma unroll
-        for (int sl = 0; sl < SL; ++sl) {
-          const int e = wl + 64 * sl;
-          wq.r[sl] = Rep::make(e < E ? s_tv[trow * E + e] : (CT)0, e);
-        }
-        AtenTopk<WaveQueue<SL, Rep>> tk(wq);
-        tk.run(E, k);
-        TkElem<CT> res;
-        res.id = Rep::id_of(wq.r[0].unpack());
-        res.v = s_tv[trow * E + (wl < k ? res.id : 0)];
-        CT denom = tk_readlane(res.v, 0);
-        for (int c = 1; c < k; ++c) denom = round_to<T>(denom + tk_readlane(res.v, c));
-        if (wl < k) {
-          CT g = res.v;
-          if (normalize && k > 1) {
-            CT d = ct_max(denom, (CT)Elem<T>::eps());
-            if (denom != denom) d = denom;
-            g = g / d;
-          }
-          gates[(size_t)wl * Tn + tt] = Elem<T>::from_f32(g);
-          idx[(size_t)wl * Tn + tt] = res.id;
-          if (idx8 != nullptr) idx8[(size_t)wl * Tn + tt] = (uint8_t)res.id;
-          atomicAdd(&s_hist[wl * E + res.id], 1);
-        }
+        const int trow = s_list[ent];
+        gq_replay_row<T, EPQ>(trow, ts + trow, Tn, E, k, normalize, s_tv, s_sel, idx, idx8, gates, s_hist);
       }
       if (tid == 0) s_nlist[(pass + 1) & 1] = 0;
     }
diff --git a/tutel_amd/ops.py b/tutel_amd/ops.py
--- a/tutel_amd/ops.py
+++ b/tutel_amd/ops.py
@@ -114,6 +114,43 @@
                                                        clear.numel() if clear is not None else 0, _stream()),
                "tutel_amd_gate_topk_partials")
     return idx, gates, ws, logits, scores
+
+
+def route_fused_scratch(T, M, E, k, dtype):
+    if dtype not in (torch.bfloat16, torch.float16):
+        return 0
+    return int(_lib.lib().tutel_amd_route_fused_scratch_bytes(int(T), int(M), int(E), int(k), _lib.BF16 if dtype == torch.bfloat16 else _lib.F16))
+
+
+def set_route_fused(value):
+    _lib.check(_lib.lib().tutel_amd_set_route_fused(int(value)), "tutel_amd_set_route_fused")
+
+
+def route_fused(x, wg, k, normalize_gate=True, want_logits=False, ws=None, clear=None, want_idx8=False):
+    _dev(x)
+    assert x.dim() == 2 and wg.dim() == 2 and x.shape[1] == wg.shape[1] and x.dtype == wg.dtype
+    T, M = x.shape
+    E = wg.shape[0]
+    k = min(int(k), E)
+    need = route_fused_scratch(T, M, E, k, x.dtype)
+    if need == 0 or T == 0:
+        return None
+    x, wg = x.contiguous(), wg.contiguous()
+    dev = x.device
+    idx = torch.empty([k, T], dtype=torch.int32, device=dev)
+    gates = torch.empty([k, T], dtype=x.dtype, device=dev)
+    logits = torch.empty([T, E], dtype=x.dtype, device=dev) if want_logits else None
+    idx8 = torch.empty([k * T], dtype=torch.uint8, device=dev) if want_idx8 else None
+    if ws is None:
+        ws = routing_workspace(T, E, k, dev)
+    scratch = torch.empty([need], dtype=torch.uint8, device=dev)
+    rc = _lib.lib().tutel_amd_route_fused(_ptr(x), _ptr(wg), _code(x), T, M, E, k, int(bool(normalize_gate)), _ptr(logits), _ptr(idx), _ptr(idx8),
+                                          _ptr(gates), _ptr(ws), ws.numel(), _ptr(clear), clear.numel() if clear is not None else 0,
+                                          _ptr(scratch), scratch.numel(), _stream())
+    if rc == _lib.ENOTSUP:
+        return None
+    _lib.check(rc, "tutel_amd_route_fused")
+    return idx, gates, ws, logits, idx8
 
 
 def gate_logits(x, wg):
```

Result: slower. 16.53 million (-1.9%).
